# haiciyang/LaDiffCodec

Measured on AMD Instinct MI355X. Metric: audio-sec decoded / wall-sec, 16kHz 3kbps 50-step DDPM, higher is better.
Workload: dtype bf16; 1 GPU; LaDiffCodec 3 kbps, diff_dims=256, enc_ratios 8 4, 50-step DDPM, batch=32x2.4 s utterances per GPU; global_batch=32, latent_len=1200, denoise_steps=50, rccl_ranks=1, batches_in_flight=1, parallelism=dp1 (utterance-sharded, no data-path collective)

## Files before the change

include/ladiffcodec.h:

```cpp
#ifndef LADIFFCODEC_H_
#define LADIFFCODEC_H_

#include <stdint.h>

#ifdef __cplusplus
extern "C" {
#endif

#define LDC_OK 0
#define LDC_E_INVALID -1
#define LDC_E_STATE -2
#define LDC_E_MISSING -3
#define LDC_E_HIP -4
#define LDC_E_NOMEM -5

#define LDC_F32 0
#define LDC_BF16 1
#define LDC_BF16_W8 2

#define LDC_MODEL_MAIN 0
#define LDC_MODEL_COND 1

#define LDC_MAX_RATIOS 8

// ... 146 lines not shown
                     int32_t* cdf_out, void* stream);
int ldc_ac_encode(ldc_ctx* ctx, const int32_t* symbols, const int32_t* cdf, int B, int S, int card, int n_static, int total_range_bits,
                  uint8_t* out, int64_t out_stride, int64_t* nbytes_out, void* stream);
int ldc_ac_decode(ldc_ctx* ctx, const uint8_t* in, int64_t in_stride, const int64_t* nbytes, const int32_t* cdf, int B, int S, int card,
                  int n_static, int total_range_bits, int32_t* symbols_out, int32_t* status_out, void* stream);
int ldc_ac_encode_ragged(ldc_ctx* ctx, const int32_t* symbols, const int32_t* n_sym, const int32_t* cdf, int B, int S, int card,
                         int n_static, int total_range_bits, uint8_t* out, int64_t out_stride, int64_t* nbytes_out, void* stream);
int ldc_ac_decode_ragged(ldc_ctx* ctx, const uint8_t* in, int64_t in_stride, const int64_t* nbytes, const int32_t* n_sym,
                         const int32_t* cdf, int B, int S, int card, int n_static, int total_range_bits, int32_t* symbols_out,
                         int32_t* status_out, void* stream);

int64_t ldc_resample_out_len(int64_t T, int orig_freq, int new_freq);
int ldc_resample(ldc_ctx* ctx, const float* wav, int C, int64_t T, int orig_freq, int new_freq, float* out, void* stream);

int ldc_train_q_sample(ldc_ctx* ctx, const float* x_start, const int64_t* t, const float* noise, int B, int C, int L, float* x_t,
                       void* stream);
int ldc_train_num_timesteps(ldc_ctx* ctx);
int ldc_train_predict_x_start(ldc_ctx* ctx, const float* x_t, const float* eps, const int64_t* t, int B, int C, int L, float* x0_out,
                              void* stream);
int ldc_train_neg_sdsdr(ldc_ctx* ctx, const float* est, const float* tgt, int B, int64_t n_per_item, float clip_min, float* per_item_out,
                        void* stream);

int ldc_train_l1_loss(ldc_ctx* ctx, const float* model_out, const float* target, const int64_t* t, int B, int C, int L, float* loss_out,
                      float* grad_out, void* stream);
int64_t ldc_train_block_ws_floats(int B, int Cin, int Cout, int L, int groups);
int ldc_train_block_forward(ldc_ctx* ctx, const float* x, const float* w, const float* bias, const float* gamma, const float* beta,
                            const float* scale_shift, int B, int Cin, int Cout, int L, int groups, float* y, float* ws, void* stream);
int ldc_train_block_backward(ldc_ctx* ctx, const float* dy, const float* x, const float* gamma, const float* beta,
                             const float* scale_shift, int B, int Cin, int Cout, int L, int groups, float* ws, float* dx, float* dw,
                             float* db, float* dgamma, float* dbeta, float* dscale_shift, void* stream);

int ldc_train_layernorm_forward(ldc_ctx* ctx, const float* x, const float* g, int B, int C, int L, float* y, float* stats, void* stream);
int ldc_train_layernorm_backward(ldc_ctx* ctx, const float* dy, const float* x, const float* g, const float* stats, int B, int C, int L,
                                 float* dx, float* dg, void* stream);

int ldc_train_pointwise_forward(ldc_ctx* ctx, const float* x, const float* w, const float* bias, int B, int Cin, int Cout, int L, int pre_silu,
                                float* y, void* stream);
int ldc_train_pointwise_backward(ldc_ctx* ctx, const float* dy, const float* x, const float* w, int B, int Cin, int Cout, int L, int pre_silu,
                                 float* dx, float* dw, float* db, void* stream);

int64_t ldc_train_linattn_ws_floats(int B, int heads, int dim_head, int N);
int ldc_train_linattn_forward(ldc_ctx* ctx, const float* qkv, int B, int heads, int dim_head, int N, float* out, float* ws, void* stream);
int ldc_train_linattn_backward(ldc_ctx* ctx, const float* dout, const float* qkv, int B, int heads, int dim_head, int N, float* ws, float* dqkv,
                               void* stream);

int ldc_train_conv_forward(ldc_ctx* ctx, const float* x, const float* w, const float* bias, int B, int Cin, int Cout, int Lin, int K, int stride,
                           int pad, float* y, void* stream);
int ldc_train_conv_backward(ldc_ctx* ctx, const float* dy, const float* x, const float* w, int B, int Cin, int Cout, int Lin, int K, int stride,
                            int pad, float* dx, float* dw, float* db, void* stream);
int ldc_train_join(ldc_ctx* ctx, void* stream);
int ldc_train_side_stream(ldc_ctx* ctx, void** stream_out);
int ldc_train_upsample2(ldc_ctx* ctx, const float* in, int64_t rows, int L, int backward, float* out, void* stream);
int ldc_train_activation(ldc_ctx* ctx, const float* x, const float* dy, int64_t n, int kind, float* out, void* stream);
int64_t ldc_train_attn_ws_floats(int B, int heads, int N);
int ldc_train_attn_forward(ldc_ctx* ctx, const float* qkv, int B, int heads, int dim_head, int N, float* out, float* ws, void* stream);
int ldc_train_attn_backward(ldc_ctx* ctx, const float* dout, const float* qkv, int B, int heads, int dim_head, int N, float* ws, float* dqkv,
                            void* stream);

int ldc_train_convtr_forward(ldc_ctx* ctx, const float* x, const float* w, const float* bias, int B, int Cin, int Cout, int L, int ratio, float* y,
                             void* stream);
int ldc_train_convtr_backward(ldc_ctx* ctx, const float* dy, const float* x, const float* w, int B, int Cin, int Cout, int L, int ratio, float* dx,
                              float* dw, float* db, void* stream);
int ldc_train_maxscale(ldc_ctx* ctx, const float* x, const float* dy, int B, int64_t n_per_item, float* out, void* stream);

int ldc_train_adam_step(ldc_ctx* ctx, float* param, const float* grad, float* exp_avg, float* exp_avg_sq, int64_t n, int step, float lr,
                        float beta1, float beta2, float eps, void* stream);
int ldc_train_adam_step_dev(ldc_ctx* ctx, float* param, const float* grad, float* exp_avg, float* exp_avg_sq, int64_t n, int32_t* step_dev,
                            float lr, float beta1, float beta2, float eps, void* stream);

int ldc_sconv1d(ldc_ctx* ctx, const float* x, int B, int Cin, int L, const float* w_host, const float* b_host,
                int Cout, int k, int stride, int dilation, int causal, int pre_elu, float* y, void* stream);
int ldc_sconvtr1d(ldc_ctx* ctx, const float* x, int B, int Cin, int L, const float* w_host, const float* b_host,
                  int Cout, int k, int stride, int causal, float* y, void* stream);
int ldc_slstm(ldc_ctx* ctx, const float* x, int B, int H, int T, const float* const* weights_host, int layers,
              float* y, void* stream);

int ldc_unet_debug_tap(ldc_ctx* ctx, const char* name, float* out, int64_t capacity_elems, void* stream);
int ldc_unet_step_cost(ldc_ctx* ctx, int B, int L, double* flops, double* bytes);
int ldc_profile_enable(ldc_ctx* ctx, int on);
int ldc_xcc_census(ldc_ctx* ctx, const uint32_t* mask, int n_words, int wgs, int* hist16);

int ldc_debug_attn_core(ldc_ctx* ctx, int kind, const float* qkv, int B, int L, const float* w_out, const float* b_out,
                        const float* gain, const float* resid, int C, float* out, void* stream);
int ldc_debug_attention_block(ldc_ctx* ctx, const char* name, const float* x, int B, int L, float* out, void* stream);

int ldc_debug_sea_conv(ldc_ctx* ctx, const float* x, int B, int Cin, int L, const float* w_host, const float* b_host, int Cout, int k,
                       int stride, int dilation, int causal, int transposed, int pre_elu, const float* residual, float* y, int* route,
                       void* stream);
int ldc_debug_sea_op(ldc_ctx* ctx, int which, int decoder, int index, const float* x, int B, int L, float* out, int64_t capacity_elems,
                     int* info, void* stream);

int ldc_debug_raise_failure(ldc_ctx* ctx, int code);
long long ldc_debug_sync_count(void);

int ldc_host_stats(ldc_ctx* ctx, int reset, double* graph_launch_ms, double* lookahead_wait_ms, int64_t* graph_launches);
int ldc_stream_info(ldc_ctx* ctx, int* good, int* candidates, double* one_spin_ms, double* all_spin_ms, int* parts);
int ldc_clock_sample(ldc_ctx* ctx, uint64_t* out2, void* stream);

int ldc_timeline_enable(ldc_ctx* ctx, int on);
int ldc_timeline_read(ldc_ctx* ctx, int part, int n, uint64_t* ticks);
int ldc_kstamps_enable(ldc_ctx* ctx, int on);
int ldc_kstamps_reset(ldc_ctx* ctx);
int ldc_kstamps_read(ldc_ctx* ctx, int idx, int n_steps, int* n_ops, uint64_t* ticks, char* infos, int info_cap, int* classes);
int ldc_gn_microbench(ldc_ctx* ctx, int dtype, int B, int L, int C, int with_residual, int iters, double* ms_per_launch);
int ldc_conv_microbench(ldc_ctx* ctx, int dtype, int B, int L, int cin1, int cin2, int cout, int k, int stride, int ups,
                        int iters, double* ms_per_launch);
int ldc_conv_compare(ldc_ctx* ctx, int dtype, int B, int L, int cin1, int cin2, int cout, int k, int stride, int ups, int tile_cfg,
                     int with_gn, int with_colmax, int with_residual, double* max_abs_diff, double* max_abs_ref, double* max_rel_stat);
int ldc_ln_fold_compare(ldc_ctx* ctx, int dtype, int rows, int C, int n_out, double dc, double* max_abs_diff2, double* max_abs_ref);
int ldc_conv_compare_fp8(ldc_ctx* ctx, int B, int L, int cin1, int cin2, int cout, int k, int stride, int ups, int with_gn, int with_colmax,
                         double* max_abs_diff, double* max_abs_ref, double* max_rel_stat);
int ldc_profile_read(ldc_ctx* ctx, double* conv_ms_total, int64_t* conv_launches, double* conv_flops_total);
enum {
  LDC_CLASS_OTHER = 0,
  LDC_CLASS_CONV = 1,
  LDC_CLASS_GN_APPLY = 2,
  LDC_CLASS_LAYERNORM = 3,
  LDC_CLASS_LINATTN = 4,
  LDC_CLASS_ATTN_FULL = 5,
  LDC_CLASS_ELEMENTWISE = 6,
  LDC_N_CLASSES = 7
};
int ldc_profile_read_classes(ldc_ctx* ctx, int n, double* ms, int64_t* launches, double* flops, double* bytes);

#ifdef __cplusplus
}
#endif
#endif
```

ladiffcodec_amd/csrc/attention.hip:

```cpp
#include <algorithm>

#include "ldc_kernels.h"
#include "ldc_math.h"

namespace ldc {

__device__ __forceinline__ float abf2f(unsigned short h) { return __uint_as_float(((unsigned)h) << 16); }
__device__ __forceinline__ unsigned short af2bf(float f) { return hw_bf16(f); }
template <typename T>
__device__ __forceinline__ float ld1(const void* p, size_t i);
template <>
__device__ __forceinline__ float ld1<float>(const void* p, size_t i) { return reinterpret_cast<const float*>(p)[i]; }
template <>
__device__ __forceinline__ float ld1<__bf16>(const void* p, size_t i) {
  return abf2f(reinterpret_cast<const unsigned short*>(p)[i]);
}
template <typename T>
__device__ __forceinline__ void st1(void* p, size_t i, float v);
template <>
__device__ __forceinline__ void st1<float>(void* p, size_t i, float v) { reinterpret_cast<float*>(p)[i] = v; }
template <>
__device__ __forceinline__ void st1<__bf16>(void* p, size_t i, float v) {
  reinterpret_cast<unsigned short*>(p)[i] = af2bf(v);
}
// ... 47 lines not shown
  float acc[4] = {0.f, 0.f, 0.f, 0.f};
  float ssum = 0.f;
  for (int t0 = r0; t0 < r1; t0 += TR) {
    const int nr = min(TR, r1 - t0);
    for (int idx = tid; idx < TR * D; idx += 256) {
      const int r = idx / D, c = idx % D;
      float p = 0.f, v = 0.f;
      if (r < nr) {
        const size_t base = ((size_t)(b * L + t0 + r)) * (3 * HD);
        p = __expf(ld1<T>(qkv, base + HD + h * D + c) - skmax[c]);
        v = ld1<T>(qkv, base + 2 * HD + h * D + c);
      }
      sp[r][c] = p;
      sv[r][c] = v;
    }
    __syncthreads();
#pragma unroll 8
    for (int r = 0; r < TR; ++r) {
      const float p = sp[r][d];
      const float4 v4 = *reinterpret_cast<const float4*>(&sv[r][e0]);
      acc[0] += p * v4.x; acc[1] += p * v4.y; acc[2] += p * v4.z; acc[3] += p * v4.w;
      ssum += p;
    }
    __syncthreads();
  }
  float* ctx = wsb + 2 * HD + (size_t)h * D * D;
#pragma unroll
  for (int j = 0; j < 4; ++j) atomicAdd(&ctx[d * D + e0 + j], acc[j]);
  if ((tid % 8) == 0) atomicAdd(&wsb[HD + h * D + d], ssum);
}

template <typename T, int D>
__global__ __launch_bounds__(256) void linattn_out_kernel(const void* qkv, void* out, const float* ws, int L, int H,
                                                          size_t ws_stride, float scale, const int* lens, int shift) {
  constexpr int HS = D * D + 8;
  extern __shared__ __attribute__((aligned(16))) char smem_raw[];
  float* sctx = reinterpret_cast<float*>(smem_raw);
  const int HD = H * D;
  const int rows_per_block = 256 / H;
  const int b = blockIdx.y;
  const float* wsb = ws + (size_t)b * ws_stride;
  for (int idx = threadIdx.x; idx < H * D * D; idx += 256) {
    const int h = idx / (D * D), rem = idx % (D * D), d = rem / D;
    sctx[h * HS + rem] = wsb[2 * HD + idx] / wsb[HD + h * D + d];
  }
  __syncthreads();
  const int h = threadIdx.x % H;
  const int r = blockIdx.x * rows_per_block + threadIdx.x / H;
  if (r >= L) return;
  if (r >= valid_rows(lens, shift, b, L)) {
    const size_t ob = ((size_t)(b * L + r)) * HD + h * D;
#pragma unroll
    for (int e = 0; e < D; ++e) st1<T>(out, ob + e, 0.f);
    return;
  }
  const size_t base = ((size_t)(b * L + r)) * (3 * HD) + h * D;
  float q[D];
  float m = -INFINITY;
#pragma unroll
  for (int d = 0; d < D; ++d) { q[d] = ld1<T>(qkv, base + d); m = fmaxf(m, q[d]); }
  float s = 0.f;
#pragma unroll
  for (int d = 0; d < D; ++d) { q[d] = __expf(q[d] - m); s += q[d]; }
  const float inv = scale / s;
#pragma unroll
  for (int d = 0; d < D; ++d) q[d] *= inv;
  const float* c = sctx + h * HS;
  const size_t obase = ((size_t)(b * L + r)) * HD + h * D;
#pragma unroll
  for (int e0 = 0; e0 < D; e0 += 4) {
    float4 o = make_float4(0.f, 0.f, 0.f, 0.f);
#pragma unroll
    for (int d = 0; d < D; ++d) {
      const float4 cv = *reinterpret_cast<const float4*>(&c[d * D + e0]);
      o.x += cv.x * q[d]; o.y += cv.y * q[d]; o.z += cv.z * q[d]; o.w += cv.w * q[d];
    }
    st1<T>(out, obase + e0 + 0, o.x); st1<T>(out, obase + e0 + 1, o.y);
    st1<T>(out, obase + e0 + 2, o.z); st1<T>(out, obase + e0 + 3, o.w);
  }
}

typedef float lf32x16 __attribute__((ext_vector_type(16)));
typedef __bf16 lbf16x8 __attribute__((ext_vector_type(8)));
__device__ __forceinline__ lf32x16 mfma_bf16(const uint4& a, const uint4& b, lf32x16 acc) {
  lbf16x8 va, vb;
  __builtin_memcpy(&va, &a, 16);
  __builtin_memcpy(&vb, &b, 16);
  return __builtin_amdgcn_mfma_f32_32x32x16_bf16(va, vb, acc, 0, 0, 0);
}

template <int R>
__global__ __launch_bounds__(256) void linattn_ctx_mfma_kernel(const unsigned short* qkv, float* ws, int Lfull, size_t ws_stride, const int* lens, int shift) {
  constexpr int H = 4, D = 32, HD = 128, P = R + 8;
  __shared__ __attribute__((aligned(16))) unsigned short spT[HD][P];
  __shared__ __attribute__((aligned(16))) unsigned short svT[HD][P];
  __shared__ float skmax[HD];
  const int b = blockIdx.y, tid = threadIdx.x;
  float* wsb = ws + (size_t)b * ws_stride;
  const int r0 = blockIdx.x * R;
  const int L = valid_rows(lens, shift, b, Lfull);
  if (r0 >= L) return;
  constexpr int NP = R / 16;
  uint4 kk[NP], vv[NP];
#pragma unroll
  for (int i = 0; i < NP; ++i) {
    const int id = tid + 256 * i, row = id >> 4, c16 = id & 15;
    if (r0 + row < L) {
      const unsigned short* base = qkv + ((size_t)b * Lfull + r0 + row) * (3 * HD) + 8 * c16;
      kk[i] = *reinterpret_cast<const uint4*>(base + HD);
      vv[i] = *reinterpret_cast<const uint4*>(base + 2 * HD);
    } else {
      kk[i] = make_uint4(0, 0, 0, 0); vv[i] = make_uint4(0, 0, 0, 0);
    }
  }
  if (tid < HD) skmax[tid] = fkey_inv(reinterpret_cast<const unsigned*>(wsb)[tid]);
  __syncthreads();
#pragma unroll
  for (int i = 0; i < NP; ++i) {
    const int id = tid + 256 * i, row = id >> 4, c16 = id & 15;
    const bool live = r0 + row < L;
    const unsigned kw[4] = {kk[i].x, kk[i].y, kk[i].z, kk[i].w};
    const unsigned vw[4] = {vv[i].x, vv[i].y, vv[i].z, vv[i].w};
#pragma unroll
    for (int m = 0; m < 8; ++m) {
      const int col = 8 * c16 + m;
      const unsigned short kb = (unsigned short)((m & 1) ? (kw[m >> 1] >> 16) : (kw[m >> 1] & 0xffffu));
      const unsigned short vb = (unsigned short)((m & 1) ? (vw[m >> 1] >> 16) : (vw[m >> 1] & 0xffffu));
      spT[col][row] = live ? af2bf(__expf(abf2f(kb) - skmax[col])) : (unsigned short)0;
      svT[col][row] = vb;
    }
  }
  __syncthreads();
  const int h = tid >> 6, lane = tid & 63, i32 = lane & 31, g = lane >> 5;
  lf32x16 acc;
#pragma unroll
  for (int r = 0; r < 16; ++r) acc[r] = 0.f;
#pragma unroll
  for (int sx = 0; sx < R / 16; ++sx) {
    const uint4 a = *reinterpret_cast<const uint4*>(&spT[h * D + i32][16 * sx + 8 * g]);
    const uint4 bq = *reinterpret_cast<const uint4*>(&svT[h * D + i32][16 * sx + 8 * g]);
    acc = mfma_bf16(a, bq, acc);
  }
  float* ctx = wsb + 2 * HD + (size_t)h * D * D;
#pragma unroll
  for (int r = 0; r < 16; ++r) {
    const int d = (r & 3) + 8 * (r >> 2) + 4 * g;
    atomicAdd(&ctx[d * D + i32], acc[r]);
  }
  if (tid < HD) {
    float sum = 0.f;
#pragma unroll
    for (int q8 = 0; q8 < R / 8; ++q8) {
      const uint4 u = *reinterpret_cast<const uint4*>(&spT[tid][8 * q8]);
      const unsigned w[4] = {u.x, u.y, u.z, u.w};
#pragma unroll
      for (int m = 0; m < 4; ++m) sum += abf2f((unsigned short)(w[m] & 0xffffu)) + abf2f((unsigned short)(w[m] >> 16));
    }
    atomicAdd(&wsb[HD + tid], sum);
  }
}

template <int TILES>
__global__ __launch_bounds__(256) void linattn_out_mfma_kernel(const unsigned short* qkv, unsigned short* out, const float* ws,
                                                               int L, size_t ws_stride, float scale, const int* lens, int shift) {
  constexpr int D = 32, HD = 128;
  const int b = blockIdx.y, tid = threadIdx.x;
  const int h = tid >> 6, lane = tid & 63, i32 = lane & 31, g = lane >> 5;
  const int r0 = blockIdx.x * (32 * TILES);
  const int Lv = valid_rows(lens, shift, b, L);
  uint4 qq[TILES][2];
#pragma unroll
  for (int t = 0; t < TILES; ++t) {
    const int n = r0 + 32 * t + i32;
#pragma unroll
    for (int sx = 0; sx < 2; ++sx) {
      if (n < Lv) qq[t][sx] = *reinterpret_cast<const uint4*>(qkv + ((size_t)b * L + n) * (3 * HD) + h * D + 16 * sx + 8 * g);
      else qq[t][sx] = make_uint4(0, 0, 0, 0);
    }
  }
  const float* wsb = ws + (size_t)b * ws_stride;
  uint4 af[2];
#pragma unroll
  for (int sx = 0; sx < 2; ++sx) {
    unsigned w[4];
#pragma unroll
    for (int m = 0; m < 8; m += 2) {
      const int d0 = 16 * sx + 8 * g + m;
      const float c0 = wsb[2 * HD + (size_t)h * D * D + d0 * D + i32] * (scale / wsb[HD + h * D + d0]);
      const float c1 = wsb[2 * HD + (size_t)h * D * D + (d0 + 1) * D + i32] * (scale / wsb[HD + h * D + d0 + 1]);
      w[m >> 1] = (unsigned)af2bf(c0) | ((unsigned)af2bf(c1) << 16);
    }
    af[sx] = make_uint4(w[0], w[1], w[2], w[3]);
  }
#pragma unroll
  for (int t = 0; t < TILES; ++t) {
    const int n = r0 + 32 * t + i32;
    float x[16];
    float mx = -INFINITY;
#pragma unroll
    for (int sx = 0; sx < 2; ++sx) {
      const unsigned w[4] = {qq[t][sx].x, qq[t][sx].y, qq[t][sx].z, qq[t][sx].w};
#pragma unroll
      for (int m = 0; m < 4; ++m) {
        x[8 * sx + 2 * m] = abf2f((unsigned short)(w[m] & 0xffffu));
        x[8 * sx + 2 * m + 1] = abf2f((unsigned short)(w[m] >> 16));
      }
    }
#pragma unroll
    for (int m = 0; m < 16; ++m) mx = fmaxf(mx, x[m]);
    mx = fmaxf(mx, __shfl_xor(mx, 32));
    float sum = 0.f;
#pragma unroll
    for (int m = 0; m < 16; ++m) { x[m] = __expf(x[m] - mx); sum += x[m]; }
    sum += __shfl_xor(sum, 32);
    const float inv = 1.0f / sum;
    uint4 bq[2];
#pragma unroll
    for (int sx = 0; sx < 2; ++sx) {
      unsigned w[4];
#pragma unroll
      for (int m = 0; m < 4; ++m)
        w[m] = (unsigned)af2bf(x[8 * sx + 2 * m] * inv) | ((unsigned)af2bf(x[8 * sx + 2 * m + 1] * inv) << 16);
      bq[sx] = make_uint4(w[0], w[1], w[2], w[3]);
    }
    lf32x16 acc;
#pragma unroll
    for (int r = 0; r < 16; ++r) acc[r] = 0.f;
    acc = mfma_bf16(af[0], bq[0], acc);
    acc = mfma_bf16(af[1], bq[1], acc);
    if (n < L) {
      unsigned short* orow = out + ((size_t)b * L + n) * HD + h * D;
#pragma unroll
      for (int rr = 0; rr < 4; ++rr) {
        const unsigned lo = (unsigned)af2bf(acc[4 * rr]) | ((unsigned)af2bf(acc[4 * rr + 1]) << 16);
        const unsigned hi = (unsigned)af2bf(acc[4 * rr + 2]) | ((unsigned)af2bf(acc[4 * rr + 3]) << 16);
        *reinterpret_cast<uint2*>(orow + 8 * rr + 4 * g) = n < Lv ? make_uint2(lo, hi) : make_uint2(0u, 0u);
      }
    }
  }
}


__device__ __forceinline__ float reduce16_over32(const float (&v)[16], int lane) {
  float a8[8], a4[4], a2[2];
  const bool b4 = lane & 16, b3 = lane & 8, b2 = lane & 4, b1 = lane & 2;
#pragma unroll
  for (int k = 0; k < 8; ++k) a8[k] = (b4 ? v[8 + k] : v[k]) + __shfl_xor(b4 ? v[k] : v[8 + k], 16);
#pragma unroll
  for (int k = 0; k < 4; ++k) a4[k] = (b3 ? a8[4 + k] : a8[k]) + __shfl_xor(b3 ? a8[k] : a8[4 + k], 8);
#pragma unroll
  for (int k = 0; k < 2; ++k) a2[k] = (b2 ? a4[2 + k] : a4[k]) + __shfl_xor(b2 ? a4[k] : a4[2 + k], 4);
  float a1 = (b1 ? a2[1] : a2[0]) + __shfl_xor(b1 ? a2[0] : a2[1], 2);
  a1 += __shfl_xor(a1, 1);
  return a1;
}

template <int C>
__global__ __launch_bounds__(256) void linattn_tail_mfma_kernel(const unsigned short* qkv, const float* ws, size_t ws_stride, float scale,
                                                                const unsigned short* wo, int n_pad, const float* bias, const float* gain,
                                                                const unsigned short* resid, unsigned short* out, int L, unsigned* fail_flag) {
  constexpr int D = 32, HD = 128, R = 32, CPW = C / 4, NT = CPW / 32;
  constexpr int AP = HD + 8;
  constexpr int TP = CPW * 4 + 16;
  extern __shared__ __attribute__((aligned(16))) char smem[];
  unsigned short* sA = reinterpret_cast<unsigned short*>(smem);
  float* sred = reinterpret_cast<float*>(smem + (size_t)R * AP * 2);
  float* srow = sred + 4 * R;
  char* strans = smem + (size_t)R * AP * 2 + (size_t)5 * R * 4;
  const int b = blockIdx.y, tid = threadIdx.x;
  const int w = tid >> 6, lane = tid & 63, i32 = lane & 31, g = lane >> 5;
  const int r0 = blockIdx.x * R;
  const float* wsb = ws + (size_t)b * ws_stride;
  const int colw = w * CPW + i32;
  uint4 bfr[8][NT];
#pragma unroll
  for (int ks = 0; ks < 8; ++ks)
#pragma unroll
    for (int j = 0; j < NT; ++j)
      bfr[ks][j] = *reinterpret_cast<const uint4*>(wo + ((size_t)(ks >> 1) * n_pad + colw + 32 * j) * 32 + (ks & 1) * 16 + 8 * g);
  float bv[NT], gv[NT];
#pragma unroll
  for (int j = 0; j < NT; ++j) { bv[j] = bias[colw + 32 * j]; gv[j] = gain[colw + 32 * j]; }
  {
    const int h = w;
    const int n = r0 + i32;
    uint4 qq[2];
#pragma unroll
    for (int sx = 0; sx < 2; ++sx) {
      if (n < L) qq[sx] = *reinterpret_cast<const uint4*>(qkv + ((size_t)b * L + n) * (3 * HD) + h * D + 16 * sx + 8 * g);
      else qq[sx] = make_uint4(0, 0, 0, 0);
    }
    uint4 af[2];
    bool ks_bad = false;
#pragma unroll
    for (int sx = 0; sx < 2; ++sx) {
      unsigned wv[4];
#pragma unroll
      for (int m = 0; m < 8; m += 2) {
        const int d0 = 16 * sx + 8 * g + m;
        const float ks0 = wsb[HD + h * D + d0], ks1 = wsb[HD + h * D + d0 + 1];
        ks_bad |= !(ks0 >= kLinattnKsumMin && ks0 < kLinattnKsumMax) | !(ks1 >= kLinattnKsumMin && ks1 < kLinattnKsumMax);
        const float c0 = wsb[2 * HD + (size_t)h * D * D + d0 * D + i32] * (scale / ks0);
        const float c1 = wsb[2 * HD + (size_t)h * D * D + (d0 + 1) * D + i32] * (scale / ks1);
        wv[m >> 1] = (unsigned)af2bf(c0) | ((unsigned)af2bf(c1) << 16);
      }
      af[sx] = make_uint4(wv[0], wv[1], wv[2], wv[3]);
    }
    if (ks_bad && fail_flag) __hip_atomic_store(fail_flag, kDevFailCtxRange, __ATOMIC_RELAXED, __HIP_MEMORY_SCOPE_SYSTEM);
    float x[16];
    float mx = -INFINITY;
#pragma unroll
    for (int sx = 0; sx < 2; ++sx) {
      const unsigned wv[4] = {qq[sx].x, qq[sx].y, qq[sx].z, qq[sx].w};
#pragma unroll
      for (int m = 0; m < 4; ++m) {
        x[8 * sx + 2 * m] = abf2f((unsigned short)(wv[m] & 0xffffu));
        x[8 * sx + 2 * m + 1] = abf2f((unsigned short)(wv[m] >> 16));
      }
    }
#pragma unroll
    for (int m = 0; m < 16; ++m) mx = fmaxf(mx, x[m]);
    mx = fmaxf(mx, __shfl_xor(mx, 32));
    float sum = 0.f;
#pragma unroll
    for (int m = 0; m < 16; ++m) { x[m] = __expf(x[m] - mx); sum += x[m]; }
    sum += __shfl_xor(sum, 32);
    const float inv = 1.0f / sum;
    uint4 bq[2];
#pragma unroll
    for (int sx = 0; sx < 2; ++sx) {
      unsigned wv[4];
#pragma unroll
      for (int m = 0; m < 4; ++m)
        wv[m] = (unsigned)af2bf(x[8 * sx + 2 * m] * inv) | ((unsigned)af2bf(x[8 * sx + 2 * m + 1] * inv) << 16);
      bq[sx] = make_uint4(wv[0], wv[1], wv[2], wv[3]);
    }
    lf32x16 acc1;
#pragma unroll
    for (int r = 0; r < 16; ++r) acc1[r] = 0.f;
    acc1 = mfma_bf16(af[0], bq[0], acc1);
    acc1 = mfma_bf16(af[1], bq[1], acc1);
    unsigned short* arow = sA + (size_t)i32 * AP + h * D;
#pragma unroll
    for (int rr = 0; rr < 4; ++rr) {
      const unsigned lo = (unsigned)af2bf(acc1[4 * rr]) | ((unsigned)af2bf(acc1[4 * rr + 1]) << 16);
      const unsigned hi = (unsigned)af2bf(acc1[4 * rr + 2]) | ((unsigned)af2bf(acc1[4 * rr + 3]) << 16);
      *reinterpret_cast<uint2*>(arow + 8 * rr + 4 * g) = make_uint2(lo, hi);
    }
  }
  __syncthreads();
  lf32x16 acc[NT];
#pragma unroll
  for (int j = 0; j < NT; ++j)
#pragma unroll
    for (int r = 0; r < 16; ++r) acc[j][r] = 0.f;
#pragma unroll
  for (int ks = 0; ks < 8; ++ks) {
    const uint4 afr = *reinterpret_cast<const uint4*>(sA + (size_t)i32 * AP + 16 * ks + 8 * g);
#pragma unroll
    for (int j = 0; j < NT; ++j) acc[j] = mfma_bf16(afr, bfr[ks][j], acc[j]);
  }
  constexpr int LPR = CPW / 4;
  constexpr int RPS = 64 / LPR;
  constexpr int NSW = R / RPS;
  const int rsub = lane / LPR, piece = lane % LPR;
  uint2 rres[NSW];
#pragma unroll
  for (int sw = 0; sw < NSW; ++sw) {
    const int n = r0 + sw * RPS + rsub;
    rres[sw] = n < L ? *reinterpret_cast<const uint2*>(resid + ((size_t)b * L + n) * C + w * CPW + piece * 4) : make_uint2(0, 0);
  }
#pragma unroll
  for (int j = 0; j < NT; ++j)
#pragma unroll
    for (int r = 0; r < 16; ++r) acc[j][r] += bv[j];
  const int rr = i32 >> 1;
  const int my_row = (rr & 3) + 8 * (rr >> 2) + 4 * g;
  {
    float v[16];
#pragma unroll
    for (int r = 0; r < 16; ++r) {
      float sacc = 0.f;
#pragma unroll
      for (int j = 0; j < NT; ++j) sacc += acc[j][r];
      v[r] = sacc;
    }
    const float tot = reduce16_over32(v, lane);
    if ((lane & 1) == 0) sred[w * R + my_row] = tot;
  }
  __syncthreads();
  if (tid < R) srow[tid] = (sred[tid] + sred[R + tid] + sred[2 * R + tid] + sred[3 * R + tid]) * (1.0f / (float)C);
  __syncthreads();
  float mean[16];
#pragma unroll
  for (int r = 0; r < 16; ++r) mean[r] = srow[(r & 3) + 8 * (r >> 2) + 4 * g];
  {
    float v[16];
#pragma unroll
    for (int r = 0; r < 16; ++r) {
      float sacc = 0.f;
#pragma unroll
      for (int j = 0; j < NT; ++j) { const float d = acc[j][r] - mean[r]; sacc = fmaf(d, d, sacc); }
      v[r] = sacc;
    }
    const float tot = reduce16_over32(v, lane);
    if ((lane & 1) == 0) sred[w * R + my_row] = tot;
  }
  __syncthreads();
  if (tid < R) srow[tid] = rsqrtf((sred[tid] + sred[R + tid] + sred[2 * R + tid] + sred[3 * R + tid]) * (1.0f / (float)C) + 1e-5f);
  __syncthreads();
  char* tw = strans + (size_t)w * R * TP;
#pragma unroll
  for (int r = 0; r < 16; ++r) {
    const int row = (r & 3) + 8 * (r >> 2) + 4 * g;
    const float rstd = srow[row];
#pragma unroll
    for (int j = 0; j < NT; ++j)
      reinterpret_cast<float*>(tw + (size_t)row * TP)[32 * j + i32] = (acc[j][r] - mean[r]) * rstd * gv[j];
  }
#pragma unroll
  for (int sw = 0; sw < NSW; ++sw) {
    const int row = sw * RPS + rsub;
    const int n = r0 + row;
    const float4 y = *reinterpret_cast<const float4*>(tw + (size_t)row * TP + piece * 16);
    const float o0 = y.x + abf2f((unsigned short)(rres[sw].x & 0xffffu)), o1 = y.y + abf2f((unsigned short)(rres[sw].x >> 16));
    const float o2 = y.z + abf2f((unsigned short)(rres[sw].y & 0xffffu)), o3 = y.w + abf2f((unsigned short)(rres[sw].y >> 16));
    const uint2 o = make_uint2((unsigned)af2bf(o0) | ((unsigned)af2bf(o1) << 16), (unsigned)af2bf(o2) | ((unsigned)af2bf(o3) << 16));
    if (n < L) *reinterpret_cast<uint2*>(out + ((size_t)b * L + n) * C + w * CPW + piece * 4) = o;
  }
}

template <int C>
static hipError_t launch_tail_cfg(const void* qkv, const float* ws, size_t wss, float scale, const void* wo, int n_pad, const float* bias,
                                  const float* gain, const void* resid, void* out, int B, int L, unsigned* fail_flag, hipStream_t s) {
  constexpr int R = 32, CPW = C / 4;
  const size_t lds = (size_t)R * (128 + 8) * 2 + (size_t)5 * R * 4 + (size_t)4 * R * (CPW * 4 + 16);
  auto kern = linattn_tail_mfma_kernel<C>;
  static bool lds_opt_in = false;
  if (!lds_opt_in) {
    hipError_t e = hipFuncSetAttribute(reinterpret_cast<const void*>(kern), hipFuncAttributeMaxDynamicSharedMemorySize, 160 * 1024);
    if (e != hipSuccess) return e;
    lds_opt_in = true;
  }
  hipLaunchKernelGGL(kern, dim3((L + R - 1) / R, B), dim3(256), lds, s, reinterpret_cast<const unsigned short*>(qkv), ws, wss, scale,
                     reinterpret_cast<const unsigned short*>(wo), n_pad, bias, gain, reinterpret_cast<const unsigned short*>(resid),
                     reinterpret_cast<unsigned short*>(out), L, fail_flag);
  return hipGetLastError();
}

bool linattn_tail_supported(int dt, int heads, int dim_head, int C) {
  return dt == DT_BF16 && heads == 4 && dim_head == 32 && (C == 256 || C == 512 || C == 1024);
}

hipError_t launch_linattn_ctx(int dt, const void* qkv, float* ws, int B, int L, int heads, int dim_head, hipStream_t s) {
  if (dt != DT_BF16 || heads != 4 || dim_head != 32) return hipErrorInvalidValue;
  const size_t wss = linattn_ws_per_item(heads, dim_head);
  hipLaunchKernelGGL(linattn_ctx_mfma_kernel<64>, dim3((L + 63) / 64, B), dim3(256), 0, s, reinterpret_cast<const unsigned short*>(qkv), ws, L, wss,
                     static_cast<const int*>(nullptr), 0);
  return hipGetLastError();
}

hipError_t launch_linattn_tail(int dt, const void* qkv, const float* ws, const void* wo_packed, int n_pad, const float* bias, const float* gain,
                               const void* resid, void* out, int B, int L, int heads, int dim_head, int C, unsigned* fail_flag, hipStream_t s) {
  if (!linattn_tail_supported(dt, heads, dim_head, C) || !bias || !gain || !resid) return hipErrorInvalidValue;
  const size_t wss = linattn_ws_per_item(heads, dim_head);
  const float scale = 1.0f / sqrtf((float)dim_head);
  if (C == 256) return launch_tail_cfg<256>(qkv, ws, wss, scale, wo_packed, n_pad, bias, gain, resid, out, B, L, fail_flag, s);
  if (C == 512) return launch_tail_cfg<512>(qkv, ws, wss, scale, wo_packed, n_pad, bias, gain, resid, out, B, L, fail_flag, s);
  return launch_tail_cfg<1024>(qkv, ws, wss, scale, wo_packed, n_pad, bias, gain, resid, out, B, L, fail_flag, s);
}

size_t linattn_ws_floats_per_item(int heads, int dim_head) { return linattn_ws_per_item(heads, dim_head); }

hipError_t launch_linattn_kmax(int dt, const void* qkv, float* ws, int B, int L, int heads, int dim_head, hipStream_t s, const int* lens, int shift) {
  const int HD = heads * dim_head;
  if (dim_head != 32 || HD > 256 || 256 % HD) return hipErrorInvalidValue;
  const size_t wss = linattn_ws_per_item(heads, dim_head);
  hipError_t e = hipMemsetAsync(ws, 0, (size_t)B * wss * sizeof(float), s);
  if (e != hipSuccess) return e;
  const int rpb = 128;
  if (dt == DT_F32) hipLaunchKernelGGL(linattn_kmax_kernel<float>, dim3((L + rpb - 1) / rpb, B), dim3(256), 0, s, qkv, ws, L, HD, rpb, wss, lens, shift);
  else hipLaunchKernelGGL(linattn_kmax_kernel<__bf16>, dim3((L + rpb - 1) / rpb, B), dim3(256), 0, s, qkv, ws, L, HD, rpb, wss, lens, shift);
  return hipGetLastError();
}

hipError_t launch_linattn(int dt, const void* qkv, void* out, float* ws, int B, int L, int heads, int dim_head,
                          bool kmax_fused, hipStream_t s, const int* lens, int shift, bool ws_zeroed) {
  if (lens && kmax_fused) return hipErrorInvalidValue;
  if (dim_head != 32 || heads * dim_head > 256 || 256 % (heads * dim_head) || 256 % heads) return hipErrorInvalidValue;
  const int HD = heads * dim_head;
  const size_t wss = linattn_ws_per_item(heads, dim_head);
  if (!kmax_fused && !ws_zeroed) {
    hipError_t e = hipMemsetAsync(ws, 0, (size_t)B * wss * sizeof(float), s);
    if (e != hipSuccess) return e;
  }
  const int rpb = 128;
  const int chunks = (L + rpb - 1) / rpb;
  const float scale = 1.0f / sqrtf((float)dim_head);
  const size_t lds_out = (size_t)heads * (dim_head * dim_head + 8) * sizeof(float);
  const int rows_out = 256 / heads;
  if (dt == DT_BF16 && heads == 4) {
    if (!kmax_fused) hipLaunchKernelGGL(linattn_kmax_kernel<__bf16>, dim3(chunks, B), dim3(256), 0, s, qkv, ws, L, HD, rpb, wss, lens, shift);
    hipLaunchKernelGGL(linattn_ctx_mfma_kernel<64>, dim3((L + 63) / 64, B), dim3(256), 0, s,
                       reinterpret_cast<const unsigned short*>(qkv), ws, L, wss, lens, shift);
    hipLaunchKernelGGL(linattn_out_mfma_kernel<2>, dim3((L + 63) / 64, B), dim3(256), 0, s,
                       reinterpret_cast<const unsigned short*>(qkv), reinterpret_cast<unsigned short*>(out), ws, L, wss, scale, lens, shift);
  } else if (dt == DT_F32) {
    if (!kmax_fused) hipLaunchKernelGGL(linattn_kmax_kernel<float>, dim3(chunks, B), dim3(256), 0, s, qkv, ws, L, HD, rpb, wss, lens, shift);
    hipLaunchKernelGGL((linattn_ctx_kernel<float, 32>), dim3(chunks, B * heads), dim3(256), 0, s, qkv, ws, L, heads, rpb, wss, lens, shift);
    hipLaunchKernelGGL((linattn_out_kernel<float, 32>), dim3((L + rows_out - 1) / rows_out, B), dim3(256), lds_out, s, qkv,
                       out, ws, L, heads, wss, scale, lens, shift);
  } else {
    if (!kmax_fused) hipLaunchKernelGGL(linattn_kmax_kernel<__bf16>, dim3(chunks, B), dim3(256), 0, s, qkv, ws, L, HD, rpb, wss, lens, shift);
    hipLaunchKernelGGL((linattn_ctx_kernel<__bf16, 32>), dim3(chunks, B * heads), dim3(256), 0, s, qkv, ws, L, heads, rpb, wss, lens, shift);
    hipLaunchKernelGGL((linattn_out_kernel<__bf16, 32>), dim3((L + rows_out - 1) / rows_out, B), dim3(256), lds_out, s,
                       qkv, out, ws, L, heads, wss, scale, lens, shift);
  }
  return hipGetLastError();
}

template <typename T, int D>
__global__ __launch_bounds__(256) void attn_full_kernel(const void* qkv, void* out, int L, int H, float scale, int CH, const int* lens, int shift) {
  constexpr int P = D + 4;
  extern __shared__ __attribute__((aligned(16))) char smem_raw[];
  float* sk = reinterpret_cast<float*>(smem_raw);
  float* sv = sk + (size_t)CH * P;
  const int HD = H * D;
  const int b = blockIdx.x / H, h = blockIdx.x % H;
  const int part = threadIdx.x & 3;
  const int i = blockIdx.y * 64 + (threadIdx.x >> 2);
  const int Lv = valid_rows(lens, shift, b, L);
  const int iq = min(i, Lv - 1);
  float q[D], acc[D];
  const size_t qb = ((size_t)(b * L + iq)) * (3 * HD) + h * D;
#pragma unroll
  for (int d = 0; d < D; ++d) { q[d] = ld1<T>(qkv, qb + d) * scale; acc[d] = 0.f; }
  float m = -INFINITY, l = 0.f;
  for (int k0 = 0; k0 < Lv; k0 += CH) {
    const int nk = min(CH, Lv - k0);
    if (k0) __syncthreads();
    for (int idx = threadIdx.x; idx < nk * (D / 8); idx += 256) {
      const int r = idx / (D / 8), c8 = idx % (D / 8);
      const size_t base = ((size_t)(b * L + k0 + r)) * (3 * HD) + h * D + c8 * 8;
#pragma unroll
      for (int mm = 0; mm < 8; ++mm) {
        sk[r * P + c8 * 8 + mm] = ld1<T>(qkv, base + HD + mm);
        sv[r * P + c8 * 8 + mm] = ld1<T>(qkv, base + 2 * HD + mm);
      }
    }
    __syncthreads();
    for (int j = part; j < nk; j += 4) {
      const float4* kj = reinterpret_cast<const float4*>(sk + (size_t)j * P);
// ... 62 lines not shown
```

ladiffcodec_amd/csrc/ldc_api.cpp:

```cpp
#include "ldc_internal.h"

long long g_device_syncs = 0;

static thread_local char g_err[1024] = "";
int fail(int code, const char* fmt, ...) {
  va_list ap;
  va_start(ap, fmt);
  vsnprintf(g_err, sizeof(g_err), fmt, ap);
  va_end(ap);
  return code;
}

extern "C" const char* ldc_last_error(void) { return g_err; }
extern "C" const char* ldc_version(void) { return "ladiffcodec-amd 0.1 (gfx950)"; }



static std::vector<float> fold_weight_norm(const HostTensor& g, const HostTensor& v) {
  const size_t n0 = (size_t)v.shape[0], inner = v.numel() / n0;
  std::vector<float> w(v.numel());
  for (size_t i = 0; i < n0; ++i) {
    double s = 0;
    for (size_t j = 0; j < inner; ++j) s += (double)v.data[i * inner + j] * v.data[i * inner + j];
    const float nrm = (float)sqrt(s);
// ... 702 lines not shown
  return LDC_OK;
}

void drop_plans(ldc_ctx* c) {
  (void)counted_device_sync();
  for (auto& g : c->graphs) g.destroy();
  c->graphs.clear();
  for (auto& pl : c->plans) {
    for (hipEvent_t e : pl->marker_events) (void)hipEventDestroy(e);
    if (pl->arena_base) (void)hipFree(pl->arena_base);
    if (pl->x0_prev) (void)hipFree(pl->x0_prev);
    if (pl->win_base) (void)hipFree(pl->win_base);
  }
  c->plans.clear();
  c->plan_bytes = 0;
  c->last_halves = Halves();
}

extern "C" int ldc_destroy(ldc_ctx* c) {
  if (!c) return LDC_OK;
  (void)hipSetDevice(c->device);
  (void)counted_device_sync();
  drop_plans(c);
  if (c->scratch) (void)hipFree(c->scratch);
  if (c->outnorm_ws) (void)hipFree(c->outnorm_ws);
  if (c->state_buf) (void)hipFree(c->state_buf);
  if (c->ddim_table) (void)hipFree(c->ddim_table);
  if (c->dpm_table) (void)hipFree(c->dpm_table);
  if (c->step_state) (void)hipFree(c->step_state);
  if (c->dev_flag_host) (void)hipHostFree(c->dev_flag_host);
  if (c->tl_buf) (void)hipFree(c->tl_buf);
  for (auto& e : c->prof_events) { (void)hipEventDestroy(e.first); (void)hipEventDestroy(e.second); }
  if (c->ev_fork) (void)hipEventDestroy(c->ev_fork);
  for (int k = 0; k < kMaxParts; ++k) {
    for (int e = 0; e <= ldc_ctx::kLstmChunks; ++e)
      if (c->lstm_ev[k][e]) (void)hipEventDestroy(c->lstm_ev[k][e]);
  }
  for (auto& e : c->flow_ev) if (e) (void)hipEventDestroy(e);
  for (int k = 1; k < kMaxParts; ++k) {
    if (c->ev_join[k]) (void)hipEventDestroy(c->ev_join[k]);
    if (c->aux_stream[k]) (void)hipStreamDestroy(c->aux_stream[k]);
  }
  for (int k = 0; k < kMaxParts; ++k) {
    if (c->ev_side_fork[k]) (void)hipEventDestroy(c->ev_side_fork[k]);
    if (c->ev_side_join[k]) (void)hipEventDestroy(c->ev_side_join[k]);
    if (c->side_stream[k]) (void)hipStreamDestroy(c->side_stream[k]);
  }
  if (c->own_stream) (void)hipStreamDestroy(c->own_stream);
  delete c;
  return LDC_OK;
}

extern "C" void ldc_quantize_e4m3(const float* in, int64_t n, uint8_t* out_codes, float* out_values) {
  for (int64_t i = 0; i < n; ++i) {
    const uint8_t q = host_f32_to_e4m3(in[i]);
    if (out_codes) out_codes[i] = q;
    if (out_values) out_values[i] = host_e4m3_to_f32(q);
  }
}

struct OptRef { int* p; bool replan; int lo, hi; };
static bool find_option(ldc_ctx* c, const std::string& n, OptRef* r) {
#define LDC_OPT(NAME, FIELD, REPLAN, LO, HI) if (n == NAME) { r->p = &(FIELD); r->replan = REPLAN; r->lo = LO; r->hi = HI; return true; }
  LDC_OPT("split", c->split_batch, true, 1, kMaxParts)
  LDC_OPT("part_graphs", c->part_graphs, false, 0, 2)
  LDC_OPT("graph_steps", c->graph_steps, false, 0, 1000)
  LDC_OPT("flow_depth", c->flow_depth, false, 0, (int)ldc_ctx::kFlowRing - 1)
  LDC_OPT("split_ends", c->split_ends, false, 0, 1)
  LDC_OPT("ends_join", c->ends_join, false, 0, 1)
  LDC_OPT("split_init", c->split_init, true, 0, 1)
  LDC_OPT("side_streams", c->side_streams, true, 0, 1)
  LDC_OPT("serial_parts", c->serial_parts, false, 0, 1)
  LDC_OPT("stream_calib", c->calib, false, 0, 1)
  LDC_OPT("merge_advance", c->merge_advance, true, 0, 1)
  LDC_OPT("fuse_gn_stats", c->fuse_gn_stats, true, 0, 1)
  LDC_OPT("fuse_gn_epi", c->fuse_gn_epi, true, 0, 1)
  LDC_OPT("gn_epi_min_l", c->gn_epi_min_l, true, 0, 1 << 30)
  LDC_OPT("gn_epi_max_tiles", c->gn_epi_max_tiles, true, 0, 1 << 30)
  LDC_OPT("fold_res", c->fold_res, true, 0, 1)
  LDC_OPT("fold_ln", c->fold_ln, true, 0, 1)
  LDC_OPT("fuse_kmax", c->fuse_kmax, true, 0, 1)
  LDC_OPT("fuse_ln", c->fuse_ln, true, 0, 1)
  LDC_OPT("fuse_attn_tail", c->fuse_attn_tail, true, 0, 1)
  LDC_OPT("fold_ctx", c->fold_ctx, true, 0, 1)
  LDC_OPT("conv_lean", c->tune.lean, true, 0, 1)
  LDC_OPT("conv_generic", c->tune.force_generic, true, 0, 1)
  LDC_OPT("conv_small_tiles", c->tune.small_max, true, 0, 1 << 30)
  LDC_OPT("conv_splitk", c->tune.splitk, true, 0, 4)
  LDC_OPT("sk_tiles", c->tune.sk_tiles, true, 0, 1 << 30)
  LDC_OPT("sk_u2", c->tune.sk_u2, true, 0, 1 << 30)
  LDC_OPT("sk_u3", c->tune.sk_u3, true, 0, 1 << 30)
  LDC_OPT("conv_mfast", c->tune.m_fastest, true, 0, 2)
  LDC_OPT("conv_debug", c->tune.debug, true, 0, 255)
  LDC_OPT("conv_tile", c->tune.force_tile, true, -1, 1)
  LDC_OPT("conv_xcd_order", c->tune.xcd_order, true, 0, 8)
  LDC_OPT("gn_nap", c->tune.gn_nap, true, 0, 4096)
  LDC_OPT("gn_nap0", c->tune.gn_nap0, true, 0, 4096)
  LDC_OPT("lstm_stream", c->lstm_stream_only, false, 0, 1)
  LDC_OPT("lstm_xcd", c->lstm_xcd, false, 0, 1)
  LDC_OPT("lstm_pipe", c->lstm_pipe, false, 0, 1)
  LDC_OPT("coop_launch", c->coop_launch, false, 0, 1)
  LDC_OPT("sea_splitk", c->sea_splitk, false, 0, 1)
  LDC_OPT("rvq_tiled", c->rvq_tiled, false, 0, 1)
  LDC_OPT("train_bf16", g_train_bf16, false, 0, 1)
  LDC_OPT("train_fp32_mfma", g_train_fp32_mfma, false, 0, 1)
  LDC_OPT("train_valu", g_train_valu, false, 0, 1)
  LDC_OPT("train_dw_side", g_train_dw_side, false, 0, 1)
#undef LDC_OPT
  return false;
}

extern "C" int ldc_set_option(ldc_ctx* c, const char* name, int value) {
  if (!c || !name) return fail(LDC_E_INVALID, "null context or option name");
  const std::string n(name);
  if (n == "fp8_act") {
    if (c->finalized) return fail(LDC_E_STATE, "fp8_act must be set before ldc_finalize_weights");
    c->fp8_act = value ? 1 : 0;
    return LDC_OK;
  }
  if (n == "plan_cache_gb") { c->plan_bytes_cap = (size_t)std::max(1, value) << 30; return LDC_OK; }
  if (n == "plan_cache_n") { c->plan_count_cap = std::max(2 * kMaxParts, value); return LDC_OK; }
  OptRef r;
  if (!find_option(c, n, &r)) return fail(LDC_E_INVALID, "unknown option '%s' (tools/README.md lists the options)", name);
  if (value < r.lo || value > r.hi) return fail(LDC_E_INVALID, "option %s must be in %d..%d", name, r.lo, r.hi);
  if (n == "side_streams" && value && c->split_batch != 1) return fail(LDC_E_INVALID, "side streams need a single chain (split 1)");
  if (value == *r.p) return LDC_OK;
  if (r.replan && c->live_pools > 0)
    return fail(LDC_E_STATE, "option %s rebuilds every plan, and %d decode pool(s) keep their items' state in theirs: destroy the pools first", name, c->live_pools);
  if (r.replan && !c->plans.empty()) { HIPCHK(hipSetDevice(c->device)); drop_plans(c); }
  *r.p = value;
  if (n == "split" && value != 1) c->side_streams = 0;
  return LDC_OK;
}

extern "C" long long ldc_debug_sync_count(void) { return g_device_syncs; }

extern "C" int ldc_debug_raise_failure(ldc_ctx* c, int code) {
  if (!c || !c->dev_flag_host || (code != 1 && code != 2 && code != (int)kDevFailCtxRange)) return fail(LDC_E_INVALID, "bad arguments");
  *reinterpret_cast<volatile unsigned*>(c->dev_flag_host) = (unsigned)code;
  return LDC_OK;
}

extern "C" int ldc_reseed(ldc_ctx* c, uint64_t seed) {
  if (!c) return fail(LDC_E_INVALID, "null ctx");
  c->cfg.noise_seed = seed;
  c->noise_epoch = 0;
  return LDC_OK;
}

extern "C" int ldc_set_weight(ldc_ctx* c, int which, const char* key, const float* data, const int64_t* shape, int ndim) {
  if (!c || !key || !data || (ndim > 0 && !shape)) return fail(LDC_E_INVALID, "null argument");
  if (which != LDC_MODEL_MAIN && which != LDC_MODEL_COND) return fail(LDC_E_INVALID, "which must be LDC_MODEL_MAIN or LDC_MODEL_COND");
  if (c->finalized) return fail(LDC_E_STATE, "weights already finalized");
  HostTensor t;
  t.shape.assign(shape, shape + ndim);
  t.data.assign(data, data + t.numel());
  c->raw[which][key] = std::move(t);
  return LDC_OK;
}

extern "C" int ldc_finalize_weights(ldc_ctx* c, int strict) {
  if (!c) return fail(LDC_E_INVALID, "null ctx");
  if (c->finalized) return fail(LDC_E_STATE, "already finalized");
  HIPCHK(hipSetDevice(c->device));
  std::string missing;
  std::vector<int> main_ratios(c->cfg.enc_ratios, c->cfg.enc_ratios + c->cfg.n_enc_ratios);
// ... 609 lines not shown
      };
      epi1 = (!f8 || dt == DT_BF16) && few_tiles(t1) && t1[0] <= 2 * L && take_part(&ge1, L, t1[0], t1[1], r.cout);
      conv_bm(f8 ? r.c2_f8 : r.c2, L, L, false, t2);
      epi2 = (!(out_mode & 1) || dt == DT_BF16) && few_tiles(t2) && t2[0] <= 2 * L && take_part(&ge2, L, t2[0], t2[1], r.cout);
    }
    void* a = epi1 ? nullptr : act(rows, r.cout);
    void* d = epi2 ? nullptr : act(rows, r.cout);
    const void* res = x1;
    bool folded = false;
    void* rr = r.has_res ? act(rows, r.cout) : nullptr;
    if (r.has_res && c->fold_res && r.c1r.w) {
      int t[4];
      conv_bm(r.c1, L, L, false, t);
      folded = t[0] > 0 && t[2] == 1;
    }
    if (r.has_res && !folded) {
      mark(2);
      where = 1;
      conv(r.res, x1, x2, rr, nullptr, L, L);
      where = 0;
    }
    if (r.has_res) res = rr;
    const ConvLayer& c1 = folded ? r.c1r : r.c1;
    const ResnetW* rp = &r;
    if (epi1) {
      ge1.gamma = r.g1; ge1.beta = r.b1; ge1.ss = cur_ss + r.ss_off; ge1.out = f8 ? 1 : 0;
      if (folded) y2_next = rr;
      conv(c1, x1, x2, b, nullptr, L, L, nullptr, nullptr, 0, 0, 0, &ge1);
    } else {
      if (folded) y2_next = rr;
      conv(c1, x1, x2, a, nullptr, L, L, fuse_stats ? st1 : nullptr);
      if (!fuse_stats) add([=](hipStream_t s) { return launch_gn_stats(dt, a, Bn, L, rp->cout, g, st1, s, ln, sh); });
      add([=](hipStream_t s) {
        if (item_t)
          return launch_gn_apply(dt, a, b, nullptr, Bn, L, rp->cout, g, st1, rp->g1, rp->b1, ss_tab, ss_stride, item_t, ACT_SILU, s, nullptr,
                                 nullptr, 0, ln, sh, kItemStateInts, n_t);
        return launch_gn_apply(dt, a, b, nullptr, Bn, L, rp->cout, g, st1, rp->g1, rp->b1, cur_ss + rp->ss_off,
                               0, nullptr, ACT_SILU, s, nullptr, nullptr, f8 ? 1 : 0, ln, sh);
      }, false, 0, LDC_CLASS_GN_APPLY, (f8 ? 1.5 : 2.0) * Bn * L * rp->cout * es);
    }
    void* xn = nullptr;
    if (ln_g && xn_out && c->fuse_ln && !ln && gn_apply_ln_fusable(r.cout)) {
      xn = xn_fp8 ? ar->alloc((size_t)rows * r.cout) : act(rows, r.cout);
      *xn_out = xn;
    }
    if (epi2) {
      ge2.gamma = r.g2; ge2.beta = r.b2; ge2.ss = nullptr; ge2.out = out_mode & 5;
      if (rowstat_wanted && !f8) ge2.rowstat = last_rowstat = (float*)ar->alloc((size_t)rows * (r.cout / 32) * 8);
      if (r.has_res && !folded) mark(3);
      conv(f8 ? r.c2_f8 : r.c2, b, nullptr, out, res, L, L, nullptr, nullptr, 0, 0, 0, &ge2);
      if (xn) {
        const int C = r.cout;
        add([=](hipStream_t s) { return launch_ln_rows(dt, out, xn, nullptr, ln_g, rows, C, s, xn_fp8 ? 1 : 0); }, false, 0, LDC_CLASS_LAYERNORM,
            (xn_fp8 ? 1.5 : 2.0) * rows * C * es);
      }
      return out;
    }
    conv(f8 ? r.c2_f8 : r.c2, b, nullptr, d, nullptr, L, L, fuse_stats ? st2 : nullptr);
    if (!fuse_stats) add([=](hipStream_t s) { return launch_gn_stats(dt, d, Bn, L, rp->cout, g, st2, s, ln, sh); });
    if (r.has_res && !folded) mark(3);
    const int out8_ln = ((xn && xn_fp8) ? 2 : 0) | (gn_apply_fp8_ok(r.cout) ? out_mode : 0);
    add([=](hipStream_t s) {
      return launch_gn_apply(dt, d, out, res, Bn, L, rp->cout, g, st2, rp->g2, rp->b2, nullptr, 0, nullptr, ACT_SILU, s, xn, ln_g, out8_ln, ln, sh);
    }, false, 0, LDC_CLASS_GN_APPLY, (xn ? 4.0 : 3.0) * Bn * L * rp->cout * es);
    return out;
  }
  bool qkv_fp8(const LinAttnW& a) const { return c->w8 && c->fp8_act && a.qkv_f8.w != nullptr; }
  bool ln_foldable(const LinAttnW& a, int L) {
    if (pl->ragged || !c->fold_ln || !c->fuse_gn_epi || c->w8 || !a.qkv_ln.w || L < c->gn_epi_min_l) return false;
    int t[4];
    conv_bm(a.qkv_ln, L, L, false, t);
    return t[0] > 0;
  }
  void* attention(const LinAttnW& a, const void* x, int L, bool linear, void* xn_pre = nullptr) {
    const int rows = B * L, dt = c->dt, Bn = B;
    const int H = c->unet.heads, Dh = c->unet.dim_head, hid = H * Dh;
    const bool f8 = qkv_fp8(a);
    const bool lnf = !xn_pre && ln_foldable(a, L);
    const float* rowstat = lnf ? last_rowstat : nullptr;
    last_rowstat = nullptr;
    void* xn = lnf ? const_cast<void*>(x) : (xn_pre ? xn_pre : (f8 ? ar->alloc((size_t)rows * a.dim) : act(rows, a.dim)));
    const ConvLayer& qkv_ly = lnf ? a.qkv_ln : (f8 ? a.qkv_f8 : a.qkv);
    void* qkv = act(rows, 3 * hid);
    void* o = act(rows, hid);
    void* out = act(rows, a.dim);
    const LinAttnW* ap = &a;
    const int* ln = lens();
    const int sh = ln ? level(L) : 0;
    float* ws = (linear && (c->fuse_kmax || ln)) ? linattn_ws + (size_t)(linattn_used++) * B * linattn_ws_floats_per_item(H, Dh) : linattn_ws;
    if (!xn_pre && !lnf)
      add([=](hipStream_t s) { return launch_ln_rows(dt, x, xn, nullptr, ap->norm_g, rows, ap->dim, s, f8 ? 1 : 0, ln, sh, L); }, false, 0, LDC_CLASS_LAYERNORM,
          2.0 * rows * a.dim * es);
    if (linear) {
      const size_t wss = linattn_ws_floats_per_item(H, Dh);
      if (!ln && c->fuse_kmax && c->fuse_attn_tail && !a.out.w8 && linattn_tail_supported(dt, H, Dh, a.dim)) {
        ln_rowstat_next = rowstat;
        if (lnf && c->fold_ctx && c->tune.lean && !c->tune.force_generic && dt == DT_BF16 && a.qkv_ctx.w && hid == 128 && a.dim % 64 == 0) {
          qkv_ctx_next = ws; qkv_ctx_stride_next = (int)wss;
          conv(a.qkv_ctx, xn, nullptr, qkv, nullptr, L, L);
        } else {
          conv(qkv_ly, xn, nullptr, qkv, nullptr, L, L, nullptr, reinterpret_cast<unsigned*>(ws), hid, 2 * hid, (int)wss);
          add([=](hipStream_t s) { return launch_linattn_ctx(dt, qkv, ws, Bn, L, H, Dh, s); }, false, 0, LDC_CLASS_LINATTN, 2.0 * rows * hid * es);
        }
        const int dim = a.dim;
        info = "tail_c" + std::to_string(dim) + "_L" + std::to_string(L) + "_B" + std::to_string(B);
        unsigned* flag = c->dev_flag_dev;
        add([=](hipStream_t s) {
          return launch_linattn_tail(dt, qkv, ws, ap->out.w, ap->out.n_pad, ap->out.bias, ap->out_g, x, out, Bn, L, H, Dh, dim, flag, s);
        }, false, 2.0 * rows * hid * dim, LDC_CLASS_LINATTN, (1.0 * hid + 2.0 * dim) * rows * es);
        return out;
      }
      if (c->fuse_kmax && !ln) {
        ln_rowstat_next = rowstat;
        conv(qkv_ly, xn, nullptr, qkv, nullptr, L, L, nullptr, reinterpret_cast<unsigned*>(ws), hid, 2 * hid, (int)wss);
        add([=](hipStream_t s) { return launch_linattn(dt, qkv, o, ws, Bn, L, H, Dh, true, s); }, false, 0, LDC_CLASS_LINATTN,
            4.0 * rows * hid * es);
      } else {
        ln_rowstat_next = rowstat;
        conv(qkv_ly, xn, nullptr, qkv, nullptr, L, L);
        add([=](hipStream_t s) { return launch_linattn(dt, qkv, o, ws, Bn, L, H, Dh, false, s, ln, sh, ln != nullptr); }, false, 0, LDC_CLASS_LINATTN,
            5.0 * rows * hid * es);
      }
      void* t = act(rows, a.dim);
      conv(a.out, o, nullptr, t, nullptr, L, L);
      add([=](hipStream_t s) { return launch_ln_rows(dt, t, out, x, ap->out_g, rows, ap->dim, s, 0, ln, sh, L); }, false, 0, LDC_CLASS_LAYERNORM,
          3.0 * rows * a.dim * es);
    } else {
      ln_rowstat_next = rowstat;
      conv(qkv_ly, xn, nullptr, qkv, nullptr, L, L);
      add([=](hipStream_t s) { return launch_attn_full(dt, qkv, o, Bn, L, H, Dh, s, ln, sh); }, false, 0, LDC_CLASS_ATTN_FULL, 4.0 * rows * hid * es);
      conv(a.out, o, nullptr, out, x, L, L);
      mask(out, L, a.dim);
    }
    return out;
  }
};

int build_plan(ldc_ctx* c, Plan* pl, Arena& ar, int B, int L, int F) {
  const UnetW& u = c->unet;
  pl->B = B; pl->L = L; pl->F = F; pl->init_pc = nullptr;
  pl->cond_ops.clear(); pl->step_ops.clear(); pl->step_is_conv.clear(); pl->step_where.clear(); pl->step_flops.clear(); pl->step_class.clear(); pl->step_bytes.clear(); pl->step_info.clear(); pl->taps.clear();
  pl->flops = 0; pl->act_bytes = 0; pl->conv_bytes = 0; pl->sk_need_max = 0; pl->part_need = 0;
  const int dt = c->dt;
  const size_t es = dt_size(dt);
  const int Cc = u.cond_channels, Cx = u.channels;
  PlanBuilder pb{c, pl, &ar, B, es};
  pl->zero_once.clear();
  const int n_gn = 2 * (int)(2 * u.downs.size() + 2 + 2 * u.ups.size() + 1);
  const size_t gn_bytes = (size_t)n_gn * B * u.groups * kGnPad * 4;
  const bool lin_zeroed = c->fuse_kmax || pl->ragged;
  const size_t n_lin = lin_zeroed ? u.downs.size() + u.ups.size() : 1;
  const size_t lin_bytes = n_lin * B * linattn_ws_floats_per_item(u.heads, u.dim_head) * 4;
  const int sk_tiles_cap = 1024;
  const size_t part_bytes = (pl->part_bytes + 63) / 64 * 64;
  const size_t sk_count_bytes = (size_t)sk_tiles_cap * 4 + part_bytes;
  const size_t sx_bytes = c->cfg.unet_scale_x ? (size_t)B * 4 : 0;
  pb.stats_pool = (float*)ar.alloc(gn_bytes + sk_count_bytes + lin_bytes + sx_bytes + 64);
  pb.sk_count = reinterpret_cast<unsigned*>(pb.stats_pool + gn_bytes / 4);
  pb.part_pool = reinterpret_cast<char*>(pb.sk_count + sk_tiles_cap);
  pb.part_cap = part_bytes;
  pb.sk_count_cap = sk_tiles_cap;
  pb.linattn_ws = pb.stats_pool + (gn_bytes + sk_count_bytes) / 4;
  float* sx_max = pb.linattn_ws + (lin_zeroed ? lin_bytes / 4 : 0);
  const size_t stats_bytes = gn_bytes + sk_count_bytes + (lin_zeroed ? lin_bytes : 0) + sx_bytes;
  pb.sk_part_cap = pl->sk_floats;
  pb.sk_part = (float*)ar.alloc((size_t)std::max<long long>(pb.sk_part_cap, 4) * 4);
  pl->maxabs = (float*)ar.alloc((size_t)B * 4);
  pl->step_state = (int*)ar.alloc(64);
  if (ar.base) pl->zero_once.push_back({pl->step_state, 64});
  pl->kst = c->kstamps ? (unsigned long long*)ar.alloc((size_t)2048 * kKstOps * 2 * 8) : nullptr;
  pl->cur_ss = (float*)ar.alloc((size_t)std::max(1, u.ss_stride) * 4);
  pl->x_cl = ar.alloc((size_t)B * L * Cx * es);
  pl->eps_cl = ar.alloc((size_t)B * L * Cx * es);
  pl->cond_cl = ar.alloc((size_t)B * L * Cc * es);
  if (pl->items && !pl->ragged) return fail(LDC_E_INVALID, "a per-item plan is a ragged plan");
  pl->item_state = pl->items ? (ItemState*)ar.alloc((size_t)B * sizeof(ItemState)) : nullptr;
  if (pl->ragged) {
    if (c->w8) return fail(LDC_E_INVALID, "ragged batches are not available on the fp8 engine (its fused forms have no length-aware variant): use dtype bf16 or f32");
    pl->lens = (int*)ar.alloc((size_t)B * 4);
    pl->flens = (int*)ar.alloc((size_t)B * 4);
  } else {
    pl->lens = pl->flens = nullptr;
  }
  void* cond_in = ar.alloc((size_t)B * F * Cc * 4);
  pl->cond_in_cl = cond_in;
  {
    const void* x = cond_in;
    int Lc = F;
    const int Bn0 = B;
    const int *rl = pl->ragged ? pl->lens : nullptr, *rf = pl->ragged ? pl->flens : nullptr;
    if (rf) pl->cond_ops.push_back([=](hipStream_t s) { return launch_mask_rows(DT_F32, cond_in, Bn0, F, Cc, rf, 0, s); });
    for (const ConvLayer& ly : u.upsamplers) {
      ConvCall cc;
      cc.B = B; cc.L_in = Lc; cc.L_rows = Lc + 1; cc.L_final = Lc * ly.tr_stride; cc.y_ld = ly.tr_cout; cc.x1 = x; cc.tune = &c->tune;
      void* y = ar.alloc((size_t)B * cc.L_final * ly.tr_cout * 4);
      cc.y = y;
      const ConvLayer* lp = &ly;
      pl->cond_ops.push_back([lp, cc](hipStream_t s) { return launch_conv(*lp, cc, s); });
      if (rf) {
        const int row = cc.L_final / F * ly.tr_cout;
        pl->cond_ops.push_back([=](hipStream_t s) { return launch_mask_rows(DT_F32, y, Bn0, F, row, rf, 0, s); });
      }
      x = y;
      Lc = cc.L_final;
    }
    (void)rl;
    if (Lc != L) return fail(LDC_E_INVALID, "upsampled condition length %d != latent length %d (F=%d, upsampling product %d)", Lc, L, F, upsample_factor(c));
    float* mx = pl->maxabs;
    void* cond_cl = pl->cond_cl;
    const bool scale = c->cfg.unet_scale_cond != 0;
    const int Bn = B;
    const int64_t npi = (int64_t)L * Cc;
// ... 353 lines not shown
                          0, 0.f, s));
  }
  return finish_stream(c, stream);
}

static int unet_halvings(const ldc_ctx* c) {
  int n = 0;
  for (const LevelW& lv : c->unet.downs) n += lv.kind == 0;
  return n;
}
static long long lcm_ll(long long a, long long b) {
  long long x = a, y = b;
  while (y) { const long long t = x % y; x = y; y = t; }
  return a / x * b;
}
int ragged_latent_quantum(const ldc_ctx* c) { return (int)lcm_ll(upsample_factor(c), 1ll << unet_halvings(c)); }
static int check_ragged_lengths(const int32_t* lens, int B, int maxlen, long long quantum, const char* unit) {
  if (!lens) return fail(LDC_E_INVALID, "null lengths");
  if (maxlen <= 0 || maxlen % quantum) return fail(LDC_E_INVALID, "the padded length %d is not a positive multiple of %lld %s", maxlen, quantum, unit);
  for (int b = 0; b < B; ++b)
    if (lens[b] <= 0 || lens[b] > maxlen || lens[b] % quantum)
      return fail(LDC_E_INVALID, "length %d of item %d must be a multiple of %lld %s in (0, %d]", (int)lens[b], b, quantum, unit, maxlen);
  return LDC_OK;
}
static int write_plan_lens(ldc_ctx* c, const Halves& h, const std::vector<int>& lat, hipStream_t s) {
  const int up = upsample_factor(c);
  for (int k = 0; k < h.n; ++k) {
    Plan* pl = h.p[k];
    std::vector<int> fr(pl->B);
    for (int b = 0; b < pl->B; ++b) fr[b] = lat[h.b0[k] + b] / up;
    HIPCHK(launch_lens_write(pl->lens, lat.data() + h.b0[k], pl->B, s));
    HIPCHK(launch_lens_write(pl->flens, fr.data(), pl->B, s));
  }
  return LDC_OK;
}

extern "C" int ldc_unet_forward_ragged(ldc_ctx* c, const float* x, int t, const float* cond, const int32_t* latent_lens_host, int B, int Lmax,
                                       int Fmax, float* eps_out, void* stream) {
  LDCCHK(check_ready(c, LDC_MODEL_MAIN));
  if (!x || !cond || !eps_out) return fail(LDC_E_INVALID, "null tensor");
  if (t < 0 || t >= c->unet.timesteps) return fail(LDC_E_INVALID, "t out of range");
  LDCCHK(check_unet_args(c, B, Lmax, Fmax));
  LDCCHK(check_ragged_lengths(latent_lens_host, B, Lmax, ragged_latent_quantum(c), "latent frames"));
  if (c->w8) return fail(LDC_E_INVALID, "ragged batches are not available on the fp8 engine (its fused forms have no length-aware variant): use dtype bf16 or f32");
  hipStream_t s = pick_stream(c, stream);
  Halves h;
  LDCCHK(get_halves(c, B, Lmax, Fmax, s, &h, true));
  LDCCHK(write_plan_lens(c, h, std::vector<int>(latent_lens_host, latent_lens_host + B), s));
  LDCCHK(load_cond(c, h, cond, s));
  LDCCHK(load_x(c, h, x, s));
  for (int k = 0; k < h.n; ++k) {
    Plan* pl = h.p[k];
    HIPCHK(launch_mask_rows(c->dt, pl->x_cl, pl->B, Lmax, c->unet.channels, pl->lens, 0, s));
    HIPCHK(launch_step_set(pl->step_state, t, 0, c->cur_key, s));
    HIPCHK(launch_step_begin(c->unet.ss_table, c->unet.ss_stride, pl->step_state, pl->cur_ss, nullptr, s, pl->zero_ptr, pl->zero_bytes));
    LDCCHK(run_ops(c, pl, pl->step_ops, true, s));
    HIPCHK(launch_mask_rows(c->dt, pl->eps_cl, pl->B, Lmax, c->unet.channels, pl->lens, 0, s));
    HIPCHK(launch_from_cl(c->dt, pl->eps_cl, eps_out + (size_t)h.b0[k] * c->unet.channels * Lmax, pl->B, c->unet.channels, Lmax, nullptr,
                          0, 0.f, s));
  }
  return finish_stream(c, stream);
}

extern "C" int ldc_unet_debug_tap(ldc_ctx* c, const char* name, float* out, int64_t capacity, void* stream) {
  LDCCHK(check_ready(c, LDC_MODEL_MAIN));
  if (!name || !out) return fail(LDC_E_INVALID, "null argument");
  const Halves& h = c->last_halves;
  if (h.n == 0) return fail(LDC_E_STATE, "no UNet call has been made yet");
  int64_t need = 0;
  for (int k = 0; k < h.n; ++k) {
    auto it = h.p[k]->taps.find(name);
    if (it == h.p[k]->taps.end()) return fail(LDC_E_INVALID, "unknown tap '%s'", name);
    need += (int64_t)h.p[k]->B * it->second.C * it->second.L;
  }
  if (capacity < need) return fail(LDC_E_INVALID, "tap '%s' needs %lld elements", name, (long long)need);
  hipStream_t s = pick_stream(c, stream);
  for (int k = 0; k < h.n; ++k) {
    const Plan::Tap& tp = h.p[k]->taps.find(name)->second;
    HIPCHK(launch_from_cl(c->dt, tp.p, out + (size_t)h.b0[k] * tp.C * tp.L, h.p[k]->B, tp.C, tp.L, nullptr, 0, 0.f, s));
  }
  return finish_stream(c, stream);
}

extern "C" int ldc_debug_attention_block(ldc_ctx* c, const char* name, const float* x, int B, int L, float* out, void* stream) {
  LDCCHK(check_ready(c, LDC_MODEL_MAIN));
  if (!name || !x || !out || B <= 0 || L <= 0) return fail(LDC_E_INVALID, "bad arguments");
  const UnetW& u = c->unet;
  const LinAttnW* a = nullptr;
  bool linear = true;
  const std::string n = name;
  auto level = [&](const char* pre, const std::vector<LevelW>& lv) {
    const size_t pl = strlen(pre);
    if (n.compare(0, pl, pre) != 0 || n.size() == pl || n.find_first_not_of("0123456789", pl) != std::string::npos) return;
    const size_t i = (size_t)atoi(n.c_str() + pl);
    if (i < lv.size()) a = &lv[i].attn;
  };
  if (n == "mid") { a = &u.mid_attn; linear = false; }
  else { level("down", u.downs); level("up", u.ups); }
  if (!a) return fail(LDC_E_INVALID, "unknown attention block '%s' (down0..down%zu, mid, up0..up%zu)", name, u.downs.size() - 1, u.ups.size() - 1);
  hipStream_t s = pick_stream(c, stream);
  const int dt = c->dt, C = a->dim;
  const size_t es = dt_size(dt);
  const size_t lin_bytes = (size_t)B * linattn_ws_floats_per_item(u.heads, u.dim_head) * 4;
  const int sk_tiles_cap = 1024;
  Plan pl;
  pl.B = B; pl.L = L;
  void *x_cl = nullptr, *y_cl = nullptr, *zero = nullptr;
  auto build = [&](Arena& ar) {
    pl.step_ops.clear(); pl.step_is_conv.clear(); pl.step_where.clear(); pl.step_flops.clear(); pl.step_class.clear(); pl.step_bytes.clear(); pl.step_info.clear();
    pl.sk_need_max = 0; pl.part_need = 0;
    PlanBuilder pb{c, &pl, &ar, B, es};
    zero = ar.alloc((size_t)sk_tiles_cap * 4 + lin_bytes);
    pb.sk_count = reinterpret_cast<unsigned*>(zero);
    pb.sk_count_cap = sk_tiles_cap;
    pb.linattn_ws = reinterpret_cast<float*>(pb.sk_count + sk_tiles_cap);
    pb.sk_part_cap = pl.sk_floats;
    pb.sk_part = (float*)ar.alloc((size_t)std::max<long long>(pb.sk_part_cap, 4) * 4);
    x_cl = pb.act(B * L, C);
    y_cl = pb.attention(*a, x_cl, L, linear);
  };
  for (int pass = 0; pass < 2; ++pass) {
    Arena dry;
    build(dry);
    pl.sk_floats = std::max(pl.sk_floats, pl.sk_need_max);
  }
  Arena measure;
  build(measure);
  DevMem keep;
  void* base = nullptr;
  LDCCHK(keep.alloc(&base, measure.off + 4096));
  Arena real;
  real.base = (char*)base; real.cap = measure.off + 4096;
  build(real);
  HIPCHK(hipMemsetAsync(zero, 0, (size_t)sk_tiles_cap * 4 + lin_bytes, s));
  HIPCHK(launch_to_cl(dt, x, x_cl, B, C, L, nullptr, 0, 0.f, s));
  LDCCHK(run_ops(c, &pl, pl.step_ops, true, s));
  HIPCHK(launch_from_cl(dt, y_cl, out, B, C, L, nullptr, 0, 0.f, s));
  HIPCHK(hipStreamSynchronize(s));
  return check_dev_flag(c);
}

static int half_step(ldc_ctx* c, const Halves& h, int k, float* x, const float* noise, int64_t noise_stride, hipStream_t s,
                     const StepSampler& sm = StepSampler()) {
  Plan* pl = h.p[k];
  const size_t off = (size_t)h.b0[k] * c->unet.channels * pl->L;
  unsigned long long* tl = c->timeline ? c->tl_buf + (size_t)k * 2048 * 2 : nullptr;
  if (sm.kind == SAMPLER_DPM) {
    if (!sm.dpm || !pl->x0_prev) return fail(LDC_E_STATE, "internal: a DPM step without its schedule table or history buffer");
    HIPCHK(launch_step_begin_sched(c->unet.ss_table, c->unet.ss_stride, pl->step_state, pl->cur_ss, tl, s, pl->zero_ptr, pl->zero_bytes,
                                   c->merge_advance, &sm.dpm->t, (int)(sizeof(DpmStep) / sizeof(int))));
  } else {
    HIPCHK(launch_step_begin(c->unet.ss_table, c->unet.ss_stride, pl->step_state, pl->cur_ss, tl, s, pl->zero_ptr, pl->zero_bytes, c->merge_advance,
                             sm.kind == SAMPLER_DDIM ? sm.ddim : nullptr));
  }
  LDCCHK(run_ops(c, pl, pl->step_ops, true, s));
  if (pl->win_Ltot) {
    if (sm.kind == SAMPLER_DPM || h.n != 1) return fail(LDC_E_STATE, "internal: a windows plan steps as one part, on DDPM or DDIM");
    HIPCHK(launch_windows_update(c->dt, sm.kind == SAMPLER_DDIM ? WIN_DDIM : WIN_DDPM, x, pl->eps_cl, noise, noise_stride, pl->x_cl, nullptr,
                                 c->unet.channels, pl->win, c->sched, sm.ddim, pl->step_state, s));
  } else if (sm.kind == SAMPLER_DPM)
    HIPCHK(launch_dpm_update(c->dt, x + off, pl->eps_cl, pl->x0_prev, pl->x_cl, pl->B, c->unet.channels, pl->L, c->sched, sm.dpm,
                             pl->step_state, s, pl->ragged ? pl->lens : nullptr));
  else if (sm.kind == SAMPLER_DDIM)
    HIPCHK(launch_ddim_update(c->dt, x + off, pl->eps_cl, noise ? noise + off : nullptr, noise_stride, pl->x_cl, pl->B,
                              c->unet.channels, pl->L, c->sched, sm.ddim, pl->step_state, (uint64_t)off, s, pl->ragged ? pl->lens : nullptr));
  else
    HIPCHK(launch_p_sample_update(c->dt, x + off, pl->eps_cl, noise ? noise + off : nullptr, noise_stride, pl->x_cl, pl->B,
                                  c->unet.channels, pl->L, c->sched, pl->step_state, (uint64_t)off, s, pl->ragged ? pl->lens : nullptr));
  if (!c->merge_advance) HIPCHK(launch_step_advance(pl->step_state, tl, s));
  return LDC_OK;
}
static int stamp_loop_end(ldc_ctx* c, const Halves& h, int k, hipStream_t s) {
  if (!c->timeline || !c->merge_advance) return LDC_OK;
  HIPCHK(launch_step_advance(h.p[k]->step_state, c->tl_buf + (size_t)k * 2048 * 2, s));
  return LDC_OK;
}

bool parts_parallel(ldc_ctx* c, const Halves& h) {
  return h.n >= 2 && !c->profile && !c->serial_parts;
}
int fork_parts(ldc_ctx* c, const Halves& h, hipStream_t s) {
  HIPCHK(hipEventRecord(c->ev_fork, s));
// ... 1102 lines not shown
```

ladiffcodec_amd/csrc/ldc_api_tuning.cpp:

```cpp
#include "ldc_internal.h"

static int round_up(int v, int m) { return (v + m - 1) / m * m; }

extern "C" int ldc_sconv1d(ldc_ctx* c, const float* x, int B, int Cin, int L, const float* w_host, const float* b_host,
                           int Cout, int k, int stride, int dilation, int causal, int pre_elu, float* y, void* stream) {
  if (!c || !x || !w_host || !y) return fail(LDC_E_INVALID, "null argument");
  if (B <= 0 || Cin <= 0 || L <= 0 || Cout <= 0 || k <= 0 || stride <= 0 || dilation <= 0) return fail(LDC_E_INVALID, "bad sizes");
  HIPCHK(hipSetDevice(c->device));
  hipStream_t s = pick_stream(c, stream);
  const int cp = round_up(Cin, 16);
  std::vector<float> wp((size_t)Cout * cp * k, 0.f);
  for (int o = 0; o < Cout; ++o)
    for (int i = 0; i < Cin; ++i)
      for (int t = 0; t < k; ++t) wp[((size_t)o * cp + i) * k + t] = w_host[((size_t)o * Cin + i) * k + t];
  DevMem keep;
  std::swap(keep.ptrs, c->wmem.ptrs);
  ConvLayer ly;
  ConvSpec sp;
  sp.dt = DT_F32; sp.cin1 = cp; sp.cout = Cout; sp.k = k; sp.stride = stride; sp.dil = dilation;
  const int padding_total = (k - 1) * dilation - (stride - 1);
  sp.pad_left = causal ? padding_total : padding_total - padding_total / 2;
  sp.pad_mode = PAD_REFLECT; sp.pre_act = pre_elu ? ACT_ELU : ACT_NONE;
  int rc = make_conv(c, sp, wp.data(), b_host, &ly);
  std::swap(keep.ptrs, c->wmem.ptrs);
// ... 589 lines not shown
  const int L_out = ups ? 2 * L : (stride == 2 ? (L + 2 * sp.pad_left - k) / 2 + 1 : L);
  const size_t es = dt_size(dt);
  const int groups = 8;
  const size_t n_out = (size_t)B * L_out * cout, stat_n = (size_t)B * groups * kGnPad, cm_n = (size_t)B * cout;
  void *x1 = nullptr, *x2 = nullptr, *res = nullptr, *y[2] = {nullptr, nullptr}, *st[2] = {nullptr, nullptr}, *cm[2] = {nullptr, nullptr};
  LDCCHK(keep.alloc(&x1, (size_t)B * L * cin1 * es));
  LDCCHK(fill_random(x1, (size_t)B * L * cin1, dt, 901u));
  if (cin2) {
    LDCCHK(keep.alloc(&x2, (size_t)B * L * cin2 * es));
    LDCCHK(fill_random(x2, (size_t)B * L * cin2, dt, 902u));
  }
  if (with_residual) {
    LDCCHK(keep.alloc(&res, n_out * es));
    LDCCHK(fill_random(res, n_out, dt, 903u));
  }
  void *part = nullptr, *cnt = nullptr;
  LDCCHK(keep.alloc(&part, (size_t)(8 << 20) * 4));
  LDCCHK(keep.alloc(&cnt, 1024 * 4));
  HIPCHK(hipMemset(cnt, 0, 1024 * 4));
  hipStream_t s = c->own_stream;
  ConvTune tune = c->tune;
  for (int v = 0; v < 2; ++v) {
    LDCCHK(keep.alloc(&y[v], n_out * es));
    LDCCHK(keep.alloc(&st[v], stat_n * 4));
    LDCCHK(keep.alloc(&cm[v], cm_n * 4));
    HIPCHK(hipMemset(y[v], 0, n_out * es));
    HIPCHK(hipMemset(st[v], 0, stat_n * 4));
    HIPCHK(hipMemset(cm[v], 0, cm_n * 4));
    HIPCHK(hipDeviceSynchronize());
    const bool lean_ab = tile_cfg >= 100;
    tune.force_generic = lean_ab ? 0 : (v == 0 ? 1 : 0);
    if (lean_ab) tune.lean = tile_cfg >= 300 ? 1 : (tile_cfg >= 200 ? 0 : v);
    tune.force_tile = lean_ab ? (tile_cfg % 100 == 99 ? -1 : tile_cfg % 100) : tile_cfg;
    ConvCall cc;
    cc.B = B; cc.L_in = L; cc.L_rows = L_out; cc.x1 = x1; cc.x2 = x2; cc.y = y[v]; cc.y_ld = cout; cc.residual = res;
    if (with_gn) { cc.gn_sum = (float*)st[v]; cc.gn_groups = groups; }
    if (with_colmax) { cc.colmax = (unsigned*)cm[v]; cc.colmax_lo = 0; cc.colmax_hi = cout; cc.colmax_stride = cout; }
    cc.sk_part = (float*)part; cc.sk_part_cap = (long long)8 << 20; cc.sk_count = (unsigned*)cnt; cc.sk_count_cap = 1024;
    cc.tune = &tune;
    HIPCHK(launch_conv(ly, cc, s));
  }
  HIPCHK(hipStreamSynchronize(s));
  std::vector<char> h0(n_out * es), h1(n_out * es);
  HIPCHK(hipMemcpy(h0.data(), y[0], h0.size(), hipMemcpyDeviceToHost));
  HIPCHK(hipMemcpy(h1.data(), y[1], h1.size(), hipMemcpyDeviceToHost));
  auto val = [&](const std::vector<char>& h, size_t i) {
    if (dt == DT_F32) return (double)reinterpret_cast<const float*>(h.data())[i];
    const uint32_t u = (uint32_t)reinterpret_cast<const uint16_t*>(h.data())[i] << 16;
    float f;
    memcpy(&f, &u, 4);
    return (double)f;
  };
  double d = 0, m = 0;
  for (size_t i = 0; i < n_out; ++i) {
    const double a = val(h0, i), b = val(h1, i);
    if (!(b == b)) { d = 1e30; break; }
    d = std::max(d, fabs(a - b));
    m = std::max(m, fabs(a));
  }
  *max_abs_diff = d;
  *max_abs_ref = m;
  double rs = 0;
  if (with_gn) {
    std::vector<float> s0(stat_n), s1(stat_n);
    HIPCHK(hipMemcpy(s0.data(), st[0], stat_n * 4, hipMemcpyDeviceToHost));
    HIPCHK(hipMemcpy(s1.data(), st[1], stat_n * 4, hipMemcpyDeviceToHost));
    double smax = 0;
    for (size_t i = 0; i < stat_n; ++i) smax = std::max(smax, (double)fabsf(s0[i]));
    for (size_t i = 0; i < stat_n; ++i) rs = std::max(rs, fabs((double)s0[i] - s1[i]) / (smax + 1e-30));
  }
  if (with_colmax) {
    std::vector<unsigned> c0(cm_n), c1(cm_n);
    HIPCHK(hipMemcpy(c0.data(), cm[0], cm_n * 4, hipMemcpyDeviceToHost));
    HIPCHK(hipMemcpy(c1.data(), cm[1], cm_n * 4, hipMemcpyDeviceToHost));
    auto unkey = [](unsigned kx) { const unsigned b = (kx & 0x80000000u) ? (kx & 0x7fffffffu) : ~kx; float f; memcpy(&f, &b, 4); return (double)f; };
    for (size_t i = 0; i < cm_n; ++i) rs = std::max(rs, fabs(unkey(c0[i]) - unkey(c1[i])) / (m + 1e-30));
  }
  *max_rel_stat = rs;
  return LDC_OK;
}

extern "C" int ldc_debug_attn_core(ldc_ctx* c, int kind, const float* qkv, int B, int L, const float* w_out, const float* b_out,
                                   const float* gain, const float* resid, int C, float* out, void* stream) {
  if (!c || !qkv || !out || B < 1 || L < 1 || kind < 0 || kind > 3) return fail(LDC_E_INVALID, "bad arguments");
  HIPCHK(hipSetDevice(c->device));
  const int dt = c->dt, H = 4, D = 32, HD = H * D;
  const size_t es = dt_size(dt), wss = linattn_ws_floats_per_item(H, D);
  if (kind == 2 && (!w_out || !b_out || !gain || !resid || !linattn_tail_supported(dt, H, D, C)))
    return fail(LDC_E_INVALID, "the fused tail needs a bf16 context, C in {256, 512, 1024}, and to_out weight, bias, gain and residual");
  hipStream_t s = pick_stream(c, stream);
  const int Co = kind == 2 ? C : HD;
  DevMem keep;
  void *q_cl = nullptr, *o_cl = nullptr, *ws = nullptr, *r_cl = nullptr;
  LDCCHK(keep.alloc(&q_cl, (size_t)B * L * 3 * HD * es));
  LDCCHK(keep.alloc(&o_cl, (size_t)B * L * Co * es));
  LDCCHK(keep.alloc(&ws, (size_t)B * wss * 4));
  ConvLayer to_out;
  float* d_gain = nullptr;
  if (kind == 2) {
    const bool saved_w8 = c->w8;
    c->w8 = false;
    std::swap(keep.ptrs, c->wmem.ptrs);
    ConvSpec sp;
    sp.dt = dt; sp.cin1 = HD; sp.cout = C; sp.k = 1;
    int rc = make_conv(c, sp, w_out, b_out, &to_out);
    if (rc == LDC_OK) rc = c->wmem.upload(&d_gain, std::vector<float>(gain, gain + C));
    std::swap(keep.ptrs, c->wmem.ptrs);
    c->w8 = saved_w8;
    LDCCHK(rc);
    LDCCHK(keep.alloc(&r_cl, (size_t)B * L * C * es));
    HIPCHK(launch_to_cl(dt, resid, r_cl, B, C, L, nullptr, 0, 0.f, s));
  }
  HIPCHK(launch_to_cl(dt, qkv, q_cl, B, 3 * HD, L, nullptr, 0, 0.f, s));
  if (kind == 0) {
    HIPCHK(launch_linattn(dt, q_cl, o_cl, (float*)ws, B, L, H, D, false, s));
  } else if (kind == 1) {
    HIPCHK(launch_linattn_kmax(dt, q_cl, (float*)ws, B, L, H, D, s));
    HIPCHK(launch_linattn(dt, q_cl, o_cl, (float*)ws, B, L, H, D, true, s));
  } else if (kind == 2) {
    HIPCHK(launch_linattn_kmax(dt, q_cl, (float*)ws, B, L, H, D, s));
    HIPCHK(launch_linattn_ctx(dt, q_cl, (float*)ws, B, L, H, D, s));
    HIPCHK(launch_linattn_tail(dt, q_cl, (const float*)ws, to_out.w, to_out.n_pad, to_out.bias, d_gain, r_cl, o_cl, B, L, H, D, C, c->dev_flag_dev, s));
  } else {
    HIPCHK(launch_attn_full(dt, q_cl, o_cl, B, L, H, D, s));
  }
  HIPCHK(launch_from_cl(dt, o_cl, out, B, Co, L, nullptr, 0, 0.f, s));
  HIPCHK(hipStreamSynchronize(s));
  return check_dev_flag(c);
}

extern "C" int ldc_conv_compare_fp8(ldc_ctx* c, int B, int L, int cin1, int cin2, int cout, int k, int stride, int ups, int with_gn,
                                    int with_colmax, double* max_abs_diff, double* max_abs_ref, double* max_rel_stat) {
  if (!c || !max_abs_diff || !max_abs_ref || !max_rel_stat) return fail(LDC_E_INVALID, "bad arguments");
  if ((cin1 % 64) || (cin2 % 64)) return fail(LDC_E_INVALID, "fp8 inputs need channel counts that are multiples of 64");
  HIPCHK(hipSetDevice(c->device));
  const int cin = cin1 + cin2;
  std::vector<float> w((size_t)cout * cin * k), bias(cout);
  unsigned seed = 777u;
  for (auto& v : w) { seed = seed * 1664525u + 1013904223u; v = ((seed >> 8) * (1.0f / 16777216.0f) - 0.5f) * 0.2f; }
  for (auto& v : bias) { seed = seed * 1664525u + 1013904223u; v = ((seed >> 8) * (1.0f / 16777216.0f) - 0.5f); }
  DevMem keep;
  const bool saved_w8 = c->w8;
  c->w8 = true;
  std::swap(keep.ptrs, c->wmem.ptrs);
  ConvLayer ly[2];
  ConvSpec sp;
  sp.cin1 = cin1; sp.cin2 = cin2; sp.cout = cout; sp.k = k; sp.stride = stride; sp.ups = ups;
  sp.pad_left = (k == 4 && stride == 2) ? 1 : (k - 1) / 2;
  sp.dt = DT_BF16;
  int rc = make_conv(c, sp, w.data(), bias.data(), &ly[0]);
  sp.dt = DT_FP8; sp.act8 = 1;
  if (rc == LDC_OK) rc = make_conv(c, sp, w.data(), bias.data(), &ly[1]);
  std::swap(keep.ptrs, c->wmem.ptrs);
  c->w8 = saved_w8;
  LDCCHK(rc);
  const int L_out = ups ? 2 * L : (stride == 2 ? (L + 2 * sp.pad_left - k) / 2 + 1 : L);
  const int groups = 8;
  const size_t n_out = (size_t)B * L_out * cout, stat_n = (size_t)B * groups * kGnPad, cm_n = (size_t)B * cout;
  auto make_input = [&](size_t n, unsigned sd, void** d8, void** d16) -> int {
    std::vector<uint8_t> h8(n);
    std::vector<uint16_t> h16(n);
    for (size_t i = 0; i < n; ++i) {
      sd = sd * 1664525u + 1013904223u;
      uint8_t code = (uint8_t)(sd >> 13);
      if (((code >> 3) & 0xf) > 8) code = (uint8_t)((code & 0x87) | (8 << 3));
      h8[i] = code;
      const float f = host_e4m3_to_f32(code);
      uint32_t u;
      memcpy(&u, &f, 4);
      h16[i] = (uint16_t)(u >> 16);
    }
    LDCCHK(keep.alloc(d8, n));
    LDCCHK(keep.alloc(d16, n * 2));
    HIPCHK(hipMemcpy(*d8, h8.data(), n, hipMemcpyHostToDevice));
    HIPCHK(hipMemcpy(*d16, h16.data(), n * 2, hipMemcpyHostToDevice));
    return LDC_OK;
  };
  void *x1[2] = {nullptr, nullptr}, *x2[2] = {nullptr, nullptr};
  LDCCHK(make_input((size_t)B * L * cin1, 31u, &x1[1], &x1[0]));
  if (cin2) LDCCHK(make_input((size_t)B * L * cin2, 32u, &x2[1], &x2[0]));
  void *part = nullptr, *cnt = nullptr;
  LDCCHK(keep.alloc(&part, (size_t)(8 << 20) * 4));
  LDCCHK(keep.alloc(&cnt, 1024 * 4));
  HIPCHK(hipMemset(cnt, 0, 1024 * 4));
  hipStream_t s = c->own_stream;
  void *y[2], *st[2], *cm[2];
  for (int v = 0; v < 2; ++v) {
    LDCCHK(keep.alloc(&y[v], n_out * 2));
    LDCCHK(keep.alloc(&st[v], stat_n * 4));
    LDCCHK(keep.alloc(&cm[v], cm_n * 4));
    HIPCHK(hipMemset(y[v], 0, n_out * 2));
    HIPCHK(hipMemset(st[v], 0, stat_n * 4));
    HIPCHK(hipMemset(cm[v], 0, cm_n * 4));
    HIPCHK(hipDeviceSynchronize());
    ConvCall cc;
    cc.B = B; cc.L_in = L; cc.L_rows = L_out; cc.x1 = x1[v]; cc.x2 = x2[v]; cc.y = y[v]; cc.y_ld = cout;
    if (with_gn) { cc.gn_sum = (float*)st[v]; cc.gn_groups = groups; }
    if (with_colmax) { cc.colmax = (unsigned*)cm[v]; cc.colmax_lo = 0; cc.colmax_hi = cout; cc.colmax_stride = cout; }
    cc.sk_part = (float*)part; cc.sk_part_cap = (long long)8 << 20; cc.sk_count = (unsigned*)cnt; cc.sk_count_cap = 1024;
    cc.tune = &c->tune;
    HIPCHK(launch_conv(ly[v], cc, s));
  }
  HIPCHK(hipStreamSynchronize(s));
  std::vector<uint16_t> h0(n_out), h1(n_out);
  HIPCHK(hipMemcpy(h0.data(), y[0], n_out * 2, hipMemcpyDeviceToHost));
// ... 174 lines not shown
```

ladiffcodec_amd/csrc/ldc_internal.h:

```cpp
#pragma once
#include "../../include/ladiffcodec.h"

#include <hip/hip_runtime.h>
#include <math.h>
#include <stdarg.h>
#include <stdio.h>
#include <string.h>

#include <algorithm>
#include <chrono>
#include <functional>
#include <map>
#include <memory>
#include <set>
#include <string>
#include <vector>

#include "ldc_kernels.h"

extern long long g_device_syncs;
inline hipError_t counted_device_sync() {
  ++g_device_syncs;
  return hipDeviceSynchronize();
}
// ... 196 lines not shown
};

struct StepGraph {
  int B = 0, L = 0, F = 0, n = 0;
  int ragged = 0;
  int pool_id = 0;
  int win_Ltot = 0, win_O = 0;
  int sampler = SAMPLER_DDPM;
  const float* noise = nullptr;
  float* x = nullptr;
  hipStream_t stream = nullptr;
  hipGraphExec_t exec[4] = {nullptr, nullptr, nullptr, nullptr};
  hipGraphExec_t pexec[kMaxParts][2] = {};
  bool per_part = false;
  std::vector<hipEvent_t> part_ev;
  uint64_t last_use = 0;
  bool any() const { return exec[0] != nullptr; }
  void destroy() {
    if (per_part) exec[0] = nullptr;
    for (hipEvent_t e : part_ev) (void)hipEventDestroy(e);
    part_ev.clear();
    for (auto& e : exec) { if (e) (void)hipGraphExecDestroy(e); e = nullptr; }
    for (auto& pe : pexec) for (auto& e : pe) { if (e) (void)hipGraphExecDestroy(e); e = nullptr; }
    per_part = false;
  }
};

struct ldc_ctx {
  ldc_config cfg;
  int device = 0;
  int dt = DT_F32;
  bool w8 = false;
  bool finalized = false;
  std::map<std::string, HostTensor> raw[2];
  DevMem wmem;
  Codec codec[2];
  UnetW unet;
  StepTables sched{};
  const float* sqrt_alphas_cumprod = nullptr;
  const float* sqrt_one_minus_alphas_cumprod = nullptr;
  const float* p2_loss_weight = nullptr;
  std::vector<float> alphas_cumprod;
  DdimStep* ddim_table = nullptr;
  std::vector<DdimStep> ddim_host;
  std::vector<float> sqrt_recip_ac, sqrt_recipm1_ac;
  DpmStep* dpm_table = nullptr;
  std::vector<DpmStep> dpm_host;
  int* step_state = nullptr;
  std::vector<std::unique_ptr<Plan>> plans;
  std::vector<StepGraph> graphs;
  Halves last_halves;
  hipStream_t aux_stream[kMaxParts] = {nullptr, nullptr, nullptr, nullptr};
  hipEvent_t ev_fork = nullptr, ev_join[kMaxParts] = {nullptr, nullptr, nullptr, nullptr};
  static constexpr int kLstmChunks = 4;
  hipEvent_t lstm_ev[kMaxParts][kLstmChunks + 1] = {};
  hipStream_t calib_stream = nullptr; bool calibrated = false;
  int calib_good = -1, calib_cand = 0; double calib_one_ms = 0, calib_all_ms = 0;
  struct CalibOrder { hipStream_t s; std::vector<hipStream_t> order; int good, cand; double one_ms, all_ms; };
  std::vector<CalibOrder> calib_cache;
  int calib = 1;
  int ends_join = 0;
  int lstm_pipe = 0;
  int split_batch = 2;
  int merge_advance = 1;
  int rvq_tiled = 1;
  int sea_splitk = 1;
  int split_init = 1;
  int split_ends = 1;
  int fp8_act = 1;
  int part_graphs = 1;
  double host_graph_ms = 0, host_wait_ms = 0;
  long long host_graph_launches = 0;
  hipStream_t side_stream[kMaxParts] = {nullptr, nullptr, nullptr, nullptr};
  hipEvent_t ev_side_fork[kMaxParts] = {nullptr, nullptr, nullptr, nullptr}, ev_side_join[kMaxParts] = {nullptr, nullptr, nullptr, nullptr};
  int side_streams = 0;
  int fuse_kmax = 1;
  int fuse_ln = 1;
  int coop_launch = 0;
  int lstm_xcd = 1;
  int num_cus = 256;
  int xcd_resident[2] = {0, 0};
  int coop_resident[2] = {0, 0};
  int fuse_attn_tail = 1;
  int fold_ctx = 1;
  static constexpr int kFlowRing = 32;
  hipEvent_t flow_ev[kFlowRing] = {};
  unsigned long long flow_n = 0;
  int flow_depth = 8;
  int fuse_gn_stats = 1;
  int gn_epi_max_tiles = 1300;
  int gn_epi_min_l = 0;
  int fold_ln = 1;
  int fold_res = 1;
  int fuse_gn_epi = 1;
  ConvTune tune;
  int lstm_stream_only = 0;
  int serial_parts = 0;
  int graph_steps = 0;
  uint64_t use_tick = 0, call_tick = 0;
  size_t plan_bytes = 0, plan_bytes_cap = (size_t)48 << 30;
  int plan_count_cap = 24;
  int live_pools = 0, next_pool_id = 1;
  uint64_t noise_epoch = 0, cur_key = 0;
  unsigned* dev_flag_host = nullptr;
  unsigned* dev_flag_dev = nullptr;
  int enc_final_act = ACT_NONE;
  unsigned long long* tl_buf = nullptr;
  bool timeline = false;
  bool kstamps = false;
  char* scratch = nullptr;
  size_t scratch_cap = 0;
  void* outnorm_ws = nullptr;
  size_t outnorm_ws_bytes = 0;
  float* state_buf = nullptr;
  size_t state_bytes = 0;
  hipStream_t own_stream = nullptr;
  bool profile = false;
  double prof_ms = 0, prof_flops = 0;
  int64_t prof_launches = 0;
  std::vector<std::pair<hipEvent_t, hipEvent_t>> prof_events;
  std::vector<double> prof_event_flops;
  std::vector<int> prof_event_class;
  std::vector<double> prof_event_bytes;
  std::vector<std::string> prof_event_info;
  double cls_ms[LDC_N_CLASSES] = {}, cls_flops[LDC_N_CLASSES] = {}, cls_bytes[LDC_N_CLASSES] = {};
  int64_t cls_launches[LDC_N_CLASSES] = {};
};

inline hipStream_t pick_stream(ldc_ctx* c, void* s) { return s ? reinterpret_cast<hipStream_t>(s) : c->own_stream; }
inline int check_dev_flag(ldc_ctx* c) {
  const unsigned v = c->dev_flag_host ? *reinterpret_cast<volatile unsigned*>(c->dev_flag_host) : 0u;
  if (v) {
    *reinterpret_cast<volatile unsigned*>(c->dev_flag_host) = 0u;
    if (v == LDC_DEV_BAD_CODE) {
      const uint64_t w = *reinterpret_cast<volatile uint64_t*>(c->dev_flag_host + 2);
      return fail(LDC_E_INVALID, "[bad_code] an RVQ code is outside [0, %d) (e.g. codebook %d, item %d, frame %d); the rows of such "
                                 "codes are NaN", c->codec[LDC_MODEL_COND].bins, (int)(w >> 56), (int)((w >> 32) & 0xffffff), (int)(uint32_t)w);
    }
    if (v == 2)
      return fail(LDC_E_HIP, "device-side failure [gn_wait]: the in-launch GroupNorm exchange of a fused conv timed out (its tiles were "
                             "not all resident in time: is the GPU shared with another process?); the outputs of that call are NaN; "
                             "ldc_set_option(ctx, \"fuse_gn_epi\", 0) restores the separate conv + gn_apply launches");
    if (v == kDevFailCtxRange)
      return fail(LDC_E_HIP, "device-side failure [ctx_range]: the LinearAttention context folded into to_qkv met k values outside the range "
                             "its unshifted exponentials are valid for (a column whose sum of exp(k) is below 2^-100 or reaches 1e26: a k of 60 or more); the "
                             "outputs of that call are wrong; ldc_set_option(ctx, \"fold_ctx\", 0) restores the column maximum and the "
                             "context launch, which shift by it");
    c->lstm_xcd = 0;
    return fail(LDC_E_HIP, "device-side failure [coop_lstm]: cooperative LSTM: the hidden-state exchange timed out (its workgroups were "
                           "not co-resident: is the GPU shared with another process?); the outputs of that call are NaN; "
                           "ldc_set_option(ctx, \"lstm_stream\", 1) selects the streamed LSTM kernel");
  }
  return LDC_OK;
}
inline int finish_stream(ldc_ctx* c, void* s) {
  if (!s) {
    HIPCHK(hipStreamSynchronize(c->own_stream));
    return check_dev_flag(c);
  }
  return LDC_OK;
}
inline uint64_t next_noise_key(ldc_ctx* c, bool draws) {
  c->cur_key = c->cfg.noise_seed ^ (c->noise_epoch * 0x9E3779B97F4A7C15ull);
  if (draws) ++c->noise_epoch;
  return c->cur_key;
}
// ... 114 lines not shown
```

ladiffcodec_amd/csrc/ldc_kernels.h:

```cpp
#pragma once
#include <hip/hip_runtime.h>
#include <stdint.h>

namespace ldc {

enum { DT_F32 = 0, DT_BF16 = 1, DT_FP8 = 2 };
enum { ACT_NONE = 0, ACT_SILU = 1, ACT_ELU = 2, ACT_TANH = 3, ACT_GELU = 4, ACT_SIGMOID = 5, ACT_RELU = 6 };
enum { PAD_ZERO = 0, PAD_REFLECT = 1 };
static constexpr int kGnPad = 16;

inline size_t dt_size(int dt) { return dt == DT_F32 ? 4 : (dt == DT_FP8 ? 1 : 2); }

struct ConvLayer {
  int dt = DT_F32;
  int cin1 = 0, cin2 = 0;
  int n = 0;
  int n_pad = 0;
  int bn = 128;
  int taps = 1, stride = 1, dil = 1, pad_left = 0, ups = 0, pad_mode = PAD_ZERO;
  int pre_act = ACT_NONE, post_act = ACT_NONE;
  int tr_stride = 0, tr_cout = 0, tr_trim_left = 0;
  void* w = nullptr;
  float* bias = nullptr;
  int w8 = 0;
// ... 13 lines not shown
  int debug = 0;
  int gn_nap = 16, gn_nap0 = 0;
  int force_tile = -1;
  int xcd_order = 1;
  int lean = 1;
};

struct ConvCall {
  const void* x1 = nullptr;
  const void* x2 = nullptr;
  void* y = nullptr;
  void* y2 = nullptr;
  const void* residual = nullptr;
  int B = 0;
  int L_in = 0;
  int L_rows = 0;
  int L_final = 0;
  int y_ld = 0;
  float* gn_sum = nullptr;
  int gn_groups = 0;
  unsigned* colmax = nullptr;
  int colmax_lo = 0, colmax_hi = 0, colmax_stride = 0;
  float* qkv_ctx_ws = nullptr;
  int qkv_ctx_stride = 0;
  float* sk_part = nullptr;
  unsigned* sk_count = nullptr;
  long long sk_part_cap = 0;
  int sk_count_cap = 0;
  int generic_split = 0;
  void* gn_part = nullptr;
  int gn_mslots = 0;
  const float* gn_gamma = nullptr;
  const float* gn_beta = nullptr;
  const float* gn_ss = nullptr;
  int gn_out = 0;
  unsigned* fail_flag = nullptr;
  float* rowstat_out = nullptr;
  const float* ln_rowstat = nullptr;
  unsigned long long* kst = nullptr;
  const int* kst_step = nullptr;
  int kst_stride = 0;
  const void* ctx = nullptr;
  const int* ctx_fresh = nullptr;
  int ctx_rows = 0, ctx_zero = 0;
  int check_only = 0;
  const ConvTune* tune = nullptr;
  long long* sk_need = nullptr;
  int* route_out = nullptr;
  int* bm_out = nullptr;
};

enum { CONV_ROUTE_NONE = 0, CONV_ROUTE_CIN1_ROWS = 1, CONV_ROUTE_CIN1_GENERIC = 2, CONV_ROUTE_PIPELINED = 3, CONV_ROUTE_GENERIC = 4 };
hipError_t launch_conv(const ConvLayer& ly, const ConvCall& c, hipStream_t s);
long long conv_generic_splitk_floats(const ConvLayer& ly, const ConvCall& c);
size_t conv_packed_weight_bytes(const ConvLayer& ly);
void pack_conv_weights(const ConvLayer& ly, const float* w_oik, void* dst_host);
void pack_conv_weights_fp8(const ConvLayer& ly, const float* w_oik, void* dst_host, float* scales);
void pack_conv_weights_fp8act(const ConvLayer& ly, const float* w_oik, void* dst_host, float* scales);
uint8_t host_f32_to_e4m3(float f);
float host_e4m3_to_f32(uint8_t v);
void pack_convtr_weights(const ConvLayer& ly, const float* w_iok, int cin, int cout, int stride, void* dst_host);
int conv_pick_bn(int n);

hipError_t launch_gn_stats(int dt, const void* x, int B, int L, int C, int groups, float* stats, hipStream_t s, const int* lens = nullptr,
                           int shift = 0);
hipError_t launch_gn_apply(int dt, const void* x, void* y, const void* residual, int B, int L, int C, int groups,
                           const float* stats, const float* gamma, const float* beta, const float* ss_table,
                           int ss_stride, const int* t_ptr, int act, hipStream_t s, void* y_ln = nullptr, const float* ln_g = nullptr, int out8 = 0,
                           const int* lens = nullptr, int shift = 0,
                           int t_stride = 0, int t_rows = 0);
bool gn_apply_ln_fusable(int C);
hipError_t launch_ln_rows(int dt, const void* x, void* y, const void* residual, const float* g, int rows, int C,
                          hipStream_t s, int out8 = 0, const int* lens = nullptr, int shift = 0, int L = 0);
hipError_t launch_mask_rows(int dt, void* x, int B, int L, int C, const int* lens, int shift, hipStream_t s);
hipError_t launch_act(int dt, const void* x, void* y, int64_t n, int act, hipStream_t s, int out8 = 0);

hipError_t launch_linattn(int dt, const void* qkv, void* out, float* ctx_ws, int B, int L, int heads, int dim_head,
                          bool kmax_fused, hipStream_t s, const int* lens = nullptr, int shift = 0, bool ws_zeroed = false);
size_t linattn_ws_floats_per_item(int heads, int dim_head);
bool linattn_tail_supported(int dt, int heads, int dim_head, int C);
hipError_t launch_linattn_ctx(int dt, const void* qkv, float* ctx_ws, int B, int L, int heads, int dim_head, hipStream_t s);
hipError_t launch_linattn_tail(int dt, const void* qkv, const float* ctx_ws, const void* wo_packed, int n_pad, const float* bias, const float* gain,
                               const void* resid, void* out, int B, int L, int heads, int dim_head, int C, unsigned* fail_flag, hipStream_t s);
hipError_t launch_linattn_kmax(int dt, const void* qkv, float* ctx_ws, int B, int L, int heads, int dim_head, hipStream_t s,
                               const int* lens = nullptr, int shift = 0);
constexpr float kLinattnKClamp = 60.0f;
constexpr float kLinattnKsumMin = 7.888609052210118e-31f;
constexpr float kLinattnKsumMax = 1.0e26f;
constexpr unsigned kDevFailCtxRange = 4u;
hipError_t launch_attn_full(int dt, const void* qkv, void* out, int B, int L, int heads, int dim_head, hipStream_t s, const int* lens = nullptr,
                            int shift = 0);

hipError_t launch_to_cl(int dt, const float* x_bcl, void* y_blc, int B, int C, int L, const float* maxabs,
                        int maxabs_per_item, float eps, hipStream_t s);
hipError_t launch_from_cl(int dt, const void* x_blc, float* y_bcl, int B, int C, int L, const float* maxabs,
                          int maxabs_per_item, float eps, hipStream_t s);
hipError_t launch_maxabs(int dt, const void* x, int B, int64_t n_per_item, int per_item, float* maxabs,
                         hipStream_t s);
struct StepTables {
  const float* sqrt_recip_alphas_cumprod;
  const float* sqrt_recipm1_alphas_cumprod;
  const float* posterior_mean_coef1;
  const float* posterior_mean_coef2;
  const float* posterior_log_variance_clipped;
};
hipError_t launch_random_fill(float* x, int64_t n, int uniform, uint64_t seed, unsigned step, hipStream_t s);
hipError_t launch_axpby(float* x, const float* y, float a, float b, int64_t n, hipStream_t s);
hipError_t launch_p_sample_update(int dt, float* x, const void* eps_cl, const float* noise, int64_t noise_step_stride,
                                  void* x_cl, int B, int C, int L, StepTables tb, const int* st,
                                  uint64_t elem_base, hipStream_t s, const int* lens = nullptr);
struct DdimStep;
struct ItemState {
  int t;
  int j;
  unsigned key_lo, key_hi;
  int remaining;
  int len;
  int active;
  int pad_;
  const float* noise;
  const DdimStep* sched;
};
constexpr int kItemStateInts = (int)(sizeof(ItemState) / sizeof(int));
hipError_t launch_items_write(ItemState* dst, const ItemState* src_host, int n, int* lens, int* flens, int up, hipStream_t s);
hipError_t launch_step_begin_items(ItemState* items, int B, int* st, void* zero, size_t zero_bytes, int advance, hipStream_t s);
hipError_t launch_p_sample_update_items(int dt, float* x, int64_t x_item_stride, const void* eps_cl, void* x_cl, int B, int C, int Lmax,
                                        StepTables tb, const ItemState* items, int T, hipStream_t s);
struct DdimStep {
  int t;
  int last;
  float sqrt_an;
  float c;
  float sigma;
  float pad_[3];
};
hipError_t launch_ddim_table_write(DdimStep* dst, const DdimStep* src_host, int n, hipStream_t s);
hipError_t launch_ddim_update(int dt, float* x, const void* eps_cl, const float* noise, int64_t noise_step_stride,
                              void* x_cl, int B, int C, int L, StepTables tb, const DdimStep* sched, const int* st,
                              uint64_t elem_base, hipStream_t s, const int* lens = nullptr);
struct WindowTables {
  const int* cover;
  const float* weight;
  const int* start;
  int Ltot, Lw;
};
enum { WIN_BLEND = 0, WIN_DDPM = 1, WIN_DDIM = 2 };
hipError_t launch_windows_update(int dt, int kind, float* x, const void* eps_cl, const float* noise, int64_t noise_step_stride, void* x_cl,
                                 float* ebar, int C, WindowTables wt, StepTables tb, const DdimStep* sched, const int* st, hipStream_t s);
hipError_t launch_windows_gather(int dt, const float* x, void* y, int W, int C, int Lw, int Ltot, const int* start, int div, hipStream_t s);
struct DpmStep {
  int t;
  int last;
  int has_prev;
  float a;
  float b0;
  float b1;
  float pad_[2];
};
hipError_t launch_dpm_table_write(DpmStep* dst, const DpmStep* src_host, int n, hipStream_t s);
hipError_t launch_dpm_update(int dt, float* x, const void* eps_cl, float* x0_prev, void* x_cl, int B, int C, int L, StepTables tb,
                             const DpmStep* sched, const int* st, hipStream_t s, const int* lens = nullptr);
hipError_t launch_scale_by_maxabs(int dt, void* x, int B, int64_t n_per_item, const float* maxabs, int per_item,
                                  float eps, hipStream_t s);
hipError_t launch_resample(const float* wav, int C, int64_t T, const float* bank, int orig, int nnew, int width, int64_t target, float* out,
                           hipStream_t s);
hipError_t launch_scale_copy(int dt, const void* x, void* y, int B, int64_t n_per_item, const float* maxabs, float eps,
// ... 116 lines not shown
```

ladiffcodec_amd/lib.py:

```python
from __future__ import annotations

import ctypes as C
import os
import subprocess
from typing import Optional

_HERE = os.path.dirname(os.path.abspath(__file__))
LIB_PATH = os.path.join(_HERE, "libladiffcodec.so")
CSRC = os.path.join(_HERE, "csrc")

LDC_F32, LDC_BF16, LDC_BF16_W8 = 0, 1, 2
DTYPES = {"f32": LDC_F32, "bf16": LDC_BF16, "fp8": LDC_BF16_W8}
MODEL_MAIN, MODEL_COND = 0, 1
MAX_RATIOS = 8
STREAM_ENCODER, STREAM_DECODER = 0, 1

EXPORTS = [
    "ldc_last_error", "ldc_version", "ldc_create", "ldc_destroy", "ldc_reseed", "ldc_set_option", "ldc_quantize_e4m3", "ldc_set_weight", "ldc_finalize_weights",
    "ldc_seanet_encode", "ldc_seanet_decode", "ldc_rvq_encode", "ldc_rvq_decode", "ldc_get_cond",
    "ldc_cond_upsample", "ldc_unet_forward", "ldc_p_sample", "ldc_denoise", "ldc_p_sample_loop", "ldc_infilling", "ldc_output_normalise", "ldc_decode", "ldc_ddim_times", "ldc_ddim_sample", "ldc_decode_ddim", "ldc_decode_codes", "ldc_decode_codes_ddim",
    "ldc_dpm_schedule", "ldc_dpm_sample", "ldc_decode_dpm", "ldc_decode_codes_dpm", "ldc_decode_ragged_dpm",
    "ldc_window_layout", "ldc_unet_forward_windows", "ldc_denoise_windows", "ldc_ddim_sample_windows", "ldc_decode_windows", "ldc_decode_ddim_windows",
    "ldc_decode_ragged", "ldc_unet_forward_ragged", "ldc_get_cond_ragged", "ldc_decode_codes_ragged", "ldc_ac_encode_ragged", "ldc_ac_decode_ragged",
    "ldc_unet_forward_items", "ldc_pool_create", "ldc_pool_destroy", "ldc_pool_admit", "ldc_pool_admit_ddim", "ldc_pool_step", "ldc_pool_remaining", "ldc_pool_take", "ldc_pool_peek", "ldc_pool_evict",
    "ldc_stream_min_first", "ldc_stream_create", "ldc_stream_reset", "ldc_stream_destroy", "ldc_seanet_encode_stream", "ldc_seanet_decode_stream", "ldc_get_cond_stream",
    "ldc_sconv1d", "ldc_sconvtr1d", "ldc_slstm", "ldc_unet_debug_tap", "ldc_unet_step_cost", "ldc_profile_enable",
    "ldc_profile_read", "ldc_profile_read_classes", "ldc_conv_microbench", "ldc_conv_compare", "ldc_conv_compare_fp8", "ldc_ln_fold_compare", "ldc_gn_microbench", "ldc_host_stats", "ldc_stream_info", "ldc_clock_sample", "ldc_debug_raise_failure", "ldc_debug_attn_core", "ldc_debug_attention_block", "ldc_debug_sea_conv", "ldc_debug_sea_op", "ldc_debug_sync_count", "ldc_xcc_census", "ldc_timeline_enable", "ldc_timeline_read", "ldc_kstamps_enable", "ldc_kstamps_reset", "ldc_kstamps_read", "ldc_packed_bytes", "ldc_pack_codes", "ldc_unpack_codes",
    "ldc_ac_build_cdf", "ldc_ac_encode", "ldc_ac_decode", "ldc_train_q_sample", "ldc_train_num_timesteps", "ldc_train_predict_x_start", "ldc_train_neg_sdsdr", "ldc_train_l1_loss", "ldc_train_block_ws_floats",
    "ldc_train_block_forward", "ldc_train_block_backward", "ldc_train_layernorm_forward", "ldc_train_layernorm_backward", "ldc_train_adam_step", "ldc_train_adam_step_dev", "ldc_train_pointwise_forward", "ldc_train_pointwise_backward", "ldc_train_linattn_ws_floats", "ldc_train_linattn_forward", "ldc_train_linattn_backward", "ldc_train_conv_forward", "ldc_train_conv_backward", "ldc_train_join", "ldc_train_side_stream", "ldc_train_upsample2", "ldc_train_activation", "ldc_train_attn_ws_floats", "ldc_train_attn_forward", "ldc_train_attn_backward", "ldc_train_convtr_forward", "ldc_train_convtr_backward", "ldc_train_maxscale", "ldc_resample_out_len", "ldc_resample",
]


class LdcConfig(C.Structure):
    _fields_ = [
        ("compute_dtype", C.c_int32), ("rep_dims", C.c_int32), ("n_filters", C.c_int32),
        ("n_residual_layers", C.c_int32), ("lstm", C.c_int32), ("n_enc_ratios", C.c_int32),
        ("enc_ratios", C.c_int32 * MAX_RATIOS), ("diff_dims", C.c_int32), ("n_upsampling_ratios", C.c_int32),
        ("upsampling_ratios", C.c_int32 * MAX_RATIOS), ("unet_scale_cond", C.c_int32), ("unet_scale_x", C.c_int32),
        ("has_cond_model", C.c_int32), ("cond_bandwidth", C.c_float), ("max_batch", C.c_int32),
        ("max_latent_len", C.c_int32), ("noise_seed", C.c_uint64), ("final_activation", C.c_int32),
        ("reserved_", C.c_int32),
    ]


FINAL_ACTIVATIONS = {None: 0, "Identity": 0, "Tanh": 1, "Sigmoid": 2, "ELU": 3, "SiLU": 4, "GELU": 5, "ReLU": 6}


E_INVALID, E_STATE, E_MISSING, E_HIP, E_NOMEM = -1, -2, -3, -4, -5


class LdcError(RuntimeError):
    def __init__(self, code: int, msg: str):
        super().__init__(f"libladiffcodec error {code}: {msg}")
        self.code = code


_lib: Optional[C.CDLL] = None


def build(verbose: bool = False) -> str:
    r = subprocess.run(["make", "-C", CSRC, "-j8"], capture_output=True, text=True)
    if verbose or r.returncode != 0:
        print(r.stdout[-4000:])
        print(r.stderr[-8000:])
    if r.returncode != 0:
        raise RuntimeError("building libladiffcodec.so failed")
    return LIB_PATH


def load() -> C.CDLL:
    global _lib
    if _lib is not None:
        return _lib
    path = os.environ.get("LDC_LIB_PATH", LIB_PATH)
    if not os.path.exists(path):
        raise RuntimeError(f"{path} not found: run `python -c 'import __graft_entry__ as g; g.build()'` "
                           f"(or `make -C {CSRC}`). There is no CPU fallback.")
    lib = C.CDLL(path)
    vp, i32, i64p, fp = C.c_void_p, C.c_int, C.POINTER(C.c_int64), C.c_void_p
    lib.ldc_last_error.restype = C.c_char_p
    lib.ldc_version.restype = C.c_char_p
    lib.ldc_create.argtypes = [C.POINTER(LdcConfig), i32, C.POINTER(vp)]
    lib.ldc_destroy.argtypes = [vp]
    lib.ldc_reseed.argtypes = [vp, C.c_uint64]
    lib.ldc_quantize_e4m3.argtypes = [vp, C.c_int64, vp, vp]
    lib.ldc_set_weight.argtypes = [vp, i32, C.c_char_p, vp, i64p, i32]
    lib.ldc_finalize_weights.argtypes = [vp, i32]
    lib.ldc_seanet_encode.argtypes = [vp, i32, fp, i32, i32, fp, vp]
    lib.ldc_seanet_decode.argtypes = [vp, i32, fp, i32, i32, fp, vp]
    lib.ldc_rvq_encode.argtypes = [vp, fp, i32, i32, i32, vp, fp, vp]
    lib.ldc_rvq_decode.argtypes = [vp, vp, i32, i32, i32, fp, vp]
    lib.ldc_get_cond.argtypes = [vp, fp, i32, i32, C.c_float, fp, vp, vp]
    lib.ldc_cond_upsample.argtypes = [vp, fp, i32, i32, i32, fp, vp]
    lib.ldc_unet_forward.argtypes = [vp, fp, i32, fp, i32, i32, i32, fp, vp]
    lib.ldc_p_sample.argtypes = [vp, fp, i32, fp, fp, i32, i32, i32, vp]
    lib.ldc_denoise.argtypes = [vp, fp, fp, fp, i32, i32, i32, i32, vp]
    lib.ldc_p_sample_loop.argtypes = [vp, fp, fp, fp, i32, i32, i32, i32, vp]
    lib.ldc_infilling.argtypes = [vp, fp, fp, fp, i32, fp, C.c_float, i32, i32, i32, i32, vp]
    lib.ldc_output_normalise.argtypes = [vp, fp, i32, i32, i32, vp]
    lib.ldc_decode.argtypes = [vp, fp, i32, i32, i32, fp, i32, fp, fp, fp, vp, vp]
    lib.ldc_ddim_times.argtypes = [i32, i32, C.POINTER(C.c_int)]
    lib.ldc_ddim_sample.argtypes = [vp, fp, fp, fp, i32, i32, i32, C.c_float, i32, i32, i32, vp]
    lib.ldc_decode_ddim.argtypes = [vp, fp, i32, i32, i32, i32, C.c_float, fp, i32, fp, fp, fp, vp, vp]
    lib.ldc_decode_codes.argtypes = [vp, vp, vp, C.c_int64, i32, i32, i32, i32, i32, fp, i32, fp, fp, fp, vp]
    lib.ldc_decode_codes_ddim.argtypes = [vp, vp, vp, C.c_int64, i32, i32, i32, i32, i32, i32, C.c_float, fp, i32, fp, fp, fp, vp]
    lib.ldc_decode_ragged.argtypes = [vp, fp, C.POINTER(C.c_int32), i32, i32, i32, i32, C.c_float, fp, fp, fp, fp, vp, vp]
    lib.ldc_get_cond_ragged.argtypes = [vp, fp, C.POINTER(C.c_int32), i32, i32, C.c_float, fp, vp, vp]
    lib.ldc_decode_codes_ragged.argtypes = [vp, vp, vp, C.c_int64, i32, i32, i32, i32, C.POINTER(C.c_int32), i32, i32, C.c_float, fp, fp, fp, fp, vp]
    lib.ldc_dpm_schedule.argtypes = [fp, fp, i32, i32, i32, C.POINTER(C.c_int), C.POINTER(C.c_float)]
    lib.ldc_dpm_sample.argtypes = [vp, fp, fp, i32, i32, i32, i32, i32, vp]
    lib.ldc_decode_dpm.argtypes = [vp, fp, i32, i32, i32, i32, i32, fp, fp, fp, vp, vp]
    lib.ldc_decode_codes_dpm.argtypes = [vp, vp, vp, C.c_int64, i32, i32, i32, i32, i32, i32, i32, fp, fp, fp, vp]
    lib.ldc_decode_ragged_dpm.argtypes = [vp, fp, C.POINTER(C.c_int32), i32, i32, i32, i32, fp, fp, fp, vp, vp]
    lib.ldc_window_layout.argtypes = [i32, i32, i32, i32, C.POINTER(C.c_int), C.POINTER(C.c_float)]
    lib.ldc_unet_forward_windows.argtypes = [vp, fp, i32, fp, i32, i32, i32, i32, fp, vp]
    lib.ldc_denoise_windows.argtypes = [vp, fp, fp, fp, i32, i32, i32, i32, i32, vp]
    lib.ldc_ddim_sample_windows.argtypes = [vp, fp, fp, fp, i32, i32, C.c_float, i32, i32, i32, i32, vp]
    lib.ldc_decode_windows.argtypes = [vp, fp, i32, i32, fp, i32, i32, fp, fp, fp, vp, vp]
    lib.ldc_decode_ddim_windows.argtypes = [vp, fp, i32, i32, i32, C.c_float, fp, i32, i32, fp, fp, fp, vp, vp]
    lib.ldc_ac_encode_ragged.argtypes = [vp, vp, vp, vp, i32, i32, i32, i32, i32, vp, C.c_int64, vp, vp]
    lib.ldc_ac_decode_ragged.argtypes = [vp, vp, C.c_int64, vp, vp, vp, i32, i32, i32, i32, i32, vp, vp, vp]
    lib.ldc_unet_forward_ragged.argtypes = [vp, fp, i32, fp, C.POINTER(C.c_int32), i32, i32, i32, fp, vp]
    lib.ldc_unet_forward_items.argtypes = [vp, fp, C.POINTER(C.c_int32), fp, C.POINTER(C.c_int32), i32, i32, i32, fp, vp]
    lib.ldc_pool_create.argtypes = [vp, i32, i32, C.POINTER(vp)]
    lib.ldc_pool_destroy.argtypes = [vp]
    lib.ldc_pool_admit.argtypes = [vp, vp, i32, fp, fp, i32, i32, fp, C.c_uint64, vp]
    lib.ldc_pool_admit_ddim.argtypes = [vp, vp, i32, fp, fp, i32, i32, i32, C.c_float, fp, C.c_uint64, vp]
    lib.ldc_pool_step.argtypes = [vp, vp, i32, vp]
    lib.ldc_pool_remaining.argtypes = [vp, C.POINTER(C.c_int32)]
    lib.ldc_pool_take.argtypes = [vp, vp, i32, fp, vp]
    lib.ldc_pool_peek.argtypes = [vp, vp, i32, fp, vp]
    lib.ldc_pool_evict.argtypes = [vp, i32]
    lib.ldc_stream_min_first.argtypes = [C.POINTER(LdcConfig), i32, i32]
    lib.ldc_stream_create.argtypes = [vp, i32, i32, i32, C.POINTER(vp)]
    lib.ldc_stream_reset.argtypes = [vp, vp, vp]
    lib.ldc_stream_destroy.argtypes = [vp]
    lib.ldc_seanet_encode_stream.argtypes = [vp, vp, fp, i32, fp, vp]
    lib.ldc_seanet_decode_stream.argtypes = [vp, vp, fp, i32, fp, vp]
    lib.ldc_get_cond_stream.argtypes = [vp, vp, fp, i32, C.c_float, fp, vp, vp]
    lib.ldc_sconv1d.argtypes = [vp, fp, i32, i32, i32, vp, vp, i32, i32, i32, i32, i32, i32, fp, vp]
    lib.ldc_sconvtr1d.argtypes = [vp, fp, i32, i32, i32, vp, vp, i32, i32, i32, i32, fp, vp]
    lib.ldc_slstm.argtypes = [vp, fp, i32, i32, i32, C.POINTER(vp), i32, fp, vp]
    lib.ldc_unet_debug_tap.argtypes = [vp, C.c_char_p, fp, C.c_int64, vp]
    lib.ldc_unet_step_cost.argtypes = [vp, i32, i32, C.POINTER(C.c_double), C.POINTER(C.c_double)]
    lib.ldc_profile_enable.argtypes = [vp, i32]
    lib.ldc_profile_read.argtypes = [vp, C.POINTER(C.c_double), C.POINTER(C.c_int64), C.POINTER(C.c_double)]
    lib.ldc_profile_read_classes.argtypes = [vp, C.c_int, C.POINTER(C.c_double), C.POINTER(C.c_int64), C.POINTER(C.c_double), C.POINTER(C.c_double)]
    lib.ldc_set_option.argtypes = [vp, C.c_char_p, i32]
    lib.ldc_train_num_timesteps.argtypes = [vp]
    lib.ldc_train_predict_x_start.argtypes = [vp, vp, vp, vp, i32, i32, i32, vp, vp]
    lib.ldc_train_neg_sdsdr.argtypes = [vp, vp, vp, i32, C.c_int64, C.c_float, vp, vp]
    lib.ldc_host_stats.argtypes = [vp, i32, C.POINTER(C.c_double), C.POINTER(C.c_double), C.POINTER(C.c_int64)]
    lib.ldc_stream_info.argtypes = [vp, C.POINTER(C.c_int), C.POINTER(C.c_int), C.POINTER(C.c_double), C.POINTER(C.c_double), C.POINTER(C.c_int)]
    lib.ldc_clock_sample.argtypes = [vp, C.POINTER(C.c_uint64), vp]
    lib.ldc_xcc_census.argtypes = [vp, vp, i32, i32, vp]
    lib.ldc_conv_microbench.argtypes = [vp, i32, i32, i32, i32, i32, i32, i32, i32, i32, i32, C.POINTER(C.c_double)]
    lib.ldc_conv_compare.argtypes = [vp] + [i32] * 13 + [C.POINTER(C.c_double)] * 3
    lib.ldc_conv_compare_fp8.argtypes = [vp] + [i32] * 10 + [C.POINTER(C.c_double)] * 3
    lib.ldc_ln_fold_compare.argtypes = [vp, i32, i32, i32, i32, C.c_double, C.POINTER(C.c_double), C.POINTER(C.c_double)]
    lib.ldc_debug_attn_core.argtypes = [vp, i32, fp, i32, i32, vp, vp, vp, fp, i32, fp, vp]
    lib.ldc_debug_attention_block.argtypes = [vp, C.c_char_p, fp, i32, i32, fp, vp]
    lib.ldc_debug_sea_conv.argtypes = [vp, fp, i32, i32, i32, vp, vp, i32, i32, i32, i32, i32, i32, i32, fp, fp, C.POINTER(i32), vp]
    lib.ldc_debug_sea_op.argtypes = [vp, i32, i32, i32, fp, i32, i32, fp, C.c_int64, C.POINTER(i32), vp]
    lib.ldc_timeline_enable.argtypes = [vp, i32]
    lib.ldc_timeline_read.argtypes = [vp, i32, i32, C.POINTER(C.c_uint64)]
    lib.ldc_kstamps_enable.argtypes = [vp, i32]
    lib.ldc_kstamps_reset.argtypes = [vp]
    lib.ldc_kstamps_read.argtypes = [vp, i32, i32, C.POINTER(i32), C.POINTER(C.c_uint64), C.c_char_p, i32, C.POINTER(i32)]
    lib.ldc_packed_bytes.argtypes = [i32, i32, i32]
    lib.ldc_pack_codes.argtypes = [vp, vp, i32, i32, i32, i32, vp, C.c_int64, vp]
    lib.ldc_unpack_codes.argtypes = [vp, vp, C.c_int64, i32, i32, i32, i32, vp, vp]
    lib.ldc_ac_build_cdf.argtypes = [vp, vp, i32, i32, i32, C.c_float, i32, vp, vp]
    lib.ldc_ac_encode.argtypes = [vp, vp, vp, i32, i32, i32, i32, i32, vp, C.c_int64, vp, vp]
    lib.ldc_ac_decode.argtypes = [vp, vp, C.c_int64, vp, vp, i32, i32, i32, i32, i32, vp, vp, vp]
    lib.ldc_train_q_sample.argtypes = [vp, fp, vp, fp, i32, i32, i32, fp, vp]
    lib.ldc_train_l1_loss.argtypes = [vp, fp, fp, vp, i32, i32, i32, fp, fp, vp]
    lib.ldc_train_block_ws_floats.argtypes = [i32, i32, i32, i32, i32]
    lib.ldc_train_block_forward.argtypes = [vp, fp, fp, fp, fp, fp, fp, i32, i32, i32, i32, i32, fp, fp, vp]
    lib.ldc_train_block_backward.argtypes = [vp, fp, fp, fp, fp, fp, i32, i32, i32, i32, i32, fp, fp, fp, fp, fp, fp, fp, vp]
    lib.ldc_train_layernorm_forward.argtypes = [vp, fp, fp, i32, i32, i32, fp, fp, vp]
    lib.ldc_train_layernorm_backward.argtypes = [vp, fp, fp, fp, fp, i32, i32, i32, fp, fp, vp]
    lib.ldc_train_pointwise_forward.argtypes = [vp, fp, fp, fp, i32, i32, i32, i32, i32, fp, vp]
    lib.ldc_train_pointwise_backward.argtypes = [vp, fp, fp, fp, i32, i32, i32, i32, i32, fp, fp, fp, vp]
    lib.ldc_train_linattn_ws_floats.argtypes = [i32, i32, i32, i32]
    lib.ldc_train_linattn_ws_floats.restype = C.c_int64
    lib.ldc_train_linattn_forward.argtypes = [vp, fp, i32, i32, i32, i32, fp, fp, vp]
    lib.ldc_train_linattn_backward.argtypes = [vp, fp, fp, i32, i32, i32, i32, fp, fp, vp]
    lib.ldc_train_conv_forward.argtypes = [vp, fp, fp, fp, i32, i32, i32, i32, i32, i32, i32, fp, vp]
    lib.ldc_train_conv_backward.argtypes = [vp, fp, fp, fp, i32, i32, i32, i32, i32, i32, i32, fp, fp, fp, vp]
    lib.ldc_train_join.argtypes = [vp, vp]
    lib.ldc_train_side_stream.argtypes = [vp, C.POINTER(C.c_void_p)]
    lib.ldc_train_upsample2.argtypes = [vp, fp, C.c_int64, i32, i32, fp, vp]
    lib.ldc_train_activation.argtypes = [vp, fp, fp, C.c_int64, i32, fp, vp]
    lib.ldc_train_attn_ws_floats.argtypes = [i32, i32, i32]
    lib.ldc_train_attn_forward.argtypes = [vp, fp, i32, i32, i32, i32, fp, fp, vp]
    lib.ldc_train_attn_backward.argtypes = [vp, fp, fp, i32, i32, i32, i32, fp, fp, vp]
    lib.ldc_train_convtr_forward.argtypes = [vp, fp, fp, fp, i32, i32, i32, i32, i32, fp, vp]
    lib.ldc_train_convtr_backward.argtypes = [vp, fp, fp, fp, i32, i32, i32, i32, i32, fp, fp, fp, vp]
    lib.ldc_train_maxscale.argtypes = [vp, fp, fp, i32, C.c_int64, fp, vp]
    lib.ldc_train_adam_step.argtypes = [vp, fp, fp, fp, fp, C.c_int64, i32, C.c_float, C.c_float, C.c_float, C.c_float, vp]
    lib.ldc_train_adam_step_dev.argtypes = [vp, fp, fp, fp, fp, C.c_int64, vp, C.c_float, C.c_float, C.c_float, C.c_float, vp]
    lib.ldc_resample_out_len.argtypes = [C.c_int64, i32, i32]
    lib.ldc_resample.argtypes = [vp, fp, i32, C.c_int64, i32, i32, fp, vp]
    lib.ldc_gn_microbench.argtypes = [vp, i32, i32, i32, i32, i32, i32, C.POINTER(C.c_double)]
    for name in EXPORTS:
        fn = getattr(lib, name)
        if name in ("ldc_debug_sync_count", "ldc_packed_bytes", "ldc_train_block_ws_floats", "ldc_train_linattn_ws_floats", "ldc_train_attn_ws_floats", "ldc_resample_out_len"):
            fn.restype = C.c_int64
        elif name == "ldc_quantize_e4m3":
            fn.restype = None
        elif name not in ("ldc_last_error", "ldc_version"):
            fn.restype = C.c_int
    _lib = lib
    return lib


def ddim_times(t_start: int, n_steps: int):
    out = (C.c_int * (int(n_steps) + 1))() if n_steps >= 0 else (C.c_int * 1)()
    check(load().ldc_ddim_times(int(t_start), int(n_steps), out))
    return list(out)


def window_layout(Ltot: int, Lw: int, overlap: int, up: int):
    import numpy as np
    starts = (C.c_int * 32)()
    W = load().ldc_window_layout(int(Ltot), int(Lw), int(overlap), int(up), starts, None)
    if W < 0:
        check(W)
    lw = min(int(Lw), int(Ltot))
    weights = (C.c_float * (W * lw))()
    check(min(0, load().ldc_window_layout(int(Ltot), int(Lw), int(overlap), int(up), starts, weights)))
    return list(starts)[:W], np.array(weights, dtype=np.float32).reshape(W, lw)


def dpm_schedule(sqrt_recip, sqrt_recipm1, t_start: int, n_steps: int):
    import numpy as np
    R = np.ascontiguousarray(np.asarray(sqrt_recip, dtype=np.float32))
    M = np.ascontiguousarray(np.asarray(sqrt_recipm1, dtype=np.float32))
    if R.ndim != 1 or R.shape != M.shape:
        raise ValueError("the two tables must be one-dimensional and of one length")
    n = max(int(n_steps), 1)
    t_out, coef = (C.c_int * n)(), (C.c_float * (3 * n))()
    check(load().ldc_dpm_schedule(R.ctypes.data, M.ctypes.data, int(R.shape[0]), int(t_start), int(n_steps), t_out, coef))
# ... 14 lines not shown
```

ladiffcodec_amd/model.py:

```python
from __future__ import annotations

import ctypes as C
from dataclasses import dataclass
from typing import Dict, Optional, Sequence

import numpy as np

from . import lib as L
from .spec import CodecConfig, UnetConfig


@dataclass
class QuantizedResult:
    quantized: "object"
    codes: "object"
    bandwidth: "object"
    penalty: Optional["object"] = None


class Engine:

    def __init__(self, main_codec: CodecConfig, unet: UnetConfig, cond_codec: Optional[CodecConfig] = None,
                 dtype: str = "bf16", device: int = 0, noise_seed: int = 0):
        import torch
# ... 135 lines not shown
        q = self._empty(B, D, F)
        s = self._enter()
        L.check(self.lib.ldc_rvq_encode(self._ctx, z.data_ptr(), B, F, n_q, codes.data_ptr(), q.data_ptr(), s))
        self._exit()
        return q, codes

    def rvq_decode(self, codes):
        codes = codes.to(self.device, self.torch.int64).contiguous()
        n_q, B, F = codes.shape
        q = self._empty(B, self.main_codec.rep_dims, F)
        s = self._enter()
        L.check(self.lib.ldc_rvq_decode(self._ctx, codes.data_ptr(), B, F, n_q, q.data_ptr(), s))
        self._exit()
        return q

    def resample(self, wav, orig_freq: int, new_freq: int = 16000):
        wav = self._f32(wav)
        Cc, T = wav.shape
        out = self._empty(Cc, int(self.lib.ldc_resample_out_len(T, int(orig_freq), int(new_freq))))
        s = self._enter()
        L.check(self.lib.ldc_resample(self._ctx, wav.data_ptr(), Cc, T, int(orig_freq), int(new_freq), out.data_ptr(), s))
        self._exit()
        return out

    def get_cond(self, wav, bandwidth: float = 0.0, return_codes: bool = False):
        wav = self._f32(wav)
        B, _, T = wav.shape
        F = -(-T // self.cond_codec.hop_length)
        n_q = self.cond_codec.n_q_for_bandwidth(bandwidth if bandwidth > 0 else None)
        cond = self._empty(B, self.cond_codec.rep_dims, F)
        codes = self._empty(n_q, B, F, dtype=self.torch.int64) if return_codes else None
        s = self._enter()
        L.check(self.lib.ldc_get_cond(self._ctx, wav.data_ptr(), B, T, float(bandwidth), cond.data_ptr(),
                                      codes.data_ptr() if codes is not None else None, s))
        self._exit()
        return (cond, codes) if return_codes else cond

    def get_cond_ragged(self, wav, lengths, bandwidth: float = 0.0, return_codes: bool = False):
        wav = self._f32(wav)
        B, _, T = wav.shape
        lens = self._lengths(list(lengths), B)
        F = T // self.cond_codec.hop_length
        n_q = self.cond_codec.n_q_for_bandwidth(bandwidth if bandwidth > 0 else None)
        cond = self._empty(B, self.cond_codec.rep_dims, F)
        codes = self._empty(n_q, B, F, dtype=self.torch.int64) if return_codes else None
        s = self._enter()
        try:
            L.check(self.lib.ldc_get_cond_ragged(self._ctx, wav.data_ptr(), lens, B, T, float(bandwidth), cond.data_ptr(),
                                                 codes.data_ptr() if codes is not None else None, s))
        finally:
            self._exit()
        return (cond, codes) if return_codes else cond

    def open_stream(self, which: int, side: int, B: int) -> "CodecStream":
        return CodecStream(self, which, side, B)

    def cond_upsample(self, cond, normalise: int = 0):
        cond = self._f32(cond)
        B, Cc, F = cond.shape
        f = int(np.prod(self.unet.upsampling_ratios or ()))
        img = self._empty(B, Cc, F * f)
        s = self._enter()
        L.check(self.lib.ldc_cond_upsample(self._ctx, cond.data_ptr(), B, F, normalise, img.data_ptr(), s))
        self._exit()
        return img

    def unet_forward(self, x, t: int, cond):
        x, cond = self._f32(x), self._f32(cond)
        B, Cx, Lx = x.shape
        eps = self._empty(B, Cx, Lx)
        s = self._enter()
        L.check(self.lib.ldc_unet_forward(self._ctx, x.data_ptr(), int(t), cond.data_ptr(), B, Lx, cond.shape[2],
                                          eps.data_ptr(), s))
        self._exit()
        return eps

    def debug_tap(self, name: str, shape):
        out = self._empty(*shape)
        s = self._enter()
        L.check(self.lib.ldc_unet_debug_tap(self._ctx, name.encode(), out.data_ptr(), out.numel(), s))
        self._exit()
        return out

    ATTN_CORE_KINDS = {"linattn": 0, "linattn_kmax_fused": 1, "linattn_ctx_tail": 2, "attn_full": 3}

    def debug_attn_core(self, kind: str, qkv, to_out=None):
        qkv = self._f32(qkv)
        B, _, Lx = qkv.shape
        k = self.ATTN_CORE_KINDS[kind]
        w = b = g = r = None
        Cc = 0
        if k == 2:
            w, b, g = (np.ascontiguousarray(np.asarray(t, dtype=np.float32)) for t in to_out[:3])
            r = self._f32(to_out[3])
            Cc = int(w.shape[0])
        out = self._empty(B, Cc if k == 2 else 128, Lx)
        hp = lambda a: a.ctypes.data_as(C.c_void_p) if a is not None else None
        s = self._enter()
        try:
            L.check(self.lib.ldc_debug_attn_core(self._ctx, k, qkv.data_ptr(), B, Lx, hp(w), hp(b), hp(g),
                                                 r.data_ptr() if r is not None else None, Cc, out.data_ptr(), s))
        finally:
            self._exit()
        return out

    def debug_attention_block(self, name: str, x):
        x = self._f32(x)
        B, _, Lx = x.shape
        out = self.torch.empty_like(x)
        s = self._enter()
        try:
            L.check(self.lib.ldc_debug_attention_block(self._ctx, name.encode(), x.data_ptr(), B, Lx, out.data_ptr(), s))
        finally:
            self._exit()
        return out

    SEA_ROUTES = {1: "cin1_rows", 2: "cin1_generic", 3: "pipelined", 4: "generic"}
    SEA_OP_KINDS = ("conv_cin1", "conv", "convtr", "res", "lstm")

    def debug_sea_conv(self, x, w, b, stride=1, dilation=1, causal=True, transposed=False, pre_elu=False, residual=None):
        x = self._f32(x)
        w = np.ascontiguousarray(w, np.float32)
        b = np.ascontiguousarray(b, np.float32) if b is not None else None
        B, Cin, Lx = x.shape
        if transposed:
            _, Cout, k = w.shape
            Lout = Lx * stride
        else:
            Cout, _, k = w.shape
            Lout = -(-Lx // stride)
        r = self._f32(residual) if residual is not None else None
        y = self._empty(B, Cout, Lout)
        route = (C.c_int * 8)()
        s = self._enter()
        try:
            L.check(self.lib.ldc_debug_sea_conv(self._ctx, x.data_ptr(), B, Cin, Lx, w.ctypes.data_as(C.c_void_p),
                                                b.ctypes.data_as(C.c_void_p) if b is not None else None, Cout, k, stride, dilation,
                                                int(causal), int(transposed), int(pre_elu), r.data_ptr() if r is not None else None,
                                                y.data_ptr(), route, s))
        finally:
            self._exit()
        rep = {"route": self.SEA_ROUTES.get(route[0], "none")}
        if route[0] == 4:
            rep.update(tile=tuple(route[1:5]), ksplit=route[5], tg=route[6], bn=route[7])
        return y, rep

    def debug_sea_op_info(self, which: int, decoder: bool, index: int, B: int, Lx: int):
        info = (C.c_int * 4)()
        L.check(self.lib.ldc_debug_sea_op(self._ctx, which, int(decoder), index, None, B, Lx, None, 0, info, None))
        return self.SEA_OP_KINDS[info[0]], info[1], info[2], info[3]

    def debug_sea_op(self, which: int, decoder: bool, index: int, x):
        x = self._f32(x)
        B, _, Lx = x.shape
        _, _, Co, Lo = self.debug_sea_op_info(which, decoder, index, B, Lx)
        out = self._empty(B, Co, Lo)
        info = (C.c_int * 4)()
        s = self._enter()
        try:
            L.check(self.lib.ldc_debug_sea_op(self._ctx, which, int(decoder), index, x.data_ptr(), B, Lx, out.data_ptr(), out.numel(), info, s))
        finally:
            self._exit()
        return out

    def p_sample(self, x, t: int, cond, noise=None):
        x = self._f32(x).clone()
        cond = self._f32(cond)
        noise = self._f32(noise) if noise is not None else None
        B, _, Lx = x.shape
        s = self._enter()
        L.check(self.lib.ldc_p_sample(self._ctx, x.data_ptr(), int(t), cond.data_ptr(),
                                      noise.data_ptr() if noise is not None else None, B, Lx, cond.shape[2], s))
        self._exit()
        return x

    def denoise(self, img, cond, n_steps: int, noise=None, inplace: bool = False):
        img = self._f32(img)
        if not inplace:
            img = img.clone()
        cond = self._f32(cond)
        noise = self._f32(noise) if noise is not None else None
        B, _, Lx = img.shape
        s = self._enter()
        L.check(self.lib.ldc_denoise(self._ctx, img.data_ptr(), cond.data_ptr(),
                                     noise.data_ptr() if noise is not None else None, int(n_steps), B, Lx, cond.shape[2], s))
        self._exit()
        return img
# ... 788 lines not shown
```

Baseline: 645.7 audio-s/wall-s.

## Fuse full softmax attention with output projection and residual in one tail kernel

Adds a FULL variant of the attention tail kernel. For short sequences it runs flash-style softmax attention per head in fp32 MFMA inside the same workgroup that then does the output projection, bias and residual add. This removes the separate full-attention launch and its intermediate round trip through memory. The linear-attention tail is also restructured: one wave per 64 columns, bias folded into the accumulator init, a single-reduction LayerNorm, and a swizzled LDS residual staging path. Optional s_memtime stamps and a route-debug API are added, which bring in extra code and register pressure.

```diff
diff --git a/include/ladiffcodec.h b/include/ladiffcodec.h
--- a/include/ladiffcodec.h
+++ b/include/ladiffcodec.h
@@ -252,6 +252,7 @@
 
 int ldc_debug_attn_core(ldc_ctx* ctx, int kind, const float* qkv, int B, int L, const float* w_out, const float* b_out,
                         const float* gain, const float* resid, int C, float* out, void* stream);
+int ldc_debug_attention_route(ldc_ctx* ctx, const char* name, int B, int L, int ragged, int* n_ops, char* infos, int info_cap);
 int ldc_debug_attention_block(ldc_ctx* ctx, const char* name, const float* x, int B, int L, float* out, void* stream);
 
 int ldc_debug_sea_conv(ldc_ctx* ctx, const float* x, int B, int Cin, int L, const float* w_host, const float* b_host, int Cout, int k,
diff --git a/ladiffcodec_amd/csrc/attention.hip b/ladiffcodec_amd/csrc/attention.hip
--- a/ladiffcodec_amd/csrc/attention.hip
+++ b/ladiffcodec_amd/csrc/attention.hip
@@ -153,6 +153,8 @@
 
 typedef float lf32x16 __attribute__((ext_vector_type(16)));
 typedef __bf16 lbf16x8 __attribute__((ext_vector_type(8)));
+typedef unsigned lu32x4 __attribute__((ext_vector_type(4)));
+typedef unsigned lu32x2 __attribute__((ext_vector_type(2)));
 __device__ __forceinline__ lf32x16 mfma_bf16(const uint4& a, const uint4& b, lf32x16 acc) {
   lbf16x8 va, vb;
   __builtin_memcpy(&va, &a, 16);
@@ -312,55 +314,145 @@
 }
 
 
-__device__ __forceinline__ float reduce16_over32(const float (&v)[16], int lane) {
-  float a8[8], a4[4], a2[2];
-  const bool b4 = lane & 16, b3 = lane & 8, b2 = lane & 4, b1 = lane & 2;
-#pragma unroll
-  for (int k = 0; k < 8; ++k) a8[k] = (b4 ? v[8 + k] : v[k]) + __shfl_xor(b4 ? v[k] : v[8 + k], 16);
-#pragma unroll
-  for (int k = 0; k < 4; ++k) a4[k] = (b3 ? a8[4 + k] : a8[k]) + __shfl_xor(b3 ? a8[k] : a8[4 + k], 8);
-#pragma unroll
-  for (int k = 0; k < 2; ++k) a2[k] = (b2 ? a4[2 + k] : a4[k]) + __shfl_xor(b2 ? a4[k] : a4[2 + k], 4);
-  float a1 = (b1 ? a2[1] : a2[0]) + __shfl_xor(b1 ? a2[0] : a2[1], 2);
-  a1 += __shfl_xor(a1, 1);
-  return a1;
-}
-
-template <int C>
-__global__ __launch_bounds__(256) void linattn_tail_mfma_kernel(const unsigned short* qkv, const float* ws, size_t ws_stride, float scale,
-                                                                const unsigned short* wo, int n_pad, const float* bias, const float* gain,
-                                                                const unsigned short* resid, unsigned short* out, int L, unsigned* fail_flag) {
-  constexpr int D = 32, HD = 128, R = 32, CPW = C / 4, NT = CPW / 32;
+unsigned long long* g_tail_stamps = nullptr;
+
+__device__ __forceinline__ lf32x16 mfma_f32(float a, float b, lf32x16 acc) { return __builtin_amdgcn_mfma_f32_32x32x2f32(a, b, acc, 0, 0, 0); }
+__device__ __forceinline__ float bf_half(unsigned wd, int hi) { return __uint_as_float(hi ? (wd & 0xffff0000u) : (wd << 16)); }
+
+template <int C, bool FULL>
+__global__ __launch_bounds__(C) void linattn_tail_mfma_kernel(const unsigned short* qkv, const float* ws, size_t ws_stride, float scale,
+                                                              const unsigned short* wo, int n_pad, const float* bias, const float* gain,
+                                                              const unsigned short* resid, unsigned short* out, int L, unsigned* fail_flag,
+                                                              unsigned long long* stamps) {
+  constexpr int D = 32, HD = 128, R = 32, NW = C / 64, NT = 2;
   constexpr int AP = HD + 8;
-  constexpr int TP = CPW * 4 + 16;
+  constexpr int SB = R * 128;
+  static_assert((size_t)R * AP * 2 + (size_t)NW * R * 4 + (size_t)2 * C * 4 <= (size_t)NW * SB, "sA, the first partials, bias and gain live inside the staging area");
   extern __shared__ __attribute__((aligned(16))) char smem[];
   unsigned short* sA = reinterpret_cast<unsigned short*>(smem);
-  float* sred = reinterpret_cast<float*>(smem + (size_t)R * AP * 2);
-  float* srow = sred + 4 * R;
-  char* strans = smem + (size_t)R * AP * 2 + (size_t)5 * R * 4;
+  float* sred1 = reinterpret_cast<float*>(smem + (size_t)R * AP * 2);
+  float* sbias = sred1 + NW * R;
+  float* sgain = sbias + C;
+  float* sred2 = reinterpret_cast<float*>(smem + (size_t)NW * SB);
+  constexpr size_t HDR = (size_t)R * AP * 2 + (size_t)NW * R * 4 + (size_t)2 * C * 4;
   const int b = blockIdx.y, tid = threadIdx.x;
   const int w = tid >> 6, lane = tid & 63, i32 = lane & 31, g = lane >> 5;
+  const int wu = __builtin_amdgcn_readfirstlane(w);
   const int r0 = blockIdx.x * R;
   const float* wsb = ws + (size_t)b * ws_stride;
-  const int colw = w * CPW + i32;
+  const int cw = w * 64;
+  unsigned long long t_in = 0, t_w = 0, t_p1 = 0, t_mm = 0, t_ln = 0;
+  if (stamps) t_in = __builtin_amdgcn_s_memtime();
+  const float bias_t = bias[tid];
+  float gain_t = 0.f;
+  if constexpr (!FULL) gain_t = gain[tid];
+  uint4 qq[2];
+  float cx[16], kx[16];
+  if (!FULL && w < 4) {
+    const int n = min(r0 + i32, L - 1);
+#pragma unroll
+    for (int sx = 0; sx < 2; ++sx) qq[sx] = *reinterpret_cast<const uint4*>(qkv + ((size_t)b * L + n) * (3 * HD) + w * D + 16 * sx + 8 * g);
+#pragma unroll
+    for (int m = 0; m < 16; ++m) {
+      const int d0 = 16 * (m >> 3) + 8 * g + (m & 7);
+      kx[m] = wsb[HD + w * D + d0];
+      cx[m] = wsb[2 * HD + (size_t)w * D * D + d0 * D + i32];
+    }
+  }
   uint4 bfr[8][NT];
-#pragma unroll
-  for (int ks = 0; ks < 8; ++ks)
-#pragma unroll
-    for (int j = 0; j < NT; ++j)
-      bfr[ks][j] = *reinterpret_cast<const uint4*>(wo + ((size_t)(ks >> 1) * n_pad + colw + 32 * j) * 32 + (ks & 1) * 16 + 8 * g);
-  float bv[NT], gv[NT];
-#pragma unroll
-  for (int j = 0; j < NT; ++j) { bv[j] = bias[colw + 32 * j]; gv[j] = gain[colw + 32 * j]; }
-  {
+  auto load_fragments = [&]() {
+#pragma unroll
+    for (int ks = 0; ks < 8; ++ks)
+#pragma unroll
+      for (int j = 0; j < NT; ++j)
+        bfr[ks][j] = *reinterpret_cast<const uint4*>(wo + ((size_t)(ks >> 1) * n_pad + cw + 32 * j + i32) * 32 + (ks & 1) * 16 + 8 * g);
+  };
+  if (!FULL || wu >= 4) load_fragments();
+  sbias[tid] = bias_t;
+  if constexpr (!FULL) sgain[tid] = gain_t;
+  if (FULL && wu < 4) {
+    const int h = wu;
+    float* sv = reinterpret_cast<float*>(smem + HDR + (size_t)NW * SB) + h * (32 * 32);
+    const int nq = min(r0 + i32, L - 1);
+    float qf[16];
+    {
+      const lu32x4* qp = reinterpret_cast<const lu32x4*>(qkv + ((size_t)b * L + nq) * (3 * HD) + h * D);
+      lu32x4 qw[4];
+#pragma unroll
+      for (int i = 0; i < 4; ++i) qw[i] = qp[i];
+#pragma unroll
+      for (int t = 0; t < 16; ++t) qf[t] = bf_half(qw[t >> 2][t & 3], g) * scale;
+    }
+    lu32x4 kw[4], vw[2];
+    auto load_tile = [&](int k0) {
+      const lu32x4* kp = reinterpret_cast<const lu32x4*>(qkv + ((size_t)b * L + min(k0 + i32, L - 1)) * (3 * HD) + HD + h * D);
+#pragma unroll
+      for (int i = 0; i < 4; ++i) kw[i] = kp[i];
+#pragma unroll
+      for (int i = 0; i < 2; ++i) {
+        const int id = lane + 64 * i, key = id >> 2, pc = id & 3;
+        vw[i] = *reinterpret_cast<const lu32x4*>(qkv + ((size_t)b * L + min(k0 + key, L - 1)) * (3 * HD) + 2 * HD + h * D + 8 * pc);
+      }
+    };
+    load_tile(0);
+    lf32x16 o;
+#pragma unroll
+    for (int r = 0; r < 16; ++r) o[r] = 0.f;
+    float m = -INFINITY, l = 0.f;
+    for (int k0 = 0; k0 < L; k0 += 32) {
+      float kf[16];
+#pragma unroll
+      for (int t = 0; t < 16; ++t) kf[t] = bf_half(kw[t >> 2][t & 3], g);
+#pragma unroll
+      for (int i = 0; i < 2; ++i) {
+        const int id = lane + 64 * i, key = id >> 2, pc = id & 3;
+        float4 lo, hi;
+        lo.x = bf_half(vw[i].x, 0); lo.y = bf_half(vw[i].x, 1); lo.z = bf_half(vw[i].y, 0); lo.w = bf_half(vw[i].y, 1);
+        hi.x = bf_half(vw[i].z, 0); hi.y = bf_half(vw[i].z, 1); hi.z = bf_half(vw[i].w, 0); hi.w = bf_half(vw[i].w, 1);
+        *reinterpret_cast<float4*>(sv + key * 32 + 8 * pc) = lo;
+        *reinterpret_cast<float4*>(sv + key * 32 + 8 * pc + 4) = hi;
+      }
+      if (k0 + 32 < L) load_tile(k0 + 32);
+      lf32x16 sc;
+#pragma unroll
+      for (int r = 0; r < 16; ++r) sc[r] = 0.f;
+#pragma unroll
+      for (int t = 0; t < 16; ++t) sc = mfma_f32(kf[t], qf[t], sc);
+      float mx = -INFINITY;
+#pragma unroll
+      for (int r = 0; r < 16; ++r) {
+        const int key = k0 + (r & 3) + 8 * (r >> 2) + 4 * g;
+        sc[r] = key < L ? sc[r] : -INFINITY;
+        mx = fmaxf(mx, sc[r]);
+      }
+      mx = fmaxf(mx, __shfl_xor(mx, 32));
+      const float mn = fmaxf(m, mx);
+      const float corr = __expf(m - mn);
+      float ps = 0.f;
+#pragma unroll
+      for (int r = 0; r < 16; ++r) { sc[r] = __expf(sc[r] - mn); ps += sc[r]; }
+      l = l * corr + ps;
+      m = mn;
+#pragma unroll
+      for (int r = 0; r < 16; ++r) o[r] *= corr;
+      asm volatile("" ::: "memory");
+#pragma unroll
+      for (int t = 0; t < 16; ++t) o = mfma_f32(sv[((t & 3) + 8 * (t >> 2) + 4 * g) * 32 + i32], sc[t], o);
+      asm volatile("" ::: "memory");
+    }
+    load_fragments();
+    l += __shfl_xor(l, 32);
+    const float inv = 1.0f / l;
+    unsigned short* arow = sA + (size_t)i32 * AP + h * D;
+#pragma unroll
+    for (int rr = 0; rr < 4; ++rr) {
+      const unsigned lo = (unsigned)af2bf(o[4 * rr] * inv) | ((unsigned)af2bf(o[4 * rr + 1] * inv) << 16);
+      const unsigned hi = (unsigned)af2bf(o[4 * rr + 2] * inv) | ((unsigned)af2bf(o[4 * rr + 3] * inv) << 16);
+      *reinterpret_cast<uint2*>(arow + 8 * rr + 4 * g) = make_uint2(lo, hi);
+    }
+  }
+  if (!FULL && w < 4) {
     const int h = w;
-    const int n = r0 + i32;
-    uint4 qq[2];
-#pragma unroll
-    for (int sx = 0; sx < 2; ++sx) {
-      if (n < L) qq[sx] = *reinterpret_cast<const uint4*>(qkv + ((size_t)b * L + n) * (3 * HD) + h * D + 16 * sx + 8 * g);
-      else qq[sx] = make_uint4(0, 0, 0, 0);
-    }
     uint4 af[2];
     bool ks_bad = false;
 #pragma unroll
@@ -368,11 +460,10 @@
       unsigned wv[4];
 #pragma unroll
       for (int m = 0; m < 8; m += 2) {
-        const int d0 = 16 * sx + 8 * g + m;
-        const float ks0 = wsb[HD + h * D + d0], ks1 = wsb[HD + h * D + d0 + 1];
+        const float ks0 = kx[8 * sx + m], ks1 = kx[8 * sx + m + 1];
         ks_bad |= !(ks0 >= kLinattnKsumMin && ks0 < kLinattnKsumMax) | !(ks1 >= kLinattnKsumMin && ks1 < kLinattnKsumMax);
-        const float c0 = wsb[2 * HD + (size_t)h * D * D + d0 * D + i32] * (scale / ks0);
-        const float c1 = wsb[2 * HD + (size_t)h * D * D + (d0 + 1) * D + i32] * (scale / ks1);
+        const float c0 = cx[8 * sx + m] * (scale / ks0);
+        const float c1 = cx[8 * sx + m + 1] * (scale / ks1);
         wv[m >> 1] = (unsigned)af2bf(c0) | ((unsigned)af2bf(c1) << 16);
       }
       af[sx] = make_uint4(wv[0], wv[1], wv[2], wv[3]);
@@ -419,103 +510,138 @@
       *reinterpret_cast<uint2*>(arow + 8 * rr + 4 * g) = make_uint2(lo, hi);
     }
   }
+  if (stamps) {
+    asm volatile("s_waitcnt vmcnt(0)" ::: "memory");
+    t_w = __builtin_amdgcn_s_memtime();
+  }
   __syncthreads();
+  if (stamps) t_p1 = __builtin_amdgcn_s_memtime();
   lf32x16 acc[NT];
 #pragma unroll
   for (int j = 0; j < NT; ++j)
 #pragma unroll
-    for (int r = 0; r < 16; ++r) acc[j][r] = 0.f;
+    for (int k = 0; k < 4; ++k) {
+      const float4 bq = *reinterpret_cast<const float4*>(sbias + cw + 32 * j + 8 * k + 4 * g);
+      acc[j][4 * k] = bq.x; acc[j][4 * k + 1] = bq.y; acc[j][4 * k + 2] = bq.z; acc[j][4 * k + 3] = bq.w;
+    }
 #pragma unroll
   for (int ks = 0; ks < 8; ++ks) {
     const uint4 afr = *reinterpret_cast<const uint4*>(sA + (size_t)i32 * AP + 16 * ks + 8 * g);
 #pragma unroll
-    for (int j = 0; j < NT; ++j) acc[j] = mfma_bf16(afr, bfr[ks][j], acc[j]);
-  }
-  constexpr int LPR = CPW / 4;
-  constexpr int RPS = 64 / LPR;
-  constexpr int NSW = R / RPS;
-  const int rsub = lane / LPR, piece = lane % LPR;
-  uint2 rres[NSW];
-#pragma unroll
-  for (int sw = 0; sw < NSW; ++sw) {
-    const int n = r0 + sw * RPS + rsub;
-    rres[sw] = n < L ? *reinterpret_cast<const uint2*>(resid + ((size_t)b * L + n) * C + w * CPW + piece * 4) : make_uint2(0, 0);
-  }
+    for (int j = 0; j < NT; ++j) acc[j] = mfma_bf16(bfr[ks][j], afr, acc[j]);
+  }
+  const int rsub = lane >> 3, piece = lane & 7;
+  lu32x4 rres[4];
+#pragma unroll
+  for (int sw = 0; sw < 4; ++sw) {
+    const int n = min(r0 + sw * 8 + rsub, L - 1);
+    rres[sw] = *reinterpret_cast<const lu32x4*>(resid + ((size_t)b * L + n) * C + cw + piece * 8);
+  }
+  float mean = 0.f, rstd = 1.f;
+  float4 gq[NT][4];
+  if constexpr (!FULL) {
+  {
+    float s = 0.f;
+#pragma unroll
+    for (int r = 0; r < 16; ++r)
+#pragma unroll
+      for (int j = 0; j < NT; ++j) s += acc[j][r];
+    s += __shfl_xor(s, 32);
+    if (g == 0) sred1[w * R + i32] = s;
+  }
+  __syncthreads();
+  if (stamps) t_mm = __builtin_amdgcn_s_memtime();
+#pragma unroll
+  for (int ww = 0; ww < NW; ++ww) mean += sred1[ww * R + i32];
+  mean *= 1.0f / (float)C;
 #pragma unroll
   for (int j = 0; j < NT; ++j)
 #pragma unroll
-    for (int r = 0; r < 16; ++r) acc[j][r] += bv[j];
-  const int rr = i32 >> 1;
-  const int my_row = (rr & 3) + 8 * (rr >> 2) + 4 * g;
+    for (int k = 0; k < 4; ++k) gq[j][k] = *reinterpret_cast<const float4*>(sgain + cw + 32 * j + 8 * k + 4 * g);
   {
-    float v[16];
-#pragma unroll
-    for (int r = 0; r < 16; ++r) {
-      float sacc = 0.f;
-#pragma unroll
-      for (int j = 0; j < NT; ++j) sacc += acc[j][r];
-      v[r] = sacc;
-    }
-    const float tot = reduce16_over32(v, lane);
-    if ((lane & 1) == 0) sred[w * R + my_row] = tot;
+    float s = 0.f;
+#pragma unroll
+    for (int r = 0; r < 16; ++r)
+#pragma unroll
+      for (int j = 0; j < NT; ++j) { const float d = acc[j][r] - mean; s = fmaf(d, d, s); }
+    s += __shfl_xor(s, 32);
+    if (g == 0) sred2[w * R + i32] = s;
   }
   __syncthreads();
-  if (tid < R) srow[tid] = (sred[tid] + sred[R + tid] + sred[2 * R + tid] + sred[3 * R + tid]) * (1.0f / (float)C);
-  __syncthreads();
-  float mean[16];
-#pragma unroll
-  for (int r = 0; r < 16; ++r) mean[r] = srow[(r & 3) + 8 * (r >> 2) + 4 * g];
-  {
-    float v[16];
-#pragma unroll
-    for (int r = 0; r < 16; ++r) {
-      float sacc = 0.f;
-#pragma unroll
-      for (int j = 0; j < NT; ++j) { const float d = acc[j][r] - mean[r]; sacc = fmaf(d, d, sacc); }
-      v[r] = sacc;
-    }
-    const float tot = reduce16_over32(v, lane);
-    if ((lane & 1) == 0) sred[w * R + my_row] = tot;
-  }
-  __syncthreads();
-  if (tid < R) srow[tid] = rsqrtf((sred[tid] + sred[R + tid] + sred[2 * R + tid] + sred[3 * R + tid]) * (1.0f / (float)C) + 1e-5f);
-  __syncthreads();
-  char* tw = strans + (size_t)w * R * TP;
-#pragma unroll
-  for (int r = 0; r < 16; ++r) {
-    const int row = (r & 3) + 8 * (r >> 2) + 4 * g;
-    const float rstd = srow[row];
-#pragma unroll
-    for (int j = 0; j < NT; ++j)
-      reinterpret_cast<float*>(tw + (size_t)row * TP)[32 * j + i32] = (acc[j][r] - mean[r]) * rstd * gv[j];
-  }
-#pragma unroll
-  for (int sw = 0; sw < NSW; ++sw) {
-    const int row = sw * RPS + rsub;
-    const int n = r0 + row;
-    const float4 y = *reinterpret_cast<const float4*>(tw + (size_t)row * TP + piece * 16);
-    const float o0 = y.x + abf2f((unsigned short)(rres[sw].x & 0xffffu)), o1 = y.y + abf2f((unsigned short)(rres[sw].x >> 16));
-    const float o2 = y.z + abf2f((unsigned short)(rres[sw].y & 0xffffu)), o3 = y.w + abf2f((unsigned short)(rres[sw].y >> 16));
-    const uint2 o = make_uint2((unsigned)af2bf(o0) | ((unsigned)af2bf(o1) << 16), (unsigned)af2bf(o2) | ((unsigned)af2bf(o3) << 16));
-    if (n < L) *reinterpret_cast<uint2*>(out + ((size_t)b * L + n) * C + w * CPW + piece * 4) = o;
-  }
-}
-
-template <int C>
+  if (stamps) t_ln = __builtin_amdgcn_s_memtime();
+  rstd = 0.f;
+#pragma unroll
+  for (int ww = 0; ww < NW; ++ww) rstd += sred2[ww * R + i32];
+  rstd = rsqrtf(rstd * (1.0f / (float)C) + 1e-5f);
+  }
+  char* st = smem + (FULL ? HDR : (size_t)0) + (size_t)w * SB;
+#pragma unroll
+  for (int sw = 0; sw < 4; ++sw) {
+    const int row = sw * 8 + rsub;
+    *reinterpret_cast<lu32x4*>(st + row * 128 + ((piece ^ (row & 7)) << 4)) = rres[sw];
+  }
+  asm volatile("" ::: "memory");
+  lu32x2 rq[NT][4];
+#pragma unroll
+  for (int j = 0; j < NT; ++j)
+#pragma unroll
+    for (int k = 0; k < 4; ++k) rq[j][k] = *reinterpret_cast<const lu32x2*>(st + i32 * 128 + (((4 * j + k) ^ (i32 & 7)) << 4) + 8 * g);
+#pragma unroll
+  for (int j = 0; j < NT; ++j)
+#pragma unroll
+    for (int k = 0; k < 4; ++k) {
+      lu32x2* p = reinterpret_cast<lu32x2*>(st + i32 * 128 + (((4 * j + k) ^ (i32 & 7)) << 4) + 8 * g);
+      const lu32x2 rv = rq[j][k];
+      float o0 = acc[j][4 * k], o1 = acc[j][4 * k + 1], o2 = acc[j][4 * k + 2], o3 = acc[j][4 * k + 3];
+      if constexpr (!FULL) {
+        o0 = (o0 - mean) * rstd * gq[j][k].x; o1 = (o1 - mean) * rstd * gq[j][k].y;
+        o2 = (o2 - mean) * rstd * gq[j][k].z; o3 = (o3 - mean) * rstd * gq[j][k].w;
+      }
+      o0 += abf2f((unsigned short)(rv.x & 0xffffu)); o1 += abf2f((unsigned short)(rv.x >> 16));
+      o2 += abf2f((unsigned short)(rv.y & 0xffffu)); o3 += abf2f((unsigned short)(rv.y >> 16));
+      lu32x2 o;
+      o.x = (unsigned)af2bf(o0) | ((unsigned)af2bf(o1) << 16);
+      o.y = (unsigned)af2bf(o2) | ((unsigned)af2bf(o3) << 16);
+      *p = o;
+    }
+  asm volatile("" ::: "memory");
+  lu32x4 y[4];
+#pragma unroll
+  for (int sw = 0; sw < 4; ++sw) {
+    const int row = sw * 8 + rsub;
+    y[sw] = *reinterpret_cast<const lu32x4*>(st + row * 128 + ((piece ^ (row & 7)) << 4));
+  }
+#pragma unroll
+  for (int sw = 0; sw < 4; ++sw) {
+    const int n = r0 + sw * 8 + rsub;
+    if (n < L) *reinterpret_cast<lu32x4*>(out + ((size_t)b * L + n) * C + cw + piece * 8) = y[sw];
+  }
+  if (stamps) {
+    asm volatile("s_waitcnt vmcnt(0)" ::: "memory");
+    const unsigned long long t_out = __builtin_amdgcn_s_memtime();
+    if (lane == 0) {
+      unsigned long long* o = stamps + (((size_t)b * gridDim.x + blockIdx.x) * NW + w) * kTailStamps;
+      o[0] = t_in; o[1] = t_w; o[2] = t_p1; o[3] = t_mm; o[4] = t_ln; o[5] = t_out;
+    }
+  }
+}
+
+template <int C, bool FULL>
 static hipError_t launch_tail_cfg(const void* qkv, const float* ws, size_t wss, float scale, const void* wo, int n_pad, const float* bias,
                                   const float* gain, const void* resid, void* out, int B, int L, unsigned* fail_flag, hipStream_t s) {
-  constexpr int R = 32, CPW = C / 4;
-  const size_t lds = (size_t)R * (128 + 8) * 2 + (size_t)5 * R * 4 + (size_t)4 * R * (CPW * 4 + 16);
-  auto kern = linattn_tail_mfma_kernel<C>;
+  constexpr int R = 32, NW = C / 64;
+  const size_t lds = FULL ? (size_t)R * (128 + 8) * 2 + (size_t)NW * R * 4 + (size_t)2 * C * 4 + (size_t)NW * R * 128 + (size_t)4 * 32 * 32 * 4
+                          : (size_t)NW * R * 128 + (size_t)NW * R * 4;
+  auto kern = linattn_tail_mfma_kernel<C, FULL>;
   static bool lds_opt_in = false;
   if (!lds_opt_in) {
     hipError_t e = hipFuncSetAttribute(reinterpret_cast<const void*>(kern), hipFuncAttributeMaxDynamicSharedMemorySize, 160 * 1024);
     if (e != hipSuccess) return e;
     lds_opt_in = true;
   }
-  hipLaunchKernelGGL(kern, dim3((L + R - 1) / R, B), dim3(256), lds, s, reinterpret_cast<const unsigned short*>(qkv), ws, wss, scale,
+  hipLaunchKernelGGL(kern, dim3((L + R - 1) / R, B), dim3(64 * NW), lds, s, reinterpret_cast<const unsigned short*>(qkv), ws, wss, scale,
                      reinterpret_cast<const unsigned short*>(wo), n_pad, bias, gain, reinterpret_cast<const unsigned short*>(resid),
-                     reinterpret_cast<unsigned short*>(out), L, fail_flag);
+                     reinterpret_cast<unsigned short*>(out), L, fail_flag, FULL ? nullptr : g_tail_stamps);
   return hipGetLastError();
 }
 
@@ -536,9 +662,18 @@
   if (!linattn_tail_supported(dt, heads, dim_head, C) || !bias || !gain || !resid) return hipErrorInvalidValue;
   const size_t wss = linattn_ws_per_item(heads, dim_head);
   const float scale = 1.0f / sqrtf((float)dim_head);
-  if (C == 256) return launch_tail_cfg<256>(qkv, ws, wss, scale, wo_packed, n_pad, bias, gain, resid, out, B, L, fail_flag, s);
-  if (C == 512) return launch_tail_cfg<512>(qkv, ws, wss, scale, wo_packed, n_pad, bias, gain, resid, out, B, L, fail_flag, s);
-  return launch_tail_cfg<1024>(qkv, ws, wss, scale, wo_packed, n_pad, bias, gain, resid, out, B, L, fail_flag, s);
+  if (C == 256) return launch_tail_cfg<256, false>(qkv, ws, wss, scale, wo_packed, n_pad, bias, gain, resid, out, B, L, fail_flag, s);
+  if (C == 512) return launch_tail_cfg<512, false>(qkv, ws, wss, scale, wo_packed, n_pad, bias, gain, resid, out, B, L, fail_flag, s);
+  return launch_tail_cfg<1024, false>(qkv, ws, wss, scale, wo_packed, n_pad, bias, gain, resid, out, B, L, fail_flag, s);
+}
+
+hipError_t launch_attn_full_tail(int dt, const void* qkv, const void* wo_packed, int n_pad, const float* bias, const void* resid, void* out,
+                                 int B, int L, int heads, int dim_head, int C, hipStream_t s) {
+  if (!linattn_tail_supported(dt, heads, dim_head, C) || !bias || !resid || L < 1) return hipErrorInvalidValue;
+  const float scale = 1.0f / sqrtf((float)dim_head);
+  if (C == 256) return launch_tail_cfg<256, true>(qkv, nullptr, 0, scale, wo_packed, n_pad, bias, nullptr, resid, out, B, L, nullptr, s);
+  if (C == 512) return launch_tail_cfg<512, true>(qkv, nullptr, 0, scale, wo_packed, n_pad, bias, nullptr, resid, out, B, L, nullptr, s);
+  return launch_tail_cfg<1024, true>(qkv, nullptr, 0, scale, wo_packed, n_pad, bias, nullptr, resid, out, B, L, nullptr, s);
 }
 
 size_t linattn_ws_floats_per_item(int heads, int dim_head) { return linattn_ws_per_item(heads, dim_head); }
diff --git a/ladiffcodec_amd/csrc/ldc_api.cpp b/ladiffcodec_amd/csrc/ldc_api.cpp
--- a/ladiffcodec_amd/csrc/ldc_api.cpp
+++ b/ladiffcodec_amd/csrc/ldc_api.cpp
@@ -808,6 +808,7 @@
   LDC_OPT("fuse_kmax", c->fuse_kmax, true, 0, 1)
   LDC_OPT("fuse_ln", c->fuse_ln, true, 0, 1)
   LDC_OPT("fuse_attn_tail", c->fuse_attn_tail, true, 0, 1)
+  LDC_OPT("fuse_attn_full_tail", c->fuse_attn_full_tail, true, 0, 1)
   LDC_OPT("fold_ctx", c->fold_ctx, true, 0, 1)
   LDC_OPT("conv_lean", c->tune.lean, true, 0, 1)
   LDC_OPT("conv_generic", c->tune.force_generic, true, 0, 1)
@@ -1583,7 +1584,7 @@
     void* xn = lnf ? const_cast<void*>(x) : (xn_pre ? xn_pre : (f8 ? ar->alloc((size_t)rows * a.dim) : act(rows, a.dim)));
     const ConvLayer& qkv_ly = lnf ? a.qkv_ln : (f8 ? a.qkv_f8 : a.qkv);
     void* qkv = act(rows, 3 * hid);
-    void* o = act(rows, hid);
+    void* o = nullptr;
     void* out = act(rows, a.dim);
     const LinAttnW* ap = &a;
     const int* ln = lens();
@@ -1611,6 +1612,7 @@
         }, false, 2.0 * rows * hid * dim, LDC_CLASS_LINATTN, (1.0 * hid + 2.0 * dim) * rows * es);
         return out;
       }
+      o = act(rows, hid);
       if (c->fuse_kmax && !ln) {
         ln_rowstat_next = rowstat;
         conv(qkv_ly, xn, nullptr, qkv, nullptr, L, L, nullptr, reinterpret_cast<unsigned*>(ws), hid, 2 * hid, (int)wss);
@@ -1629,6 +1631,15 @@
     } else {
       ln_rowstat_next = rowstat;
       conv(qkv_ly, xn, nullptr, qkv, nullptr, L, L);
+      if (!ln && c->fuse_attn_full_tail && L <= kAttnFullTailMaxL && !a.out.w8 && linattn_tail_supported(dt, H, Dh, a.dim)) {
+        const int dim = a.dim;
+        info = "attn_full_tail_c" + std::to_string(dim) + "_L" + std::to_string(L) + "_B" + std::to_string(B);
+        add([=](hipStream_t s) {
+          return launch_attn_full_tail(dt, qkv, ap->out.w, ap->out.n_pad, ap->out.bias, x, out, Bn, L, H, Dh, dim, s);
+        }, false, 2.0 * rows * hid * dim, LDC_CLASS_ATTN_FULL, (3.0 * hid + 2.0 * dim) * rows * es);
+        return out;
+      }
+      o = act(rows, hid);
       add([=](hipStream_t s) { return launch_attn_full(dt, qkv, o, Bn, L, H, Dh, s, ln, sh); }, false, 0, LDC_CLASS_ATTN_FULL, 4.0 * rows * hid * es);
       conv(a.out, o, nullptr, out, x, L, L);
       mask(out, L, a.dim);
@@ -2148,12 +2159,10 @@
   return finish_stream(c, stream);
 }
 
-extern "C" int ldc_debug_attention_block(ldc_ctx* c, const char* name, const float* x, int B, int L, float* out, void* stream) {
-  LDCCHK(check_ready(c, LDC_MODEL_MAIN));
-  if (!name || !x || !out || B <= 0 || L <= 0) return fail(LDC_E_INVALID, "bad arguments");
+static int find_attention_block(ldc_ctx* c, const char* name, const LinAttnW** out, bool* linear) {
   const UnetW& u = c->unet;
   const LinAttnW* a = nullptr;
-  bool linear = true;
+  *linear = true;
   const std::string n = name;
   auto level = [&](const char* pre, const std::vector<LevelW>& lv) {
     const size_t pl = strlen(pre);
@@ -2161,9 +2170,43 @@
     const size_t i = (size_t)atoi(n.c_str() + pl);
     if (i < lv.size()) a = &lv[i].attn;
   };
-  if (n == "mid") { a = &u.mid_attn; linear = false; }
+  if (n == "mid") { a = &u.mid_attn; *linear = false; }
   else { level("down", u.downs); level("up", u.ups); }
   if (!a) return fail(LDC_E_INVALID, "unknown attention block '%s' (down0..down%zu, mid, up0..up%zu)", name, u.downs.size() - 1, u.ups.size() - 1);
+  *out = a;
+  return LDC_OK;
+}
+
+extern "C" int ldc_debug_attention_route(ldc_ctx* c, const char* name, int B, int L, int ragged, int* n_ops, char* infos, int info_cap) {
+  LDCCHK(check_ready(c, LDC_MODEL_MAIN));
+  if (!name || !n_ops || B <= 0 || L <= 0 || (infos && info_cap <= 0)) return fail(LDC_E_INVALID, "bad arguments");
+  const LinAttnW* a = nullptr;
+  bool linear = true;
+  LDCCHK(find_attention_block(c, name, &a, &linear));
+  Plan pl;
+  pl.B = B; pl.L = L; pl.ragged = ragged != 0;
+  Arena dry;
+  PlanBuilder pb{c, &pl, &dry, B, dt_size(c->dt)};
+  static int no_lens = 0;
+  if (pl.ragged) pl.lens = &no_lens;
+  pb.sk_count = reinterpret_cast<unsigned*>(dry.alloc(1024 * 4));
+  pb.sk_count_cap = 1024;
+  pb.linattn_ws = (float*)dry.alloc((size_t)B * linattn_ws_floats_per_item(c->unet.heads, c->unet.dim_head) * 4);
+  pb.sk_part = (float*)dry.alloc(16);
+  pb.attention(*a, pb.act(B * L, a->dim), L, linear);
+  if (infos && *n_ops < (int)pl.step_info.size()) return fail(LDC_E_INVALID, "room for %d op descriptions, the block has %zu", *n_ops, pl.step_info.size());
+  *n_ops = (int)pl.step_info.size();
+  for (size_t o = 0; infos && o < pl.step_info.size(); ++o) snprintf(infos + o * info_cap, info_cap, "%s", pl.step_info[o].c_str());
+  return LDC_OK;
+}
+
+extern "C" int ldc_debug_attention_block(ldc_ctx* c, const char* name, const float* x, int B, int L, float* out, void* stream) {
+  LDCCHK(check_ready(c, LDC_MODEL_MAIN));
+  if (!name || !x || !out || B <= 0 || L <= 0) return fail(LDC_E_INVALID, "bad arguments");
+  const UnetW& u = c->unet;
+  const LinAttnW* a = nullptr;
+  bool linear = true;
+  LDCCHK(find_attention_block(c, name, &a, &linear));
   hipStream_t s = pick_stream(c, stream);
   const int dt = c->dt, C = a->dim;
   const size_t es = dt_size(dt);
diff --git a/ladiffcodec_amd/csrc/ldc_api_tuning.cpp b/ladiffcodec_amd/csrc/ldc_api_tuning.cpp
--- a/ladiffcodec_amd/csrc/ldc_api_tuning.cpp
+++ b/ladiffcodec_amd/csrc/ldc_api_tuning.cpp
@@ -695,14 +695,17 @@
 
 extern "C" int ldc_debug_attn_core(ldc_ctx* c, int kind, const float* qkv, int B, int L, const float* w_out, const float* b_out,
                                    const float* gain, const float* resid, int C, float* out, void* stream) {
-  if (!c || !qkv || !out || B < 1 || L < 1 || kind < 0 || kind > 3) return fail(LDC_E_INVALID, "bad arguments");
+  if (!c || !qkv || !out || B < 1 || L < 1 || kind < 0 || kind > 4) return fail(LDC_E_INVALID, "bad arguments");
   HIPCHK(hipSetDevice(c->device));
   const int dt = c->dt, H = 4, D = 32, HD = H * D;
   const size_t es = dt_size(dt), wss = linattn_ws_floats_per_item(H, D);
   if (kind == 2 && (!w_out || !b_out || !gain || !resid || !linattn_tail_supported(dt, H, D, C)))
     return fail(LDC_E_INVALID, "the fused tail needs a bf16 context, C in {256, 512, 1024}, and to_out weight, bias, gain and residual");
+  if (kind == 4 && (!w_out || !b_out || !resid || !linattn_tail_supported(dt, H, D, C)))
+    return fail(LDC_E_INVALID, "the fused bottleneck tail needs a bf16 context, C in {256, 512, 1024}, and to_out weight, bias and residual");
   hipStream_t s = pick_stream(c, stream);
-  const int Co = kind == 2 ? C : HD;
+  const bool tail = kind == 2 || kind == 4;
+  const int Co = tail ? C : HD;
   DevMem keep;
   void *q_cl = nullptr, *o_cl = nullptr, *ws = nullptr, *r_cl = nullptr;
   LDCCHK(keep.alloc(&q_cl, (size_t)B * L * 3 * HD * es));
@@ -710,14 +713,14 @@
   LDCCHK(keep.alloc(&ws, (size_t)B * wss * 4));
   ConvLayer to_out;
   float* d_gain = nullptr;
-  if (kind == 2) {
+  if (tail) {
     const bool saved_w8 = c->w8;
     c->w8 = false;
     std::swap(keep.ptrs, c->wmem.ptrs);
     ConvSpec sp;
     sp.dt = dt; sp.cin1 = HD; sp.cout = C; sp.k = 1;
     int rc = make_conv(c, sp, w_out, b_out, &to_out);
-    if (rc == LDC_OK) rc = c->wmem.upload(&d_gain, std::vector<float>(gain, gain + C));
+    if (rc == LDC_OK && kind == 2) rc = c->wmem.upload(&d_gain, std::vector<float>(gain, gain + C));
     std::swap(keep.ptrs, c->wmem.ptrs);
     c->w8 = saved_w8;
     LDCCHK(rc);
@@ -734,6 +737,39 @@
     HIPCHK(launch_linattn_kmax(dt, q_cl, (float*)ws, B, L, H, D, s));
     HIPCHK(launch_linattn_ctx(dt, q_cl, (float*)ws, B, L, H, D, s));
     HIPCHK(launch_linattn_tail(dt, q_cl, (const float*)ws, to_out.w, to_out.n_pad, to_out.bias, d_gain, r_cl, o_cl, B, L, H, D, C, c->dev_flag_dev, s));
+    if (getenv("LDC_TAIL_STAMPS")) {
+      const int nwv = C / 64, nwg = B * ((L + 31) / 32);
+      const size_t nst = (size_t)nwg * nwv * kTailStamps;
+      void* st = nullptr;
+      LDCCHK(keep.alloc(&st, nst * 8));
+      HIPCHK(hipMemsetAsync(st, 0, nst * 8, s));
+      HIPCHK(launch_linattn_tail(dt, q_cl, (const float*)ws, to_out.w, to_out.n_pad, to_out.bias, d_gain, r_cl, o_cl, B, L, H, D, C, c->dev_flag_dev, s));
+      ldc::g_tail_stamps = (unsigned long long*)st;
+      hipError_t le = launch_linattn_tail(dt, q_cl, (const float*)ws, to_out.w, to_out.n_pad, to_out.bias, d_gain, r_cl, o_cl, B, L, H, D, C, c->dev_flag_dev, s);
+      ldc::g_tail_stamps = nullptr;
+      HIPCHK(le);
+      HIPCHK(hipStreamSynchronize(s));
+      std::vector<unsigned long long> h(nst);
+      HIPCHK(hipMemcpy(h.data(), st, nst * 8, hipMemcpyDeviceToHost));
+      double ph[2][kTailStamps - 1] = {};
+      int cnt[2] = {0, 0};
+      unsigned long long t_first = ~0ull, t_last = 0;
+      for (size_t i = 0; i < (size_t)nwg * nwv; ++i) {
+        const unsigned long long* t = &h[i * kTailStamps];
+        if (!t[kTailStamps - 1]) continue;
+        const int cls = (int)(i % nwv) < 4 ? 0 : 1;
+        for (int k = 0; k + 1 < kTailStamps; ++k) ph[cls][k] += (double)(t[k + 1] - t[k]);
+        ++cnt[cls];
+        t_first = std::min(t_first, t[0]); t_last = std::max(t_last, t[kTailStamps - 1]);
+      }
+      for (int cls = 0; cls < 2; ++cls)
+        if (cnt[cls])
+          fprintf(stderr, "  tail stamps C=%d L=%d B=%d (s_memtime ticks per wave, %s, %d waves): weights landed %.1f | phase 1 + barrier %.1f | GEMM + row sums %.1f | "
+                  "LayerNorm statistics %.1f | gain, residual, stores drained %.1f | first entry -> last end %.0f\n", C, L, B, cls ? "waves 4.." : "head waves", cnt[cls],
+                  ph[cls][0] / cnt[cls], ph[cls][1] / cnt[cls], ph[cls][2] / cnt[cls], ph[cls][3] / cnt[cls], ph[cls][4] / cnt[cls], (double)(t_last - t_first));
+    }
+  } else if (kind == 4) {
+    HIPCHK(launch_attn_full_tail(dt, q_cl, to_out.w, to_out.n_pad, to_out.bias, r_cl, o_cl, B, L, H, D, C, s));
   } else {
     HIPCHK(launch_attn_full(dt, q_cl, o_cl, B, L, H, D, s));
   }
diff --git a/ladiffcodec_amd/csrc/ldc_internal.h b/ladiffcodec_amd/csrc/ldc_internal.h
--- a/ladiffcodec_amd/csrc/ldc_internal.h
+++ b/ladiffcodec_amd/csrc/ldc_internal.h
@@ -302,6 +302,7 @@
   int xcd_resident[2] = {0, 0};
   int coop_resident[2] = {0, 0};
   int fuse_attn_tail = 1;
+  int fuse_attn_full_tail = 1;
   int fold_ctx = 1;
   static constexpr int kFlowRing = 32;
   hipEvent_t flow_ev[kFlowRing] = {};
diff --git a/ladiffcodec_amd/csrc/ldc_kernels.h b/ladiffcodec_amd/csrc/ldc_kernels.h
--- a/ladiffcodec_amd/csrc/ldc_kernels.h
+++ b/ladiffcodec_amd/csrc/ldc_kernels.h
@@ -119,6 +119,11 @@
 hipError_t launch_linattn_ctx(int dt, const void* qkv, float* ctx_ws, int B, int L, int heads, int dim_head, hipStream_t s);
 hipError_t launch_linattn_tail(int dt, const void* qkv, const float* ctx_ws, const void* wo_packed, int n_pad, const float* bias, const float* gain,
                                const void* resid, void* out, int B, int L, int heads, int dim_head, int C, unsigned* fail_flag, hipStream_t s);
+hipError_t launch_attn_full_tail(int dt, const void* qkv, const void* wo_packed, int n_pad, const float* bias, const void* resid, void* out,
+                                 int B, int L, int heads, int dim_head, int C, hipStream_t s);
+constexpr int kAttnFullTailMaxL = 128;
+constexpr int kTailStamps = 6;
+extern unsigned long long* g_tail_stamps;
 hipError_t launch_linattn_kmax(int dt, const void* qkv, float* ctx_ws, int B, int L, int heads, int dim_head, hipStream_t s,
                                const int* lens = nullptr, int shift = 0);
 constexpr float kLinattnKClamp = 60.0f;
diff --git a/ladiffcodec_amd/lib.py b/ladiffcodec_amd/lib.py
--- a/ladiffcodec_amd/lib.py
+++ b/ladiffcodec_amd/lib.py
@@ -25,7 +25,7 @@
     "ldc_unet_forward_items", "ldc_pool_create", "ldc_pool_destroy", "ldc_pool_admit", "ldc_pool_admit_ddim", "ldc_pool_step", "ldc_pool_remaining", "ldc_pool_take", "ldc_pool_peek", "ldc_pool_evict",
     "ldc_stream_min_first", "ldc_stream_create", "ldc_stream_reset", "ldc_stream_destroy", "ldc_seanet_encode_stream", "ldc_seanet_decode_stream", "ldc_get_cond_stream",
     "ldc_sconv1d", "ldc_sconvtr1d", "ldc_slstm", "ldc_unet_debug_tap", "ldc_unet_step_cost", "ldc_profile_enable",
-    "ldc_profile_read", "ldc_profile_read_classes", "ldc_conv_microbench", "ldc_conv_compare", "ldc_conv_compare_fp8", "ldc_ln_fold_compare", "ldc_gn_microbench", "ldc_host_stats", "ldc_stream_info", "ldc_clock_sample", "ldc_debug_raise_failure", "ldc_debug_attn_core", "ldc_debug_attention_block", "ldc_debug_sea_conv", "ldc_debug_sea_op", "ldc_debug_sync_count", "ldc_xcc_census", "ldc_timeline_enable", "ldc_timeline_read", "ldc_kstamps_enable", "ldc_kstamps_reset", "ldc_kstamps_read", "ldc_packed_bytes", "ldc_pack_codes", "ldc_unpack_codes",
+    "ldc_profile_read", "ldc_profile_read_classes", "ldc_conv_microbench", "ldc_conv_compare", "ldc_conv_compare_fp8", "ldc_ln_fold_compare", "ldc_gn_microbench", "ldc_host_stats", "ldc_stream_info", "ldc_clock_sample", "ldc_debug_raise_failure", "ldc_debug_attn_core", "ldc_debug_attention_block", "ldc_debug_attention_route", "ldc_debug_sea_conv", "ldc_debug_sea_op", "ldc_debug_sync_count", "ldc_xcc_census", "ldc_timeline_enable", "ldc_timeline_read", "ldc_kstamps_enable", "ldc_kstamps_reset", "ldc_kstamps_read", "ldc_packed_bytes", "ldc_pack_codes", "ldc_unpack_codes",
     "ldc_ac_build_cdf", "ldc_ac_encode", "ldc_ac_decode", "ldc_train_q_sample", "ldc_train_num_timesteps", "ldc_train_predict_x_start", "ldc_train_neg_sdsdr", "ldc_train_l1_loss", "ldc_train_block_ws_floats",
     "ldc_train_block_forward", "ldc_train_block_backward", "ldc_train_layernorm_forward", "ldc_train_layernorm_backward", "ldc_train_adam_step", "ldc_train_adam_step_dev", "ldc_train_pointwise_forward", "ldc_train_pointwise_backward", "ldc_train_linattn_ws_floats", "ldc_train_linattn_forward", "ldc_train_linattn_backward", "ldc_train_conv_forward", "ldc_train_conv_backward", "ldc_train_join", "ldc_train_side_stream", "ldc_train_upsample2", "ldc_train_activation", "ldc_train_attn_ws_floats", "ldc_train_attn_forward", "ldc_train_attn_backward", "ldc_train_convtr_forward", "ldc_train_convtr_backward", "ldc_train_maxscale", "ldc_resample_out_len", "ldc_resample",
 ]
@@ -159,6 +159,7 @@
     lib.ldc_conv_compare_fp8.argtypes = [vp] + [i32] * 10 + [C.POINTER(C.c_double)] * 3
     lib.ldc_ln_fold_compare.argtypes = [vp, i32, i32, i32, i32, C.c_double, C.POINTER(C.c_double), C.POINTER(C.c_double)]
     lib.ldc_debug_attn_core.argtypes = [vp, i32, fp, i32, i32, vp, vp, vp, fp, i32, fp, vp]
+    lib.ldc_debug_attention_route.argtypes = [vp, C.c_char_p, i32, i32, i32, C.POINTER(C.c_int), C.c_char_p, i32]
     lib.ldc_debug_attention_block.argtypes = [vp, C.c_char_p, fp, i32, i32, fp, vp]
     lib.ldc_debug_sea_conv.argtypes = [vp, fp, i32, i32, i32, vp, vp, i32, i32, i32, i32, i32, i32, i32, fp, fp, C.POINTER(i32), vp]
     lib.ldc_debug_sea_op.argtypes = [vp, i32, i32, i32, fp, i32, i32, fp, C.c_int64, C.POINTER(i32), vp]
diff --git a/ladiffcodec_amd/model.py b/ladiffcodec_amd/model.py
--- a/ladiffcodec_amd/model.py
+++ b/ladiffcodec_amd/model.py
@@ -241,7 +241,7 @@
         self._exit()
         return out
 
-    ATTN_CORE_KINDS = {"linattn": 0, "linattn_kmax_fused": 1, "linattn_ctx_tail": 2, "attn_full": 3}
+    ATTN_CORE_KINDS = {"linattn": 0, "linattn_kmax_fused": 1, "linattn_ctx_tail": 2, "attn_full": 3, "attn_full_tail": 4}
 
     def debug_attn_core(self, kind: str, qkv, to_out=None):
         qkv = self._f32(qkv)
@@ -249,11 +249,11 @@
         k = self.ATTN_CORE_KINDS[kind]
         w = b = g = r = None
         Cc = 0
-        if k == 2:
-            w, b, g = (np.ascontiguousarray(np.asarray(t, dtype=np.float32)) for t in to_out[:3])
+        if k in (2, 4):
+            w, b, g = (np.ascontiguousarray(np.asarray(t, dtype=np.float32)) if t is not None else None for t in to_out[:3])
             r = self._f32(to_out[3])
             Cc = int(w.shape[0])
-        out = self._empty(B, Cc if k == 2 else 128, Lx)
+        out = self._empty(B, Cc if k in (2, 4) else 128, Lx)
         hp = lambda a: a.ctypes.data_as(C.c_void_p) if a is not None else None
         s = self._enter()
         try:
@@ -262,6 +262,14 @@
         finally:
             self._exit()
         return out
+
+    def debug_attention_route(self, name: str, B: int, Lx: int, ragged: bool = False):
+        n = C.c_int(0)
+        L.check(self.lib.ldc_debug_attention_route(self._ctx, name.encode(), int(B), int(Lx), int(ragged), C.byref(n), None, 0))
+        cap = 96
+        infos = C.create_string_buffer(max(1, n.value) * cap)
+        L.check(self.lib.ldc_debug_attention_route(self._ctx, name.encode(), int(B), int(Lx), int(ragged), C.byref(n), infos, cap))
+        return [infos.raw[o * cap:(o + 1) * cap].split(b"\0", 1)[0].decode() for o in range(n.value)]
 
     def debug_attention_block(self, name: str, x):
         x = self._f32(x)
```

New measurement: 650.0 audio-s/wall-s, median of 6. No clear change (+0.7%).
